# davipatti/abdpymc

Hardware: AMD Instinct MI355X
Metric: logp+grad evals/sec (higher is better)
Workload: dtype f64; 1 GPU; synthetic 10000 ind x 200 gaps, fp64, 4 chains/GPU; n_inds=10000, n_gaps=200, storage=f64, chains_per_gpu=4, total_chains=4, parallelism=chains sharded 4/GPU x 1

## Files before the change

abdpymc_amd/csrc/abd_context.hip:

```cpp
#include "abd_host.hpp"

#include <memory>
#include <unordered_map>
#include "abd_small.hpp"
#include "abd_curves.hpp"
#include "abd_risk.hpp"
#include "abd_diag.hpp"
#include "abd_timeline.hpp"

static_assert(ABD_TL_BINS == ABD_TIMELINE_BINS && ABD_TL_MAX_DRAWS == ABD_TIMELINE_MAX_DRAWS && ABD_TL_MAX_Q == ABD_TIMELINE_MAX_Q &&
                  ABD_TL_NINF == ABD_TIMELINE_NINF,
              "abd_timeline.hpp and include/abd_hip.h describe the same counters");

namespace abdi {

namespace {
thread_local std::string g_err = "";
}
int fail(int code, const char* fmt, ...) {
  char buf[512];
  va_list ap;
  va_start(ap, fmt);
  vsnprintf(buf, sizeof buf, fmt, ap);
  va_end(ap);
  g_err = buf;
  return code;
}
const char* last_error() { return g_err.c_str(); }
void set_error(const std::string& msg) { g_err = msg; }

double prior_constant(int G) {
  double v = -(std::lgamma(1.0) + std::lgamma((double)(G - 1)) - std::lgamma((double)G));
  v += -2.0 * (std::lgamma(10.0) + std::lgamma(1.0) - std::lgamma(11.0));
  const double gmu[5] = {2.0, 1.0, 2.0, 1.0, 1.0};
  for (int q = 0; q < 5; ++q) {
    const double al = gmu[q] * gmu[q] / 0.25, be = gmu[q] / 0.25;
    v += al * std::log(be) - std::lgamma(al);
  }
  const double nsd[6] = {1.0, 1.0, 0.5, 0.5, 0.5, 0.5};
  for (int q = 0; q < 6; ++q) v += -std::log(nsd[q]) - 0.5 * kLog2Pi;
  return v;
}

ModelSizes model_sizes(const abd_ctx* c) {
  ModelSizes m;
  m.G = c->G;
  m.dense = c->dense ? 1 : 0;
  m.N = (double)c->N;
  m.cells = (double)c->G * (double)c->N;
  m.Kn = (double)c->n.K;
  m.Ks = (double)c->s.K;
  m.prior_const = c->prior_const;
  return m;
}

void assemble(const abd_ctx* c, const HostTerms& h, const double* t, const double* sums, double* logp, double* grad,
              bool with_priors) {
  assemble_terms(model_sizes(c), h, t, sums, logp, grad, with_priors);
}

ChainPar chain_par(const abd_ctx* c, int chain, const Transformed& tr) {
  ChainPar p;
  chain_par_from_tr(p, &tr.p);
  p.rw = c->slots[chain].rw;
  p.waner = c->slots[chain].waner;
  p.iw = c->slots[chain].iw;
  p.cnt = c->slots[chain].cnt;
  return p;
}
ChainPar chain_par(const abd_ctx* c, int chain, const double* t) { return chain_par(c, chain, transform(t)); }

ConstrainArgs constrain_args(const abd_ctx* c) {
  ConstrainArgs a;
  std::memset(&a, 0, sizeof a);
  a.pw = c->ignore_pcr ? nullptr : c->pw;
  a.N = c->N;
  a.nt = c->nt;
  a.n_chunks = c->n_chunks;
  std::memcpy(a.chunk_mask, c->chunk_mask, sizeof a.chunk_mask);
  return a;
}

#ifdef ABD_STAMPS
unsigned long long* stamps_buffer() {
  static MappedBuf<unsigned long long>& stamps = *new MappedBuf<unsigned long long>();
  if (!stamps) {
    (void)stamps.alloc(4096 * 16);
    if (const char* e = std::getenv("ABD_STAMPS_PTR_OUT")) {
      FILE* f = std::fopen(e, "w");
      if (f) {
        std::fprintf(f, "%llu\n", (unsigned long long)(uintptr_t)stamps.host());
        std::fclose(f);
      }
    }
  }
  return stamps.dev();
}
#endif

void base_args(const abd_ctx* c, EvalArgs& a) {
  std::memset(&a, 0, sizeof a);
  a.y_n = c->n.y;
  a.x_n = c->n.x;
  a.y_s = c->s.y;
  a.x_s = c->s.x;
  a.g_n = c->n.g;
  a.g_s = c->s.g;
  a.ptr_n = c->n.ptr;
  a.ptr_s = c->s.ptr;
  a.j_n = c->n.j;
  a.j_s = c->s.j;
  a.K_n = (int32_t)c->n.K;
  a.K_s = (int32_t)c->s.K;
  a.ob_n = c->ob_n;
  a.ob_s = c->ob_s;
  a.ob_c = c->ob_c;
  a.yx_n = c->n.yx;
  a.yx_s = c->s.yx;
  a.yxi_n = c->n.yxi;
  a.yxi_s = c->s.yxi;
  a.od_n = c->n.od;
  a.od_s = c->s.od;
  a.xc_n = c->n.xc;
  a.xc_s = c->s.xc;
  a.dict_n = c->n.dict;
  a.dict_s = c->s.dict;
  a.n_dict_n = c->n.n_dict;
  a.n_dict_s = c->s.n_dict;
  a.vw = c->vw;
  a.pw = c->ignore_pcr ? nullptr : c->pw;
  a.exp2_tab = c->exp2_tab;
#ifdef ABD_STAMPS
  a.stamps = stamps_buffer();
#endif
  a.G = c->G;
  a.N = c->N;
  a.nt = c->nt;
  a.n_chunks = c->n_chunks;
  a.n_lg = c->n_lg;
  std::memcpy(a.chunk_mask, c->chunk_mask, sizeof a.chunk_mask);
}
int probe_stream_queues(abd_ctx* c) {
  if (c->n_queues > 0) return ABD_OK;
  HIP_TRY(hipSetDevice(c->device));
  constexpr int kCand = 2 * kMaxPipes;
  const int ns = c->n_streams;
  Stream spare[kMaxPipes];
  hipStream_t cand[kCand] = {};
  int n_cand = ns;
  for (int pi = 0; pi < ns; ++pi) cand[pi] = c->pipe[pi].st;
  for (; n_cand < ns + kMaxPipes; ++n_cand) {
    if (spare[n_cand - ns].create() != hipSuccess) {
      (void)hipGetLastError();
      break;
    }
    cand[n_cand] = spare[n_cand - ns];
  }
  DevBuf<unsigned long long> d;
  hipError_t le = d.alloc((size_t)kCand * 2);
  int best_nq = 0, best[kCand] = {};
  for (int attempt = 0; attempt < 3 && best_nq < 4 && le == hipSuccess; ++attempt) {
    le = hipDeviceSynchronize();
    for (int k = 0; k < n_cand && le == hipSuccess; ++k) {
      hipLaunchKernelGGL(abd_spin_kernel, dim3(1), dim3(64), 0, cand[k], d + 2 * k, 15000ull + 2000ull * (unsigned long long)k);
      le = hipGetLastError();
    }
    if (le == hipSuccess) le = hipDeviceSynchronize();
    unsigned long long h[kCand * 2] = {};
    if (le == hipSuccess) le = hipMemcpy(h, d, sizeof(unsigned long long) * 2 * (size_t)n_cand, hipMemcpyDeviceToHost);
    if (le != hipSuccess) break;
    int nq = 0, q_of[kCand] = {};
    unsigned long long busy_until[kCand] = {};
    for (int j = 0; j < n_cand; ++j) {
      int q = -1;
      for (int k = 0; k < nq && q < 0; ++k)
        if (h[2 * j] + 300 >= busy_until[k] && h[2 * j] <= busy_until[k] + 800) q = k;
      if (q < 0) q = nq++;
      q_of[j] = q;
      busy_until[q] = h[2 * j + 1];
    }
    if (nq > best_nq) {
      best_nq = nq;
      std::copy(q_of, q_of + kCand, best);
    }
  }
  const int nq = std::max(1, best_nq);
  if (le == hipSuccess && best_nq > 1) {
    int load[kCand] = {};
    bool used[kCand] = {};
    for (int pi = 0; pi < ns; ++pi) load[best[pi]]++;
    for (int pi = ns - 1; pi >= 1; --pi) {
      const int q = best[pi];
      int q_min = 0;
      for (int k = 1; k < nq; ++k)
        if (load[k] < load[q_min]) q_min = k;
      if (load[q] - load[q_min] < 2) continue;
      int k_spare = -1;
      for (int k = ns; k < n_cand && k_spare < 0; ++k)
        if (!used[k] && best[k] == q_min) k_spare = k;
      if (k_spare < 0) continue;
      used[k_spare] = true;
      std::swap(c->pipe[pi].st, spare[k_spare - ns]);
      cand[pi] = c->pipe[pi].st;
      best[pi] = q_min;
      load[q]--;
      load[q_min]++;
    }
  }
  HIP_TRY(le);
  int renum[kCand], n_seen = 0;
  std::fill(renum, renum + kCand, -1);
  for (int pi = 0; pi < ns; ++pi) {
    if (renum[best[pi]] < 0) renum[best[pi]] = n_seen++;
    c->queue_of_pipe[pi] = renum[best[pi]];
  }
  c->n_queues = std::max(1, n_seen);
  int k = 0;
  bool taken[kMaxPipes] = {};
  for (int round = 0; k < c->n_streams; ++round) {
    bool seen[kMaxPipes] = {};
    for (int pi = 0; pi < c->n_streams; ++pi)
      if (!taken[pi] && !seen[c->queue_of_pipe[pi]]) {
        seen[c->queue_of_pipe[pi]] = true;
// ... 90 lines not shown
    if (fits) {
      std::vector<R> od(code.size(), (R)0);
      for (size_t j = 0; j < (size_t)N; ++j)
        for (size_t g = 0; g < (size_t)G; ++g) od[cell_of(g, j)] = yx[g * N + j].y;
      d.n_dict = (int)dict.size();
      HIP_TRY(d.od.upload(od.data(), od.size() * sizeof(R)));
      HIP_TRY(d.xc.upload(code.data(), code.size()));
      dict.resize(ABD_XDICT, 0.0);
      HIP_TRY(d.dict.upload(dict.data(), ABD_XDICT));
    }
    return ABD_OK;
  }
  std::vector<R> y(std::max<size_t>(K, 1)), x(std::max<size_t>(K, 1));
  std::vector<uint16_t> g(std::max<size_t>(K, 1));
  std::vector<int32_t> jj(std::max<size_t>(K, 1));
  for (size_t k = 0; k < K; ++k) {
    const int64_t src = so.order[k];
    y[k] = (R)o.od[src];
    x[k] = (R)o.log_dilution[src];
    g[k] = (uint16_t)o.idx_gap[src];
    jj[k] = (int32_t)o.idx_ind[src];
  }
  HIP_TRY(d.j.upload(jj.data(), jj.size()));
  HIP_TRY(d.y.upload(y.data(), y.size() * sizeof(R)));
  HIP_TRY(d.x.upload(x.data(), x.size() * sizeof(R)));
  HIP_TRY(d.g.upload(g.data(), g.size()));
  HIP_TRY(d.ptr.upload(so.ptr.data(), so.ptr.size()));
  return ABD_OK;
}

std::vector<uint64_t> pack_ng(const int8_t* src, int G, int N, int nt) {
  std::vector<uint64_t> w((size_t)nt * N, 0);
  if (!src) return w;
  for (int j = 0; j < N; ++j)
    for (int g = 0; g < G; ++g)
      if (src[(size_t)j * G + g]) w[(size_t)(g >> 6) * N + j] |= 1ull << (g & 63);
  return w;
}

namespace {

int validate_desc(const abd_desc* d) {
  const int G = d->n_gaps, N = d->n_inds;
  if (G < 2) return fail(ABD_ERR_ARG, "n_gaps must be >= 2 (Beta(1, n_gaps - 1) prior on p), got %d", G);
  if (G > ABD_MAX_GAPS) return fail(ABD_ERR_ARG, "n_gaps=%d exceeds ABD_MAX_GAPS=%d", G, ABD_MAX_GAPS);
  if (N < 1) return fail(ABD_ERR_ARG, "n_inds must be >= 1, got %d", N);
  if ((int64_t)G * N >= (int64_t)1 << 31) return fail(ABD_ERR_ARG, "n_gaps*n_inds too large");
  if (d->n_chain_slots < 1) return fail(ABD_ERR_ARG, "n_chain_slots must be >= 1");
  if (d->storage != ABD_STORE_F64 && d->storage != ABD_STORE_F32) return fail(ABD_ERR_ARG, "unknown storage %d", d->storage);
  if (!d->vacs) return fail(ABD_ERR_ARG, "vacs is NULL");
  if (d->n_splits < 0 || d->n_splits > 2) return fail(ABD_ERR_ARG, "only implemented 1-3 time chunks (0-2 splits)");
  for (int k = 0; k < d->n_splits; ++k)
    if (d->splits[k] < 0) return fail(ABD_ERR_ARG, "split indexes must be positive");
  if (d->n_splits == 2 && d->splits[0] > d->splits[1]) return fail(ABD_ERR_ARG, "splits must be in ascending order");
  if (d->n_splits > 0 && d->splits[d->n_splits - 1] > G) return fail(ABD_ERR_ARG, "largest split must be less than n_gaps - 1, (%d)", d->splits[d->n_splits - 1]);
  if (d->n_splits == 2 && d->splits[0] == d->splits[1]) return fail(ABD_ERR_ARG, "splits not unique");
  for (int64_t k = 0; k < (int64_t)G * N; ++k) {
    if ((d->vacs[k] != 0 && d->vacs[k] != 1)) return fail(ABD_ERR_ARG, "vacs must be 0/1");
    if (d->pcrpos && d->pcrpos[k] != 0 && d->pcrpos[k] != 1) return fail(ABD_ERR_ARG, "pcrpos must be 0/1");
  }
  return ABD_OK;
}

int derive_sizes(abd_ctx* c, const abd_desc* d, bool one_per_cell) {
  const int G = d->n_gaps, N = d->n_inds;
  c->G = G;
  c->N = N;
  c->nt = (G + 63) / 64;
  c->prior_const = prior_constant(G);
  c->n_lg = (N + 63) / 64;
  c->n_chunks = d->n_splits + 1;
  for (int k = 0; k < d->n_splits; ++k) c->splits[k] = d->splits[k];
  c->storage = d->storage;
  c->dense = one_per_cell;
  if ((int64_t)N * (d->storage == ABD_STORE_F32 ? 8 : 16) * (G + 2) >= ((int64_t)1 << 32)) c->dense = false;
  if (!abd_div_magic_exact((uint64_t)c->n_lg * (uint64_t)G, (uint32_t)G)) c->dense = false;
  if (env_int("ABD_FORCE_SPARSE", 0)) c->dense = false;
  c->ignore_pcr = d->pcrpos == nullptr;
  c->n_slots = d->n_chain_slots;
  {
    const int edges[4] = {0, d->n_splits > 0 ? d->splits[0] : G, d->n_splits > 1 ? d->splits[1] : G, G};
    for (int ch = 0; ch < c->n_chunks; ++ch) {
      const int lo = edges[ch], hi = (ch == c->n_chunks - 1) ? G : edges[ch + 1];
      for (int g = lo; g < hi; ++g) c->chunk_mask[ch][g >> 6] |= 1ull << (g & 63);
    }
  }

  int dev = d->device;
  if (dev < 0) HIP_TRY(hipGetDevice(&dev));
  c->device = dev;
  HIP_TRY(hipSetDevice(dev));
  hipDeviceProp_t prop;
  HIP_TRY(hipGetDeviceProperties(&prop, dev));
  c->n_cu = prop.multiProcessorCount;
  snprintf(c->name, sizeof c->name, "%s %s %d CUs", prop.name, prop.gcnArchName, prop.multiProcessorCount);
  HIP_TRY(c->pipe[0].st.create());
  c->stream = c->pipe[0].st;

  const int bpc = std::max(1, tune_int("ABD_BLOCKS_PER_CU", 2));
  const int sparse_max = std::max(1, std::min((N + ABD_WAVES_PER_BLOCK - 1) / ABD_WAVES_PER_BLOCK, c->n_cu * 16));
  c->blocks_x = std::max(1, std::min(sparse_max, c->n_cu * bpc));
  c->dbpc = std::max(1, tune_int("ABD_DENSE_BLOCKS_PER_CU", 4));
  {
    const int cap = c->n_cu * 8;
    c->ob_n = (int)std::min<int64_t>((d->n.n_obs + ABD_BLOCK - 1) / ABD_BLOCK, cap);
    c->ob_s = (int)std::min<int64_t>((d->s.n_obs + ABD_BLOCK - 1) / ABD_BLOCK, cap);
    c->ob_c = 1;
    c->obs_lanes = d->s.n_obs + d->n.n_obs < (int64_t)256 * N;
    c->obs_lanes = env_int("ABD_OBS_LANES", c->obs_lanes ? 1 : 0) != 0;
  }
  c->blocks_max = std::max({sparse_max, c->n_cu * 16, c->ob_n + c->ob_s + c->ob_c});
  c->dense_blocks = std::min(c->n_cu * c->dbpc, c->blocks_max);
  if (dense_lds_bytes(G, 4) > 160 * 1024) return fail(ABD_ERR_ARG, "LDS tables for n_gaps=%d do not fit", G);
  return ABD_OK;
}

int upload_panels(abd_ctx* c, const abd_desc* d, SortedObs& so_s, SortedObs& so_n) {
  const int G = c->G, N = c->N;
  const auto upload = c->storage == ABD_STORE_F32 ? upload_antigen<float> : upload_antigen<double>;
  if (int rc = upload(c, d->s, so_s, c->s)) return rc;
  if (int rc = upload(c, d->n, so_n, c->n)) return rc;
  c->order_s = std::move(so_s.order);
  c->order_n = std::move(so_n.order);
  c->xc_ok = c->dense && c->s.od && c->n.od;
  c->xc_max_cb = tune_int("ABD_XC_MAX_CB", c->xc_max_cb);
  const size_t words = (size_t)c->nt * N;
  const std::vector<uint64_t> vw = pack_ng(d->vacs, G, N, c->nt);
  const std::vector<uint64_t> pw = pack_ng(d->pcrpos, G, N, c->nt);
  HIP_TRY(c->vw.upload(vw.data(), words));
  HIP_TRY(c->pw.upload(pw.data(), words));
  if (c->dense) {
    std::vector<double> tab(ABD_EXP2_TAB);
    for (int j = 0; j < ABD_EXP2_TAB; ++j) {
      const double t = (double)exp2l((long double)j / (long double)ABD_EXP2_TAB);
      uint64_t bits;
      std::memcpy(&bits, &t, sizeof bits);
      bits = abd_exp2_prebias(bits, j);
      std::memcpy(&tab[(size_t)j], &bits, sizeof bits);
    }
    HIP_TRY(c->exp2_tab.upload(tab.data(), tab.size()));
  }
  HIP_TRY(c->stage_gn.alloc((size_t)G * N));
  return ABD_OK;
}

int create_slots(abd_ctx* c) {
  const size_t words = (size_t)c->nt * c->N;
  c->slots.resize((size_t)c->n_slots);
  for (auto& s : c->slots) {
    HIP_TRY(s.rw.alloc(words));
    HIP_TRY(s.waner.alloc((size_t)c->N));
    HIP_TRY(s.iw.alloc(words));
    HIP_TRY(s.cnt.alloc(2));
  }
  return ABD_OK;
}

int create_pipes(abd_ctx* c) {
  c->n_pipes = std::max(1, std::min(6, env_int("ABD_PIPES", c->n_pipes)));
  if (!c->dense) c->n_pipes = 1;
  c->n_streams = kMaxPipes;
  c->n_sync_slots = std::max(4, c->n_slots);
  for (int pi = 1; pi < c->n_streams; ++pi) {
    HIP_TRY(c->pipe[pi].st.create());
    HIP_TRY(c->join_ev[pi].create(hipEventDisableTiming));
  }
  c->pipe_blocks = std::min(c->dense_blocks, c->n_cu * std::max(1, c->dbpc / c->n_pipes));
  if (const int pb = tune_int("ABD_PIPE_BLOCKS", 0)) c->pipe_blocks = std::max(1, std::min(pb, c->blocks_max));
  c->group_blocks = c->n_cu;
  if (const int gb = tune_int("ABD_GROUP_BLOCKS_PER_CU", 0)) c->group_blocks = std::max(1, std::min(c->n_cu * gb, c->blocks_max));
  for (int pi = 0; pi < kMaxPipes; ++pi)
    if (c->pipe[pi].st)
      for (int b = 0; b < 2; ++b) HIP_TRY(c->pipe[pi].partials[b].alloc((size_t)c->n_slots * c->blocks_max * ABD_NOUT));
  c->xcd_remap = tune_int("ABD_XCD_REMAP", 1) != 0;
  c->fin_rows = std::max(0, tune_int("ABD_FIN_ROWS", 2));
  HIP_TRY(c->out.alloc((size_t)(kResultSlots + c->n_sync_slots) * c->n_slots * ABD_NOUT));
  HIP_TRY(c->d_counts.alloc((size_t)c->n_slots * 2 + 8));
  HIP_TRY(c->d_work.alloc((size_t)2 * c->n_slots));
  HIP_TRY(c->d_counts_chain.alloc((size_t)c->n_slots * 2));
  HIP_TRY(c->d_fin_count.alloc_zero((size_t)kMaxPipes * ABD_MAX_BATCH, c->stream));
  HIP_TRY(c->d_train_count.alloc_zero((size_t)kMaxPipes * (1 + ABD_TRAIN_SHARDS) * ABD_TRAIN_CNT_STRIDE, c->stream));
  c->dense_own_sum = env_int("ABD_DENSE_OWN_SUM", 1) != 0;
  HIP_TRY(c->h_counts_chain.alloc_pinned((size_t)c->n_slots * 2));
  c->g2_refill_min = std::max(1, std::min(64, tune_int("ABD_G2_REFILL_MIN", ABD_G2_REFILL_MIN)));
  c->g2_tail_lanes = std::max(0, std::min(64, tune_int("ABD_G2_TAIL_LANES", ABD_G2_TAIL_LANES)));
  c->g2_tail_age = std::max(0, tune_int("ABD_G2_TAIL_AGE", ABD_G2_TAIL_AGE));
  c->results.resize((size_t)kResultSlots + c->n_sync_slots);
  HIP_TRY(hipStreamSynchronize(c->stream));
  if (c->dense && c->n_pipes > 1) {
    if (int rc = probe_stream_queues(c)) return rc;
    c->n_pipes = std::min(c->n_pipes, c->n_queues);
  }
  return ABD_OK;
}

}

int launch_deterministics(abd_ctx* c, int chain, const double* theta, hipStream_t st, int8_t* out_i, double* out_mun, double* out_mus,
                          double* sums) {
  EvalArgs a;
  base_args(c, a);
  a.n_chains = 1;
  a.ch[0] = chain_par(c, chain, theta);
  const size_t lds = (size_t)3 * (c->G + 1) * sizeof(double2_t);
  const int blocks = std::max(1, std::min((c->N + ABD_WAVES_PER_BLOCK - 1) / ABD_WAVES_PER_BLOCK, c->n_cu * 8));
  if (c->nt > ABD_MAXT)
    hipLaunchKernelGGL(abd_deterministics_kernel<ABD_MAXT_MAX>, dim3(blocks), dim3(ABD_BLOCK), lds, st, a, out_i, out_mun, out_mus, sums);
  else
    hipLaunchKernelGGL(abd_deterministics_kernel<ABD_MAXT>, dim3(blocks), dim3(ABD_BLOCK), lds, st, a, out_i, out_mun, out_mus, sums);
  HIP_TRY(hipGetLastError());
  return ABD_OK;
}

size_t curves_row_cols(const abd_ctx* c) { return (size_t)abd_curves_row_cols(c->G); }
size_t curves_scratch_cols(const abd_ctx* c) { return (size_t)abd_curves_slabs(c->N) * curves_row_cols(c); }

int launch_curves(abd_ctx* c, int chain, const double* theta, double thr_s, double thr_n, hipStream_t st, unsigned long long* scratch,
                  unsigned long long* row) {
  const ChainPar p = chain_par(c, chain, theta);
  CurvesArgs a;
  a.vw = c->vw;
  a.iw = p.iw;
  a.waner = p.waner;
  a.last = c->d_last;
  a.slab_rows = scratch;
  a.rho_n = p.rho_n, a.rho_s = p.rho_s, a.init_n = p.init_n, a.perm_n = p.perm_n, a.temp_n = p.temp_n;
  a.init_s = p.init_s, a.perm_s = p.perm_s;
  a.thr_s = thr_s, a.thr_n = thr_n;
  a.G = c->G, a.N = c->N, a.nt = c->nt, a.n_slabs = abd_curves_slabs(c->N);
  const size_t lds = (size_t)3 * (c->G + 1) * sizeof(double2_t) + (size_t)2 * c->G * sizeof(double) + ((size_t)4 * c->G + ABD_CURVES_NBIN) * sizeof(int);
  const int blocks = std::max(1, std::min(a.n_slabs, c->n_cu * 8));
  if (c->nt > ABD_MAXT)
    hipLaunchKernelGGL(abd_curves_kernel<ABD_MAXT_MAX>, dim3(blocks), dim3(ABD_BLOCK), lds, st, a);
  else
    hipLaunchKernelGGL(abd_curves_kernel<ABD_MAXT>, dim3(blocks), dim3(ABD_BLOCK), lds, st, a);
  HIP_TRY(hipGetLastError());
  const int sum_blocks = (int)((curves_row_cols(c) + ABD_CURVES_SUM_COLS - 1) / ABD_CURVES_SUM_COLS);
  hipLaunchKernelGGL(abd_curves_sum_kernel, dim3(sum_blocks), dim3(ABD_CURVES_SUM_PARTS * ABD_CURVES_SUM_COLS), 0, st, scratch, a.n_slabs,
                     c->G, row);
  HIP_TRY(hipGetLastError());
  return ABD_OK;
}

void split_curves_row(const abd_ctx* c, const unsigned long long* row, int64_t* counts, int64_t* n_infections, double* titer_sums) {
  const size_t G = (size_t)c->G;
  if (counts) std::memcpy(counts, row, 4 * G * sizeof(int64_t));
  if (n_infections) std::memcpy(n_infections, row + 4 * G, ABD_CURVES_NBIN * sizeof(int64_t));
  if (titer_sums) std::memcpy(titer_sums, row + 4 * G + ABD_CURVES_NBIN, 2 * G * sizeof(double));
}

int launch_diag(abd_ctx* c, int chain, const double* theta, hipStream_t st, int64_t d, int64_t H, int64_t L, double* tit, uint32_t* inf,
                unsigned long long* cb2) {
  const ChainPar p = chain_par(c, chain, theta);
  DiagArgs a;
  a.vw = c->vw;
  a.iw = p.iw;
  a.waner = p.waner;
  a.tit = tit, a.inf = reinterpret_cast<DiagInf*>(inf), a.cb2 = cb2;
  a.rho_n = p.rho_n, a.rho_s = p.rho_s, a.init_n = p.init_n, a.perm_n = p.perm_n, a.temp_n = p.temp_n;
  a.init_s = p.init_s, a.perm_s = p.perm_s;
  a.w = diag_draw(d, H, L);
  a.G = c->G, a.N = c->N, a.nt = c->nt;
  const size_t lds = (size_t)3 * (c->G + 1) * sizeof(double2_t);
  const int blocks = std::max(1, std::min((c->N + ABD_WAVES_PER_BLOCK - 1) / ABD_WAVES_PER_BLOCK, c->n_cu * 8));
  if (c->nt > ABD_MAXT)
    hipLaunchKernelGGL(abd_diag_kernel<ABD_MAXT_MAX>, dim3(blocks), dim3(ABD_BLOCK), lds, st, a);
  else
    hipLaunchKernelGGL(abd_diag_kernel<ABD_MAXT>, dim3(blocks), dim3(ABD_BLOCK), lds, st, a);
  HIP_TRY(hipGetLastError());
  return ABD_OK;
}

int launch_diag_export(abd_ctx* c, const void* src, int stride, int width, unsigned long long* dst, hipStream_t st) {
  const int64_t tiles = (int64_t)((c->G + ABD_DIAG_TILE - 1) / ABD_DIAG_TILE) * ((c->N + ABD_DIAG_TILE - 1) / ABD_DIAG_TILE);
  hipLaunchKernelGGL(abd_diag_export_kernel, dim3((unsigned)tiles), dim3(256), 0, st, static_cast<const unsigned char*>(src), stride, width,
                     c->G, c->N, dst);
  HIP_TRY(hipGetLastError());
  return ABD_OK;
}

int launch_timeline(abd_ctx* c, int chain, const double* theta, const double range_n[2], const double range_s[2], hipStream_t st,
                    uint32_t* hist_n, uint32_t* hist_s, uint32_t* cell, uint32_t* ninf) {
  const ChainPar p = chain_par(c, chain, theta);
  TimelineArgs a;
  a.vw = c->vw;
  a.iw = p.iw;
  a.waner = p.waner;
  a.last = c->d_last;
  a.hist_n = hist_n, a.hist_s = hist_s, a.cell = reinterpret_cast<TimelineCell*>(cell), a.ninf = ninf;
  a.rho_n = p.rho_n, a.rho_s = p.rho_s, a.init_n = p.init_n, a.perm_n = p.perm_n, a.temp_n = p.temp_n;
  a.init_s = p.init_s, a.perm_s = p.perm_s;
  a.rn = timeline_range(range_n[0], range_n[1]), a.rs = timeline_range(range_s[0], range_s[1]);
  a.G = c->G, a.N = c->N, a.nt = c->nt;
  a.n_splits = c->n_chunks - 1, a.s0 = c->splits[0], a.s1 = c->splits[1];
  const size_t lds = (size_t)3 * (c->G + 1) * sizeof(double2_t);
  const int blocks = std::max(1, std::min((c->N + ABD_WAVES_PER_BLOCK - 1) / ABD_WAVES_PER_BLOCK, c->n_cu * 8));
  if (c->nt > ABD_MAXT)
    hipLaunchKernelGGL(abd_timeline_kernel<ABD_MAXT_MAX>, dim3(blocks), dim3(ABD_BLOCK), lds, st, a);
  else
    hipLaunchKernelGGL(abd_timeline_kernel<ABD_MAXT>, dim3(blocks), dim3(ABD_BLOCK), lds, st, a);
  HIP_TRY(hipGetLastError());
  return ABD_OK;
}

int launch_timeline_hist_export(abd_ctx* c, const uint32_t* src, int g0, int n_g, void* dst, hipStream_t st) {
  const int64_t cells = (int64_t)n_g * c->N;
  const int blocks = (int)std::max<int64_t>(1, std::min<int64_t>((cells + 31) / 32, (int64_t)c->n_cu * 16));
  hipLaunchKernelGGL(abd_timeline_hist_export_kernel, dim3(blocks), dim3(256), 0, st, reinterpret_cast<const uint4*>(src), c->G, c->N, g0,
                     n_g, static_cast<uint4*>(dst));
  HIP_TRY(hipGetLastError());
  return ABD_OK;
}

int launch_timeline_quantiles(abd_ctx* c, const uint32_t* hist, int64_t chain_stride, int n_chains, const double range[2], int n_q,
                              const double* q, double* out, hipStream_t st) {
  const int64_t tiles = (int64_t)((c->G + ABD_TL_QTILE - 1) / ABD_TL_QTILE) * ((c->N + ABD_TL_QTILE - 1) / ABD_TL_QTILE);
  hipLaunchKernelGGL(abd_timeline_quantile_kernel, dim3((unsigned)tiles), dim3(256), 0, st, hist, chain_stride, n_chains, c->G, c->N,
                     timeline_range(range[0], range[1]), n_q, q, out);
  HIP_TRY(hipGetLastError());
  return ABD_OK;
}

size_t risk_table_cols(const abd_ctx* c) { return (size_t)abd_risk_table_cols(c->G); }
size_t risk_scratch_cols(const abd_ctx* c) { return (size_t)abd_curves_slabs(c->N) * (size_t)abd_risk_packed_cols(c->G); }

int check_risk_spec(const abd_ctx* c, const abd_risk_spec* spec) {
  if (!spec) return fail(ABD_ERR_ARG, "risk: spec is NULL");
  if (spec->start < 0 || spec->end > c->G || (int64_t)spec->end - spec->start < 2)
    return fail(ABD_ERR_ARG, "risk: window (%d, %d) needs 0 <= start, end <= %d and end - start >= 2", spec->start, spec->end, c->G);
  if (spec->first_only != 0 && spec->first_only != 1) return fail(ABD_ERR_ARG, "risk: first_only=%d is not 0 or 1", spec->first_only);
  const struct { const char* name; int n; const double* e; } ag[2] = {{"edges_s", spec->n_edges_s, spec->edges_s},
                                                                     {"edges_n", spec->n_edges_n, spec->edges_n}};
  for (const auto& x : ag) {
    if (x.n < 0 || x.n > ABD_RISK_MAX_EDGES) return fail(ABD_ERR_ARG, "risk: n_%s=%d outside [0, %d]", x.name, x.n, ABD_RISK_MAX_EDGES);
    for (int k = 0; k < x.n; ++k) {
      if (!std::isfinite(x.e[k])) return fail(ABD_ERR_ARG, "risk: %s[%d] is not finite", x.name, k);
      if (k && !(x.e[k] > x.e[k - 1])) return fail(ABD_ERR_ARG, "risk: %s is not strictly ascending at [%d]", x.name, k);
    }
  }
  return ABD_OK;
}

int launch_risk(abd_ctx* c, int chain, const double* theta, const abd_risk_spec& spec, hipStream_t st, unsigned long long* scratch,
                uint32_t* table) {
  const ChainPar p = chain_par(c, chain, theta);
  RiskArgs a;
  a.vw = c->vw;
  a.iw = p.iw;
  a.waner = p.waner;
  a.last = c->d_last;
  a.slab_rows = scratch;
  a.rho_n = p.rho_n, a.rho_s = p.rho_s, a.init_n = p.init_n, a.perm_n = p.perm_n, a.temp_n = p.temp_n;
  a.init_s = p.init_s, a.perm_s = p.perm_s;
  for (int k = 0; k < ABD_RISK_MAX_EDGES; ++k) {
    a.edges_s[k] = k < spec.n_edges_s ? spec.edges_s[k] : HUGE_VAL;
    a.edges_n[k] = k < spec.n_edges_n ? spec.edges_n[k] : HUGE_VAL;
  }
  a.G = c->G, a.N = c->N, a.nt = c->nt, a.n_slabs = abd_curves_slabs(c->N);
  a.start = spec.start, a.end = spec.end, a.first_only = spec.first_only;
  const size_t lds = (size_t)3 * (c->G + 1) * sizeof(double2_t) + (size_t)abd_risk_packed_cols(c->G) * sizeof(unsigned long long) +
                     (size_t)2 * ABD_RISK_MAX_EDGES * sizeof(double);
  const int blocks = std::max(1, std::min(a.n_slabs, c->n_cu * 8));
  if (c->nt > ABD_MAXT)
    hipLaunchKernelGGL(abd_risk_kernel<ABD_MAXT_MAX>, dim3(blocks), dim3(ABD_BLOCK), lds, st, a);
  else
    hipLaunchKernelGGL(abd_risk_kernel<ABD_MAXT>, dim3(blocks), dim3(ABD_BLOCK), lds, st, a);
  HIP_TRY(hipGetLastError());
  const int sum_blocks = (int)((abd_risk_packed_cols(c->G) + ABD_RISK_SUM_COLS - 1) / ABD_RISK_SUM_COLS);
  hipLaunchKernelGGL(abd_risk_sum_kernel, dim3(sum_blocks), dim3(ABD_RISK_SUM_PARTS * ABD_RISK_SUM_COLS), 0, st, scratch, a.n_slabs, c->G,
                     table);
  HIP_TRY(hipGetLastError());
  return ABD_OK;
}

int launch_unpack(abd_ctx* c, int chain, int8_t* dst, hipStream_t st) {
  dim3 grid((c->N + 255) / 256, c->G);
  hipLaunchKernelGGL(abd_unpack_bits_kernel, grid, dim3(256), 0, st, c->slots[(size_t)chain].rw, dst, c->G, c->N);
  HIP_TRY(hipGetLastError());
  return ABD_OK;
}

}

abd_ctx::~abd_ctx() {
  (void)hipSetDevice(device);
  for (Pipe& p : pipe)
    if (p.st) (void)hipStreamSynchronize(p.st);
}

extern "C" {

const char* abd_version(void) { return "abdpymc_amd hip gfx950 0.2"; }

const char* abd_last_error(void) { return last_error(); }

int abd_create(const abd_desc* d, abd_ctx** out) {
  if (!d || !out) return fail(ABD_ERR_ARG, "desc / out is NULL");
  *out = nullptr;
  if (int rc = validate_desc(d)) return rc;
  SortedObs so_s, so_n;
  if (int rc = sort_obs(d->s, d->n_gaps, d->n_inds, "s", so_s)) return rc;
  if (int rc = sort_obs(d->n, d->n_gaps, d->n_inds, "n", so_n)) return rc;
  std::unique_ptr<abd_ctx> c(new (std::nothrow) abd_ctx());
  if (!c) return fail(ABD_ERR_NOMEM, "out of host memory");
  if (int rc = derive_sizes(c.get(), d, so_s.one_per_cell && so_n.one_per_cell)) return rc;
  if (int rc = upload_panels(c.get(), d, so_s, so_n)) return rc;
  if (int rc = create_slots(c.get())) return rc;
  if (int rc = create_pipes(c.get())) return rc;
  *out = c.release();
  return ABD_OK;
}

int abd_destroy(abd_ctx* c) {
  delete c;
  return ABD_OK;
}

int abd_device_name(abd_ctx* c, char* buf, int32_t buflen) {
  if (!c || !buf || buflen < 1) return fail(ABD_ERR_ARG, "bad argument");
  snprintf(buf, (size_t)buflen, "%s", c->name);
  return ABD_OK;
}

int abd_is_dense(abd_ctx* c) { return c && c->dense ? 1 : 0; }
int abd_n_pipes(abd_ctx* c) { return c ? c->n_pipes : -1; }

int abd_set_discrete(abd_ctx* c, int32_t chain, const int8_t* i_raw, const int8_t* waner) {
  if (!c || !i_raw || !waner) return fail(ABD_ERR_ARG, "NULL argument");
  if (chain < 0 || chain >= c->n_slots) return fail(ABD_ERR_ARG, "chain %d outside [0, %d)", chain, c->n_slots);
  const size_t cells = (size_t)c->G * c->N;
  for (size_t k = 0; k < cells; ++k)
    if (i_raw[k] != 0 && i_raw[k] != 1) return fail(ABD_ERR_ARG, "i_raw must be 0/1");
  for (int j = 0; j < c->N; ++j)
    if (waner[j] != 0 && waner[j] != 1) return fail(ABD_ERR_ARG, "ab_s_waner must be 0/1");
  HIP_TRY(hipSetDevice(c->device));
  ChainSlot& s = c->slots[(size_t)chain];
  long long* const cnt = s.cnt;
  if (int jrc = join_pipes(c)) return jrc;
  HIP_TRY(hipStreamSynchronize(c->stream));
  HIP_TRY(hipMemcpy(c->stage_gn, i_raw, cells, hipMemcpyHostToDevice));
  HIP_TRY(hipMemcpy(s.waner, waner, (size_t)c->N, hipMemcpyHostToDevice));
  dim3 grid((c->N + 255) / 256, c->nt);
  hipLaunchKernelGGL(abd_pack_bits_kernel, grid, dim3(256), 0, c->stream, c->stage_gn, s.rw, c->G, c->N, c->nt);
  HIP_TRY(hipGetLastError());
  HIP_TRY(hipMemsetAsync(s.cnt, 0, 2 * sizeof(long long), c->stream));
  if (c->nt > ABD_MAXT)
    hipLaunchKernelGGL(abd_constrain_kernel<ABD_MAXT_MAX>, dim3((c->N + 255) / 256), dim3(256), 0, c->stream, constrain_args(c), s.rw,
                       s.waner, s.iw, reinterpret_cast<unsigned long long*>(cnt));
  else
    hipLaunchKernelGGL(abd_constrain_kernel<ABD_MAXT>, dim3((c->N + 255) / 256), dim3(256), 0, c->stream, constrain_args(c), s.rw,
                       s.waner, s.iw, reinterpret_cast<unsigned long long*>(cnt));
  HIP_TRY(hipGetLastError());
  HIP_TRY(hipStreamSynchronize(c->stream));
  s.set = true;
  return ABD_OK;
}

int abd_flip_discrete(abd_ctx* c, int32_t chain, int64_t flat) {
  if (!c) return fail(ABD_ERR_ARG, "ctx is NULL");
  if (chain < 0 || chain >= c->n_slots) return fail(ABD_ERR_ARG, "chain %d outside [0, %d)", chain, c->n_slots);
  const int64_t total = (int64_t)c->G * c->N + c->N;
  if (flat < 0 || flat >= total) return fail(ABD_ERR_ARG, "flat index %lld outside [0, %lld)", (long long)flat, (long long)total);
  if (!c->slots[(size_t)chain].set) return fail(ABD_ERR_STATE, "chain slot %d has no discrete state", chain);
  HIP_TRY(hipSetDevice(c->device));
  if (int jrc = join_pipes(c)) return jrc;
  ChainSlot& s = c->slots[(size_t)chain];
  long long* const cnt = s.cnt;
  if (c->nt > ABD_MAXT)
    hipLaunchKernelGGL(abd_flip_kernel<ABD_MAXT_MAX>, dim3(1), dim3(1), 0, c->stream, constrain_args(c), s.rw, s.waner, s.iw,
                       reinterpret_cast<unsigned long long*>(cnt), c->G, flat);
  else
    hipLaunchKernelGGL(abd_flip_kernel<ABD_MAXT>, dim3(1), dim3(1), 0, c->stream, constrain_args(c), s.rw, s.waner, s.iw,
                       reinterpret_cast<unsigned long long*>(cnt), c->G, flat);
  HIP_TRY(hipGetLastError());
  return ABD_OK;
}
int abd_deterministics(abd_ctx* c, int32_t chain, const double* theta, int8_t* i, double* mu_n, double* mu_s) {
  if (!c || !theta) return fail(ABD_ERR_ARG, "NULL argument");
  int rc = check_chains(c, 1, &chain);
  if (rc) return rc;
  HIP_TRY(hipSetDevice(c->device));
  if (int jrc = join_pipes(c)) return jrc;
  const size_t cells = (size_t)c->G * c->N;
  if (!c->d_det) HIP_TRY(c->d_det.alloc(2 * cells + (cells + 7) / 8));
  double* d_n = c->d_det;
  double* d_s = c->d_det + cells;
  int8_t* d_i = reinterpret_cast<int8_t*>(c->d_det + 2 * cells);
  if (int lrc = launch_deterministics(c, chain, theta, c->stream, i ? d_i : (int8_t*)nullptr, mu_n ? d_n : (double*)nullptr,
                                      mu_s ? d_s : (double*)nullptr, nullptr))
    return lrc;
  if (mu_n) HIP_TRY(hipMemcpyAsync(mu_n, d_n, cells * sizeof(double), hipMemcpyDeviceToHost, c->stream));
  if (mu_s) HIP_TRY(hipMemcpyAsync(mu_s, d_s, cells * sizeof(double), hipMemcpyDeviceToHost, c->stream));
  if (i) HIP_TRY(hipMemcpyAsync(i, d_i, cells, hipMemcpyDeviceToHost, c->stream));
  HIP_TRY(hipStreamSynchronize(c->stream));
  return ABD_OK;
}

int abd_set_follow_up(abd_ctx* c, const int32_t* last_gap) {
  if (!c) return fail(ABD_ERR_ARG, "ctx is NULL");
  if (last_gap)
    for (int j = 0; j < c->N; ++j)
      if (last_gap[j] < -1 || last_gap[j] >= c->G)
        return fail(ABD_ERR_ARG, "last_gap[%d]=%d outside [-1, %d)", j, last_gap[j], c->G);
  HIP_TRY(hipSetDevice(c->device));
  if (int jrc = join_pipes(c)) return jrc;
  HIP_TRY(hipStreamSynchronize(c->stream));
  if (!last_gap) {
    c->d_last.reset();
    return ABD_OK;
  }
  DevBuf<int32_t> fresh;
  HIP_TRY(fresh.upload(last_gap, (size_t)c->N));
  c->d_last = std::move(fresh);
  return ABD_OK;
}

int abd_curves(abd_ctx* c, int32_t chain, const double* theta, double thr_s, double thr_n, int64_t* counts, int64_t* n_infections,
               double* titer_sums) {
  if (!c || !theta) return fail(ABD_ERR_ARG, "NULL argument");
  int rc = check_chains(c, 1, &chain);
  if (rc) return rc;
  HIP_TRY(hipSetDevice(c->device));
  if (int jrc = join_pipes(c)) return jrc;
  const size_t n_scratch = curves_scratch_cols(c), n_row = curves_row_cols(c);
  if (!c->d_curves) HIP_TRY(c->d_curves.alloc(n_scratch + n_row));
  if (int lrc = launch_curves(c, chain, theta, thr_s, thr_n, c->stream, c->d_curves, c->d_curves + n_scratch)) return lrc;
  std::vector<unsigned long long> h(n_row);
  HIP_TRY(hipMemcpyAsync(h.data(), c->d_curves + n_scratch, n_row * sizeof(unsigned long long), hipMemcpyDeviceToHost, c->stream));
  HIP_TRY(hipStreamSynchronize(c->stream));
  split_curves_row(c, h.data(), counts, n_infections, titer_sums);
  return ABD_OK;
}

int abd_risk(abd_ctx* c, int32_t chain, const double* theta, const abd_risk_spec* spec, int64_t* table) {
  if (!c || !theta || !table) return fail(ABD_ERR_ARG, "NULL argument");
  int rc = check_chains(c, 1, &chain);
  if (rc) return rc;
  if (int src = check_risk_spec(c, spec)) return src;
  HIP_TRY(hipSetDevice(c->device));
  if (int jrc = join_pipes(c)) return jrc;
  const size_t n_scratch = risk_scratch_cols(c), n_tab = risk_table_cols(c);
  if (!c->d_risk) HIP_TRY(c->d_risk.alloc(n_scratch + (n_tab + 1) / 2));
  uint32_t* d_tab = reinterpret_cast<uint32_t*>(c->d_risk + n_scratch);
  if (int lrc = launch_risk(c, chain, theta, *spec, c->stream, c->d_risk, d_tab)) return lrc;
  std::vector<uint32_t> h(n_tab);
  HIP_TRY(hipMemcpyAsync(h.data(), d_tab, n_tab * sizeof(uint32_t), hipMemcpyDeviceToHost, c->stream));
  HIP_TRY(hipStreamSynchronize(c->stream));
  for (size_t e = 0; e < n_tab; ++e) table[e] = (int64_t)h[e];
  return ABD_OK;
}

int abd_get_discrete(abd_ctx* c, int32_t chain, int8_t* i_raw, int8_t* waner) {
  if (!c) return fail(ABD_ERR_ARG, "ctx is NULL");
  int rc = check_chains(c, 1, &chain);
  if (rc) return rc;
  HIP_TRY(hipSetDevice(c->device));
  if (int jrc = join_pipes(c)) return jrc;
  ChainSlot& s = c->slots[(size_t)chain];
  if (i_raw) {
    if (int urc = launch_unpack(c, chain, c->stage_gn, c->stream)) return urc;
    HIP_TRY(hipStreamSynchronize(c->stream));
    HIP_TRY(hipMemcpy(i_raw, c->stage_gn, (size_t)c->G * c->N, hipMemcpyDeviceToHost));
  } else {
    HIP_TRY(hipStreamSynchronize(c->stream));
  }
  if (waner) HIP_TRY(hipMemcpy(waner, s.waner, (size_t)c->N, hipMemcpyDeviceToHost));
  return ABD_OK;
}

int abd_set_launch_config(abd_ctx* c, int32_t blocks, int32_t chains_per_wave) {
  if (!c) return fail(ABD_ERR_ARG, "ctx is NULL");
  if (!(chains_per_wave == 0 || chains_per_wave == 1 || chains_per_wave == 2 || chains_per_wave == 4))
    return fail(ABD_ERR_ARG, "chains_per_wave must be 0 (auto), 1, 2 or 4");
  c->cpw_forced = chains_per_wave;
  if (blocks > 0) {
    if (c->dense)
      c->dense_blocks = std::max(1, std::min(blocks, c->blocks_max));
    else
      c->blocks_x = std::max(1, std::min(blocks, c->blocks_max));
  }
  return ABD_OK;
}

int abd_theta_prior(abd_ctx* c, const double* theta, double* logp, double* grad) {
  if (!c || !theta || !logp) return fail(ABD_ERR_ARG, "NULL argument");
  *logp = priors(prepare(theta), theta, c->G, 0.0, 0.0, 0.0, 0.0, grad, c->prior_const);
  return ABD_OK;
}

int abd_set_individual_offset(abd_ctx* c, int64_t first_individual) {
  if (!c) return fail(ABD_ERR_ARG, "ctx is NULL");
  if (first_individual < 0 || first_individual > 0xFFFFFFFFll) return fail(ABD_ERR_ARG, "first_individual=%lld out of range", (long long)first_individual);
  c->ind_offset = (uint32_t)first_individual;
  return ABD_OK;
}
int abd_stream_queues(abd_ctx* c, int32_t* queue_of_stream, int32_t n) {
  if (!c || !queue_of_stream) return fail(ABD_ERR_ARG, "NULL argument");
  if (int rc = probe_stream_queues(c)) return rc;
  for (int i = 0; i < n; ++i) queue_of_stream[i] = i < c->n_streams ? c->queue_of_pipe[i] : -1;
  return ABD_OK;
}

int64_t abd_algorithmic_bytes(abd_ctx* c, int32_t n_chains) {
  if (!c) return 0;
  const int64_t R = c->storage == ABD_STORE_F32 ? 4 : 8;
  const int64_t cells = (int64_t)c->G * c->N;
  const int64_t bits = (int64_t)c->nt * c->N * 8 * (2 + n_chains) + (int64_t)n_chains * c->N;
  const int cpw = n_chains % 4 == 0 ? 4 : (n_chains % 2 == 0 ? 2 : 1);
  if (c->dense && c->xc_ok && cpw <= c->xc_max_cb) return cells * 2 * (R + 1) + bits;
  if (c->dense) return cells * 4 * R + bits;
  return (c->s.K + c->n.K) * (2 * R + 2) + 2 * (int64_t)(c->N + 1) * 4 + bits;
}

}
```

abdpymc_amd/csrc/abd_dense.hpp:

```cpp
#pragma once

#include <cstddef>

#include "abd_device.hpp"
#include "abd_terms.hpp"

typedef uint32_t abd_u32x4 __attribute__((ext_vector_type(4)));
typedef uint32_t abd_u32x2 __attribute__((ext_vector_type(2)));
template <typename R>
__device__ __forceinline__ YX<R> load_yx(const __amdgpu_buffer_rsrc_t& rs, uint32_t voff, uint32_t soff);
template <>
__device__ __forceinline__ YX<double> load_yx<double>(const __amdgpu_buffer_rsrc_t& rs, uint32_t voff, uint32_t soff) {
  const abd_u32x4 v = __builtin_amdgcn_raw_buffer_load_b128(rs, voff, soff, 0);
  YX<double> r;
  r.y = __hiloint2double((int)v.y, (int)v.x);
  r.x = __hiloint2double((int)v.w, (int)v.z);
  return r;
}
template <>
__device__ __forceinline__ YX<float> load_yx<float>(const __amdgpu_buffer_rsrc_t& rs, uint32_t voff, uint32_t soff) {
  const abd_u32x2 v = __builtin_amdgcn_raw_buffer_load_b64(rs, voff, soff, 0);
  YX<float> r;
  r.y = __uint_as_float(v.x);
  r.x = __uint_as_float(v.y);
  return r;
}

template <typename R, bool XC>
struct RowData;
template <typename R>
struct RowData<R, false> {
  YX<R> v;
};
template <typename R>
struct RowData<R, true> {
  R y;
  uint32_t code;
};
template <bool XC>
struct RowDesc;
template <>
struct RowDesc<false> {
  __amdgpu_buffer_rsrc_t rs;
};
template <>
struct RowDesc<true> {
  __amdgpu_buffer_rsrc_t rs_y, rs_c;
};
__device__ __forceinline__ __amdgpu_buffer_rsrc_t rsrc_at(const void* base, int64_t byte_off) {
  return __builtin_amdgcn_make_buffer_rsrc(const_cast<char*>(reinterpret_cast<const char*>(base)) + byte_off, 0, -1, 0x00020000);
}
template <typename R, bool XC, typename ARGS>
__device__ __forceinline__ RowDesc<XC> row_desc(const ARGS& a, int antigen, int lg, int g0) {
  RowDesc<XC> d;
  if constexpr (XC) {
    const int64_t cell0 = ((int64_t)lg * a.G + g0) * 64;
    d.rs_y = rsrc_at(antigen ? a.od_s : a.od_n, cell0 * (int64_t)sizeof(R));
    d.rs_c = rsrc_at(antigen ? a.xc_s : a.xc_n, cell0);
  } else {
    const int64_t cell0 = (int64_t)g0 * a.N + (int64_t)lg * 64;
    d.rs = rsrc_at(antigen ? a.yx_s : a.yx_n, cell0 * (int64_t)sizeof(YX<R>));
  }
  return d;
}
template <typename R, bool XC>
__device__ __forceinline__ RowData<R, XC> row_load(const RowDesc<XC>& d, int lane, int row, int N) {
  RowData<R, XC> r;
  if constexpr (XC) {
    const uint32_t soff = (uint32_t)row * 64u;
    if constexpr (sizeof(R) == 8) {
      const abd_u32x2 v = __builtin_amdgcn_raw_buffer_load_b64(d.rs_y, (uint32_t)lane * 8u, soff * 8u, 0);
      r.y = __hiloint2double((int)v.y, (int)v.x);
    } else {
      r.y = __uint_as_float(__builtin_amdgcn_raw_buffer_load_b32(d.rs_y, (uint32_t)lane * 4u, soff * 4u, 0));
    }
    r.code = __builtin_amdgcn_raw_buffer_load_b8(d.rs_c, (uint32_t)lane, soff, 0);
  } else {
    r.v = load_yx<R>(d.rs, (uint32_t)lane * (uint32_t)sizeof(YX<R>), (uint32_t)row * (uint32_t)N * (uint32_t)sizeof(YX<R>));
  }
  return r;
}
template <typename R, bool XC>
__device__ __forceinline__ double row_y(const RowData<R, XC>& r) {
  if constexpr (XC) return (double)r.y;
  else return (double)r.v.y;
}
template <typename R, bool XC>
__device__ __forceinline__ double row_x(const RowData<R, XC>& r, const double* dict ) {
  if constexpr (XC) return dict[r.code];
  else return (double)r.v.x;
}

__device__ __forceinline__ uint32_t word32(const uint32_t* base, uint32_t j2, int q, int N) {
  const uint32_t* row = base + ((int64_t)(q >> 1) * 2 * N + (q & 1));
  return row[j2];
}

#define ABD_EXP2_C2 0x1.ebfbe033445b4p-23
__device__ __forceinline__ void one_plus_exp2_pair(double t_n, double t_s, const double* tab , double c2v, double& A,
                                                   double& B) {
  const double kf_n = __builtin_rint(t_n), kf_s = __builtin_rint(t_s);
  const double f_n = t_n - kf_n, f_s = t_s - kf_s;
  int k_n, k_s;
  asm("v_cvt_i32_f64 %0, %1" : "=v"(k_n) : "v"(kf_n));
  asm("v_cvt_i32_f64 %0, %1" : "=v"(k_s) : "v"(kf_s));
  const int kc_n = min(max(k_n, ABD_EXP2_K_MIN), ABD_EXP2_K_MAX), kc_s = min(max(k_s, ABD_EXP2_K_MIN), ABD_EXP2_K_MAX);
  const double T_n = tab[kc_n & (ABD_EXP2_TAB - 1)], T_s = tab[kc_s & (ABD_EXP2_TAB - 1)];
  double p_n, p_s;
  asm("v_fma_f64 %0, %1, %2, %3" : "=v"(p_n) : "s"(0x1.c6b08d910ecbdp-35), "v"(f_n), "v"(c2v));
  asm("v_fma_f64 %0, %1, %2, %3" : "=v"(p_s) : "s"(0x1.c6b08d910ecbdp-35), "v"(f_s), "v"(c2v));
  p_n = fma(p_n, f_n, 0x1.62e42fefa39efp-11);
  p_s = fma(p_s, f_s, 0x1.62e42fefa39efp-11);
  p_n = fma(p_n, f_n, 1.0);
  p_s = fma(p_s, f_s, 1.0);
  const double Ts_n = __hiloint2double((int)abd_exp2_scaled_hi((uint32_t)__double2hiint(T_n), kc_n), __double2loint(T_n));
  const double Ts_s = __hiloint2double((int)abd_exp2_scaled_hi((uint32_t)__double2hiint(T_s), kc_s), __double2loint(T_s));
  A = fma(Ts_n, p_n, 1.0);
  B = fma(Ts_s, p_s, 1.0);
}

template <bool GRAD>
__device__ __forceinline__ void obs_pair_scaled(double t_n, double yn, double d_n, double t_s, double ys, double d_s,
                                                const double* tab, double c2v, double (&acc)[16], double& h_n, double& h_s) {
  double A, B;
  one_plus_exp2_pair(t_n, t_s, tab, c2v, A, B);
  const double r = rcp_newton(A * B);
  const double s_n = r * B, s_s = r * A;
  const double q_n = fma(-d_n, s_n, yn), q_s = fma(-d_s, s_s, ys);
  acc[A_N_Q2] = fma(q_n, q_n, acc[A_N_Q2]);
  acc[A_S_Q2] = fma(q_s, q_s, acc[A_S_Q2]);
  if (GRAD) {
    const double u_n = q_n * s_n, u_s = q_s * s_s;
    acc[A_N_QS] += u_n;
    acc[A_S_QS] += u_s;
    h_n = fma(-u_n, s_n, u_n);
    h_s = fma(-u_s, s_s, u_s);
    acc[A_N_H] += h_n;
    acc[A_S_H] += h_s;
    acc[A_N_HX] = fma(h_n, t_n, acc[A_N_HX]);
    acc[A_S_HX] = fma(h_s, t_s, acc[A_S_HX]);
  }
}

#ifdef ABD_STAMPS
#define ABD_STAMP(k)                                                                                  \
  do {                                                                                                \
    if (a.stamps && wave == 0 && lane == 0 && blockIdx.y == 0)                                        \
      a.stamps[(int64_t)blockIdx.x * 16 + (k)] = __builtin_amdgcn_s_memrealtime();                   \
  } while (0)
#else
#define ABD_STAMP(k)
#endif

struct DenseChain {
  double rho_n, rho_s;
  double ct_n, cp_n, ci_n, mc_n;
  double c_s, cp_s, ci_s, mc_s;
  double d_n, d_s;
};
__device__ __forceinline__ DenseChain dense_chain(const ChainPar& p) {
  DenseChain k;
  const double c_n = p.b_n * (1.4426950408889634074 * ABD_EXP2_TAB), c_s = p.b_s * (1.4426950408889634074 * ABD_EXP2_TAB);
  k.rho_n = p.rho_n;
  k.rho_s = p.rho_s;
  k.ct_n = readfirstlane_f64(c_n * p.temp_n);
  k.cp_n = readfirstlane_f64(c_n * p.perm_n);
  k.ci_n = to_vgpr(c_n * p.init_n);
  k.mc_n = readfirstlane_f64(-c_n);
  k.c_s = readfirstlane_f64(c_s);
  k.cp_s = readfirstlane_f64(c_s * p.perm_s);
  k.ci_s = to_vgpr(c_s * p.init_s);
  k.mc_s = readfirstlane_f64(-c_s);
  k.d_n = p.d_n;
  k.d_s = p.d_s;
  return k;
}

#define ABD_SW 8
template <typename R, bool XC>
struct PieceLoads {
  uint32_t seg_i, seg_v, nxt_i, nxt_v;
  RowData<R, XC> en, es, on, os;
  int wj;
};

template <typename R, bool XC, typename ARGS>
__device__ __forceinline__ void piece_issue_loads(const ARGS& a, const RowDesc<XC>& rs_n, const RowDesc<XC>& rs_s,
                                                  const uint32_t* ibase, const uint32_t* vbase, const int8_t* waner, int lane, int j,
                                                  int g0, int g1, PieceLoads<R, XC>& pl) {
  const int N = a.N;
  const int q = g0 >> 5, q_end = (g1 - 1) >> 5;
  const int last = g1 - 1 - g0;
  const int re = min(g0 & 1, last), ro = min((g0 & 1) ^ 1, last);
  if (g0 & 1) {
    pl.on = row_load<R, XC>(rs_n, lane, ro, N);
    pl.os = row_load<R, XC>(rs_s, lane, ro, N);
    pl.en = row_load<R, XC>(rs_n, lane, re, N);
    pl.es = row_load<R, XC>(rs_s, lane, re, N);
  } else {
    pl.en = row_load<R, XC>(rs_n, lane, re, N);
    pl.es = row_load<R, XC>(rs_s, lane, re, N);
    pl.on = row_load<R, XC>(rs_n, lane, ro, N);
    pl.os = row_load<R, XC>(rs_s, lane, ro, N);
  }
  const uint32_t j2 = 2u * (uint32_t)j;
  pl.seg_i = word32(ibase, j2, q, N);
  pl.seg_v = word32(vbase, j2, q, N);
  pl.nxt_i = pl.nxt_v = 0;
  if (q < q_end) {
    pl.nxt_i = word32(ibase, j2, q + 1, N);
    pl.nxt_v = word32(vbase, j2, q + 1, N);
  }
  pl.wj = waner[j];
}

__device__ __forceinline__ void state_issue_loads(const uint32_t* ibase, const uint32_t* vbase, uint32_t j2, int N, int g0,
                                                  uint32_t (&wi)[ABD_SW], uint32_t (&wv)[ABD_SW]) {
  const int qlast = (g0 - 1) >> 5;
#pragma unroll
  for (int u = 0; u < ABD_SW; ++u) {
    wi[u] = wv[u] = 0;
    if (u <= qlast) {
      wi[u] = word32(ibase, j2, u, N);
      wv[u] = word32(vbase, j2, u, N);
    }
  }
}

__device__ __forceinline__ void dense_start_state(uint32_t (&wi)[ABD_SW], uint32_t (&wv)[ABD_SW], const uint32_t* ibase,
                                                  const uint32_t* vbase, uint32_t j2, int N, int g0, const double2_t* tab_n,
                                                  const double2_t* tab_s, bool wj, double& tn, double& dn, double& ts, double& ds,
                                                  uint32_t& cfn_hi, uint32_t& cfs_hi) {
  const int qlast = (g0 - 1) >> 5;
  uint32_t any_i = 0, any_v = 0;
  int cnt = 0;
  for (int q0 = 0;; q0 += ABD_SW) {
#pragma unroll
    for (int u = 0; u < ABD_SW; ++u) {
      const int q = q0 + u;
      if (q <= qlast) {
        const int rel = g0 - q * 32;
        uint32_t mi = wi[u], mv = wv[u];
        if (rel < 32) {
          const uint32_t below = (1u << rel) - 1u;
          mi &= below;
          mv &= below;
        }
        any_i |= mi;
        any_v |= mv;
        cnt += __builtin_popcount(mi) + __builtin_popcount(mv);
        if (__builtin_amdgcn_ballot_w64((mi | mv) != 0) != 0) {
          while (mi | mv) {
            const int idx_i = mi ? rel - __builtin_ctz(mi) : 0;
            const int idx_v = mv ? rel - __builtin_ctz(mv) : 0;
            mi &= mi - 1;
            mv &= mv - 1;
            const double2_t pn = tab_n[idx_i];
            const double2_t ps = tab_s[idx_i];
            const double2_t pv = tab_s[idx_v];
            tn += pn.x;
            dn += pn.y;
            ts += ps.x;
            ds += ps.y;
            ts += pv.x;
            ds += pv.y;
          }
        }
      }
    }
    if (q0 + ABD_SW > qlast) break;
#pragma unroll
    for (int u = 0; u < ABD_SW; ++u) {
      const int q = q0 + ABD_SW + u;
      wi[u] = wv[u] = 0;
      if (q <= qlast) {
        wi[u] = word32(ibase, j2, q, N);
        wv[u] = word32(vbase, j2, q, N);
      }
    }
  }
  if (!wj) {
    ts = (double)cnt;
    ds = 0.0;
  }
  cfn_hi = any_i ? 0x3FF00000u : 0u;
  cfs_hi = (any_i | any_v) ? 0x3FF00000u : 0u;
}

template <typename R, bool GRAD, bool XC, typename ARGS>
__device__ __forceinline__ void dense_walk(const ARGS& a, const DenseChain& k, const RowDesc<XC>& rs_n,
                                           const RowDesc<XC>& rs_s, const double* dict_n, const double* dict_s,
                                           const uint32_t* ibase, const uint32_t* vbase,
                                           uint32_t j2, PieceLoads<R, XC>& pl, int lane, int g0, int g1, bool wj, double tn, double dn, double ts,
                                           double ds, uint32_t cfn_hi, uint32_t cfs_hi, const double* tab_e2, double c2v,
                                           double (&acc)[16]) {
  const int N = a.N;
  const double rho_n = k.rho_n, ct_n = k.ct_n, cp_n = k.cp_n, ci_n = k.ci_n, mc_n = k.mc_n;
  const double c_s = k.c_s, cp_s = k.cp_s, ci_s = k.ci_s, mc_s = k.mc_s, d_n = k.d_n, d_s = k.d_s;
  const double rho_j = wj ? k.rho_s : 1.0;
  double hd_s = 0.0;
  const uint32_t z_ei = zero_vgpr(), z_ev = zero_vgpr(), z_cn = zero_vgpr(), z_cs = zero_vgpr();
  const int last = g1 - 1 - g0;
  auto ldrow = [&](const RowDesc<XC>& rs, int g) { return row_load<R, XC>(rs, lane, min(g - g0, last), N); };
  int q = g0 >> 5;
  const int q_end = (g1 - 1) >> 5;
  uint32_t seg_i = pl.seg_i, seg_v = pl.seg_v;
  auto next_word = [&]() {
    seg_i = pl.nxt_i;
    seg_v = pl.nxt_v;
    ++q;
    if (q < q_end) {
      pl.nxt_i = word32(ibase, j2, q + 1, N);
      pl.nxt_v = word32(vbase, j2, q + 1, N);
    }
  };

  auto step = [&](int g, const RowData<R, XC>& on, const RowData<R, XC>& os) {
    const uint32_t bit = (uint32_t)g & 31u;
    const uint32_t ei_hi = (uint32_t)__builtin_amdgcn_sbfe((int)seg_i, bit, 1u) & 0x3FF00000u;
    const uint32_t ev_hi = (uint32_t)__builtin_amdgcn_sbfe((int)seg_v, bit, 1u) & 0x3FF00000u;
    const double e_i = hi_to_double(ei_hi, z_ei), e_v = hi_to_double(ev_hi, z_ev);
    cfn_hi |= ei_hi;
    cfs_hi |= ei_hi | ev_hi;
    dn = fma_s(rho_n, dn, tn);
    tn = fma_s(rho_n, tn, e_i);
    ds = fma_v(rho_j, ds, ts);
    ts = fma_v(rho_j, ts, e_i + e_v);
    const double cf_n = hi_to_double(cfn_hi, z_cn), cf_s = hi_to_double(cfs_hi, z_cs);
    const double t_n = fma(mc_n, row_x<R, XC>(on, dict_n), fma(ct_n, tn, fma(cf_n, cp_n, ci_n)));
    const double t_s = fma(mc_s, row_x<R, XC>(os, dict_s), fma(c_s, ts, fma(cf_s, cp_s, ci_s)));
    double h_n = 0.0, h_s = 0.0;
    obs_pair_scaled<GRAD>(t_n, row_y<R, XC>(on), d_n, t_s, row_y<R, XC>(os), d_s, tab_e2, c2v, acc, h_n, h_s);
    if (GRAD) {
      acc[A_N_HC] = fma(h_n, cf_n, acc[A_N_HC]);
      acc[A_N_HU] = fma(h_n, tn, acc[A_N_HU]);
      acc[A_N_HD] = fma(h_n, dn, acc[A_N_HD]);
      acc[A_S_HC] = fma(h_s, cf_s, acc[A_S_HC]);
      hd_s = fma(h_s, ds, hd_s);
    }
  };

  RowData<R, XC> en = pl.en, es = pl.es, on = pl.on, os = pl.os;
  int g = g0;
  if (g & 1) {
    step(g, on, os);
    on = ldrow(rs_n, g + 2);
    os = ldrow(rs_s, g + 2);
    ++g;
    if (g < g1 && (g & 31) == 0) next_word();
  }
  while (g + 1 < g1) {
    const int pair_end = min(((g >> 5) + 1) << 5, g1 - 1);
    for (; g < pair_end; g += 2) {
      step(g, en, es);
      en = ldrow(rs_n, g + 2);
      es = ldrow(rs_s, g + 2);
      step(g + 1, on, os);
      on = ldrow(rs_n, g + 3);
      os = ldrow(rs_s, g + 3);
    }
    if (g < g1 && (g & 31) == 0) next_word();
  }
  if (g < g1) step(g, en, es);
  acc[A_S_HD] += wj ? hd_s : 0.0;
}

__device__ __forceinline__ const char* train_kernarg() {
#if defined(__HIP_DEVICE_COMPILE__)
  return (const char*)__builtin_amdgcn_kernarg_segment_ptr();
#else
  return nullptr;
#endif
}
__device__ __forceinline__ const TrainPoint* train_point(const TrainArgs& T) {
  return T.use_slot >= 0 ? T.slots + T.use_slot
                         : reinterpret_cast<const TrainPoint*>(train_kernarg() + offsetof(EvalArgs, train) + offsetof(TrainArgs, first));
}

__device__ __forceinline__ void train_forward_record(const TrainArgs& T, int lane) {
  const TrainPoint* cur = T.slots + T.use_slot;
  if (lane < ABD_NT) {
    T.fwd_rec->g[lane] = cur->prev_g[lane];
    T.fwd_rec->next_theta[lane] = cur->theta[lane];
    T.fwd_rec->next_p_half[lane] = cur->p_half[lane];
    if (lane == 0) T.fwd_rec->lp = cur->prev_lp;
  }
  __threadfence_system();
  __builtin_amdgcn_wave_barrier();
  if (lane == 0) __hip_atomic_store(&T.fwd_rec->tag, T.fwd_tag, __ATOMIC_RELEASE, __HIP_MEMORY_SCOPE_SYSTEM);
}

__device__ __forceinline__ void train_epilogue(const EvalArgs& a, double* sm, int lane) {
  const TrainArgs& T = a.train;
  const TrainPoint* cur = train_point(T);
  const double* inv_mass = reinterpret_cast<const double*>(train_kernarg() + offsetof(EvalArgs, train) + offsetof(TrainArgs, inv_mass));
  double* lps = sm + 16;
  const int k = lane < ABD_NT ? lane : 0;
  const int q4 = k == 0 ? 0 : k == 3 ? 1 : k == 6 ? 2 : k == 7 ? 3 : -1;
  abdi::Transformed tr;
  tr.p = cur->tr[0];
  tr.perm_n = cur->tr[1];
  tr.temp_n = cur->tr[2];
  tr.rho_n = cur->tr[3];
  tr.init_n = cur->tr[4];
  tr.perm_s = cur->tr[5];
  tr.rho_s = cur->tr[6];
  tr.q = cur->tr[7];
  tr.tinf = cur->tr[8];
  tr.tvac = cur->tr[9];
  tr.init_s = cur->tr[10];
  tr.b_n = cur->tr[11];
  tr.d_n = cur->tr[12];
  tr.sig_n = cur->tr[13];
  tr.b_s = cur->tr[14];
  tr.d_s = cur->tr[15];
  tr.sig_s = cur->tr[16];
  abdi::ModelSizes m;
  m.G = a.G;
  m.dense = 0;
  m.N = (double)a.N;
  m.cells = (double)a.G * (double)a.N;
  m.Kn = (double)a.K_n;
  m.Ks = (double)a.K_s;
  m.prior_const = T.prior_const;
  const double tk = cur->theta[k];
  const double l0 = q4 >= 0 ? cur->L0[q4] : 0.0, l1 = q4 >= 0 ? cur->L1[q4] : 0.0;
  double lp_k, g_k;
  abdi::assemble_lane(k, m, tr, tk, cur->tr[k], l0, l1, sm, lp_k, g_k);
  if (lane < ABD_NT) lps[lane] = lp_k;
  __builtin_amdgcn_wave_barrier();
  double lp = 0.0;
#pragma unroll
  for (int q = 0; q < ABD_NT; ++q) lp += lps[q];
  if (lane < ABD_NT) {
    if (T.own_record) {
      T.rec->g[lane] = g_k;
      if (lane == 0) T.rec->lp = lp;
    }
    const bool finite = __builtin_isfinite(lp);
    const double gd = finite ? g_k : 0.0;
    const double kick = __dmul_rn(__dmul_rn(0.5, T.ve), gd);
    const double p = __dadd_rn(cur->p_half[lane], kick);
    const double ph = __dadd_rn(p, kick);
    const double v = __dmul_rn(inv_mass[lane], ph);
    const double t2 = __dadd_rn(tk, __dmul_rn(T.ve, v));
    if (T.own_record) {
      T.rec->next_theta[lane] = t2;
      T.rec->next_p_half[lane] = ph;
    }
    double tr2, n0, n1;
    abdi::transform_lane(lane, t2, tr2, n0, n1);
    TrainPoint* nx = T.slots + T.next_slot;
    nx->theta[lane] = t2;
    nx->p_half[lane] = ph;
    nx->tr[lane] = tr2;
    if (q4 >= 0) {
      nx->L0[q4] = n0;
      nx->L1[q4] = n1;
    }
    nx->prev_g[lane] = g_k;
    if (lane == 0) nx->prev_lp = lp;
  }
  if (!T.own_record) return;
  __threadfence_system();
  __builtin_amdgcn_wave_barrier();
  if (lane == 0) __hip_atomic_store(&T.rec->tag, T.tag, __ATOMIC_RELEASE, __HIP_MEMORY_SCOPE_SYSTEM);
}

#define ABD_TRAIN_SM 64
__host__ __device__ inline size_t abd_dense_lds(int G, int cb, bool xc = false, bool train = false) {
  const size_t need = (size_t)cb * 2 * (size_t)(G + 1) * sizeof(double2_t) + (size_t)ABD_WAVES_PER_BLOCK * ABD_NOUT * sizeof(double) +
                      (size_t)ABD_EXP2_TAB * sizeof(double) + (xc ? (size_t)2 * ABD_XDICT * sizeof(double) : 0);
  const size_t fin = (size_t)ABD_FIN_PARTS * ABD_NOUT * sizeof(double) + (train ? (size_t)ABD_TRAIN_CB * ABD_TRAIN_SM * sizeof(double) : 0);
  return need > fin ? need : fin;
}

template <typename ARGS>
struct is_train_args {
  static constexpr bool value = false;
};
template <>
struct is_train_args<DenseTrainArgs> {
  static constexpr bool value = true;
};

__device__ __forceinline__ void train_service(const DenseTrainArgs& a, int wave, int lane);
__device__ __forceinline__ void train_step(const DenseTrainArgs& a, const TrainChainArgs& tc, double* sm, int lane);

template <int CB>
__device__ __forceinline__ bool two_level_sums(const double* rows, double* shard_rows, unsigned int* cnt, int nblk, int blk, unsigned int mask,
                                               int* flag, double* sm_chain, int tid) {
  const int lane = tid & 63, wave = tid >> 6;
  const int shard = blk % ABD_TRAIN_SHARDS;
  const int n_in_shard = (nblk - shard + ABD_TRAIN_SHARDS - 1) / ABD_TRAIN_SHARDS;
  const int n_shards = min(nblk, ABD_TRAIN_SHARDS);
  unsigned int* cnt_shard = cnt + (1 + shard) * ABD_TRAIN_CNT_STRIDE;
  if (wave == 0) {
    handoff_drain_stores();
    if (lane == 0) {
      const unsigned int old = handoff_count_in(cnt_shard);
      flag[0] = old + 1u == (unsigned int)n_in_shard ? 1 : 0;
    }
  }
  __syncthreads();
  const bool shard_last = flag[0] != 0;
  __syncthreads();
  if (!shard_last) return false;
  handoff_acquire();
  if (wave == 0) {
    if (lane < CB * ABD_NOUT) {
      const int cc = lane / ABD_NOUT, k = lane % ABD_NOUT;
      double v = 0.0;
      if ((mask >> cc) & 1u) {
        const double* col = rows + ((int64_t)cc * nblk + shard) * ABD_NOUT + k;
        for (int i0 = 0; i0 < n_in_shard; i0 += 8) {
          double q[8];
#pragma unroll
          for (int u = 0; u < 8; ++u)
            q[u] = i0 + u < n_in_shard ? __hip_atomic_load(col + (int64_t)(i0 + u) * ABD_TRAIN_SHARDS * ABD_NOUT, __ATOMIC_RELAXED, __HIP_MEMORY_SCOPE_AGENT) : 0.0;
#pragma unroll
          for (int u = 0; u < 8; ++u) v += q[u];
        }
      }
      __hip_atomic_store(shard_rows + ((int64_t)cc * ABD_TRAIN_SHARDS + shard) * ABD_NOUT + k, v, __ATOMIC_RELAXED, __HIP_MEMORY_SCOPE_AGENT);
    }
    handoff_drain_stores();
    if (lane == 0) {
      __hip_atomic_store(cnt_shard, 0u, __ATOMIC_RELAXED, __HIP_MEMORY_SCOPE_AGENT);
      const unsigned int old = handoff_count_in(cnt);
      flag[0] = old + 1u == (unsigned int)n_shards ? 1 : 0;
    }
  }
  __syncthreads();
  const bool last = flag[0] != 0;
  __syncthreads();
  if (!last) return false;
  handoff_acquire();
  if (wave == 0 && lane < CB * ABD_NOUT) {
    const int cc = lane / ABD_NOUT, k = lane % ABD_NOUT;
    const double* col = shard_rows + (int64_t)cc * ABD_TRAIN_SHARDS * ABD_NOUT + k;
    double v = 0.0;
    for (int i0 = 0; i0 < n_shards; i0 += 8) {
      double q[8];
#pragma unroll
      for (int u = 0; u < 8; ++u) q[u] = i0 + u < n_shards ? __hip_atomic_load(col + (int64_t)(i0 + u) * ABD_NOUT, __ATOMIC_RELAXED, __HIP_MEMORY_SCOPE_AGENT) : 0.0;
#pragma unroll
      for (int u = 0; u < 8; ++u) v += q[u];
    }
    sm_chain[cc * ABD_TRAIN_SM + k] = v;
  }
  if (tid == 0) __hip_atomic_store(cnt, 0u, __ATOMIC_RELAXED, __HIP_MEMORY_SCOPE_AGENT);
  __syncthreads();
  return true;
}

template <typename R, int CB, bool GRAD, bool XC, typename ARGS>
__device__ __forceinline__ void dense_body(const ARGS& a) {
  constexpr bool TRAINK = is_train_args<ARGS>::value;
  static_assert(CB * ABD_NOUT <= 64, "the own-sum hand-off needs every partial row of the workgroup stored by wave 0");
  static_assert(!TRAINK || (GRAD && CB <= ABD_TRAIN_CB), "a train launch evaluates gradients for at most ABD_TRAIN_CB chains");
  extern __shared__ __align__(16) unsigned char smem[];
  const int G = a.G, N = a.N;
  const int tstride = G + 1;
  double2_t* tabs = reinterpret_cast<double2_t*>(smem);
  double* red = reinterpret_cast<double*>(tabs + CB * 2 * tstride);
  double* tab_e2 = red + ABD_WAVES_PER_BLOCK * ABD_NOUT;
  double* dict_n = tab_e2 + ABD_EXP2_TAB;
  double* dict_s = dict_n + ABD_XDICT;

  const int tid = threadIdx.x;
  const int lane = tid & 63;
  const int wave = __builtin_amdgcn_readfirstlane(tid >> 6);
  constexpr int NSUB = ABD_WAVES_PER_BLOCK / CB;
  const int c = wave % CB;
  const int sub = wave / CB;
  const int cbase = blockIdx.y * CB;
  int service = 0;
  if constexpr (TRAINK) {
    service = a.service;
    if (service && blockIdx.x == 0) {
      train_service(a, wave, lane);
      return;
    }
  }
  ChainPar p;
  bool chain_on = true;
  if constexpr (TRAINK) {
    const TrainChainArgs& tc = a.tc[c];
    chain_on = tc.action == ABD_TR_STEP;
    p.rw = nullptr;
    p.waner = tc.waner;
    p.iw = tc.iw;
    p.cnt = tc.cnt;
    p.perm_n = p.temp_n = p.rho_n = p.init_n = p.perm_s = p.rho_s = p.init_s = p.b_n = p.d_n = p.b_s = p.d_s = 0.0;
    if (chain_on) {
      abdi::chain_par_from_tr(p, tc.st->pt[tc.use_slot].tr);
    }
  } else {
    p = a.ch[cbase + c];
  }

  ABD_STAMP(0);
  const int nblk = (int)gridDim.x - service;
  const int bid = (int)blockIdx.x - service;
  const int xcd = bid % 8, q8 = nblk / 8, rem8 = nblk % 8;
  const int blk = a.xcd_remap ? xcd * q8 + min(xcd, rem8) + bid / 8 : bid;

  if constexpr (!TRAINK) {
    const int n_fin = blockIdx.y == 0 ? a.prev_n_chains : 0;
    if (blk < n_fin) {
      finalize_chain<ABD_BLOCK>(a.prev_partials + (int64_t)blk * a.prev_blocks * ABD_NOUT, a.prev_blocks,
                     a.prev_out + (int64_t)blk * ABD_NOUT, reinterpret_cast<double*>(smem), tid, a.prev_tag);
      __syncthreads();
    }
  }

  double e2v[ABD_EXP2_TAB / ABD_BLOCK];
#pragma unroll
  for (int q = 0; q < ABD_EXP2_TAB / ABD_BLOCK; ++q) e2v[q] = a.exp2_tab[q * ABD_BLOCK + tid];
  double dv_n = 0.0, dv_s = 0.0;
  if (XC) {
    static_assert(ABD_XDICT == ABD_BLOCK, "one dictionary entry per thread");
    if (tid < a.n_dict_n) dv_n = a.dict_n[tid];
    if (tid < a.n_dict_s) dv_s = a.dict_s[tid];
  }

  auto range_start = [&](int r) { return r * a.rg_base + min(r, a.rg_extra) - a.rg_e_fin * min(r, a.rg_n_short); };
  auto range_of = [&](int r, int& r_lg, int& r_g0, int& r_rows) {
    const int pos = range_start(r);
    r_lg = G > 1 ? (int)__umulhi((uint32_t)pos, a.rg_g_magic) : pos;
    r_g0 = pos - r_lg * G;
    r_rows = range_start(r + 1) - pos;
  };
  int lg, g0, rows_left;
  range_of(blk * NSUB + sub, lg, g0, rows_left);
  if (TRAINK && !chain_on) rows_left = 0;
  int n_entries = rows_left > 0 ? g0 + 1 : 0;
#pragma unroll
  for (int s = 0; s < NSUB; ++s)
    if (NSUB > 1 && s != sub) {
      int o_lg, o_g0, o_rows;
      range_of(blk * NSUB + s, o_lg, o_g0, o_rows);
      n_entries = max(n_entries, o_rows > 0 ? o_g0 + 1 : 0);
    }
  if (TRAINK && !chain_on) n_entries = 0;
  ABD_STAMP(1);
#ifdef ABD_STAMPS
  if (a.stamps && wave == 0 && lane == 0 && blockIdx.y == 0) a.stamps[(int64_t)blockIdx.x * 16 + 9] = (unsigned long long)g0;
#endif

  const uint32_t* vbase = reinterpret_cast<const uint32_t*>(a.vw);
  const uint32_t* ibase = reinterpret_cast<const uint32_t*>(p.iw);
  PieceLoads<R, XC> pl;
  int g1 = min(G, g0 + rows_left);
  int j = lg * 64 + lane;
  uint32_t wi[ABD_SW], wv[ABD_SW];
  const bool first_inside = rows_left > 0 && j < N && g0 > 0;
  RowDesc<XC> rs_n = row_desc<R, XC>(a, 0, lg, g0), rs_s = row_desc<R, XC>(a, 1, lg, g0);
  if (rows_left > 0 && j < N) piece_issue_loads<R, XC>(a, rs_n, rs_s, ibase, vbase, p.waner, lane, j, g0, g1, pl);
  if (first_inside) state_issue_loads(ibase, vbase, 2u * (uint32_t)j, N, g0, wi, wv);
  long long n1 = 0, m1 = 0;
  if (blk == 0 && sub == 0 && chain_on) {
    n1 = p.cnt[0];
    m1 = p.cnt[1];
  }

  if (n_entries > 1) {
    if (NSUB >= 2) {
      if (sub == 0) fill_pow_table_wave(tabs + (c * 2 + 0) * tstride, p.rho_n, n_entries, lane);
      if (sub == 1) fill_pow_table_wave(tabs + (c * 2 + 1) * tstride, p.rho_s, n_entries, lane);
    } else {
      fill_pow_table_wave(tabs + (c * 2 + 0) * tstride, p.rho_n, n_entries, lane);
      fill_pow_table_wave(tabs + (c * 2 + 1) * tstride, p.rho_s, n_entries, lane);
    }
  }
  ABD_STAMP(2);
#pragma unroll
  for (int q = 0; q < ABD_EXP2_TAB / ABD_BLOCK; ++q) tab_e2[q * ABD_BLOCK + tid] = e2v[q];
  if (XC) {
    dict_n[tid] = dv_n;
    dict_s[tid] = dv_s;
  }
  ABD_STAMP(3);

  double acc[16];
#pragma unroll
  for (int k = 0; k < ABD_NACC; ++k) acc[k] = 0.0;

  const DenseChain kc = dense_chain(p);
  const double c2v = to_vgpr(ABD_EXP2_C2);
  const double2_t* tab_n = tabs + (c * 2 + 0) * tstride;
  const double2_t* tab_s = tabs + (c * 2 + 1) * tstride;
  if (NSUB == 1) {
    asm volatile("s_waitcnt lgkmcnt(0)" ::: "memory");
    __builtin_amdgcn_wave_barrier();
  } else {
    __syncthreads();
  }
  ABD_STAMP(4);

  double tn = 0.0, dn = 0.0, ts = 0.0, ds = 0.0;
  uint32_t cfn_hi = 0, cfs_hi = 0;
  ABD_STAMP(5);
  if (first_inside)
    dense_start_state(wi, wv, ibase, vbase, 2u * (uint32_t)j, N, g0, tab_n, tab_s, pl.wj != 0, tn, dn, ts, ds, cfn_hi, cfs_hi);
  if (NSUB == 1) __syncthreads();
  ABD_STAMP(6);

  while (rows_left > 0) {
    rows_left -= g1 - g0;
    if (j < N)
      dense_walk<R, GRAD, XC>(a, kc, rs_n, rs_s, dict_n, dict_s, ibase, vbase, 2u * (uint32_t)j, pl, lane, g0, g1, pl.wj != 0, tn, dn, ts, ds, cfn_hi, cfs_hi, tab_e2, c2v,
                          acc);
    if (rows_left <= 0) break;
    ++lg;
    g0 = 0;
    g1 = min(G, rows_left);
    j = lg * 64 + lane;
    tn = dn = ts = ds = 0.0;
    cfn_hi = cfs_hi = 0;
    rs_n = row_desc<R, XC>(a, 0, lg, g0);
    rs_s = row_desc<R, XC>(a, 1, lg, g0);
    if (j < N) piece_issue_loads<R, XC>(a, rs_n, rs_s, ibase, vbase, p.waner, lane, j, g0, g1, pl);
  }

  ABD_STAMP(7);
  acc[ABD_NACC] = lane == 0 ? (double)n1 : 0.0;
  acc[ABD_NACC + 1] = lane == 0 ? (double)m1 : 0.0;
  acc[ABD_NACC + 2] = 0.0;
  const double tot = wave_reduce16(acc, lane);
  if ((lane & 3) == 0) red[wave * ABD_NOUT + reduce16_index(lane)] = tot;
  __syncthreads();
  bool own_sum = TRAINK;
  if constexpr (!TRAINK) own_sum = a.fin_count != nullptr;
  if (tid < CB * ABD_NOUT) {
    const int cc = tid / ABD_NOUT, k = tid % ABD_NOUT;
    double v = 0.0;
#pragma unroll
    for (int w = 0; w < NSUB; ++w) v += red[(w * CB + cc) * ABD_NOUT + k];
    double* dst = a.partials + ((int64_t)(cbase + cc) * nblk + blk) * ABD_NOUT + k;
    if (own_sum)
      __hip_atomic_store(dst, v, __ATOMIC_RELAXED, __HIP_MEMORY_SCOPE_AGENT);
    else
      *dst = v;
  }
  ABD_STAMP(8);
  if (!own_sum) return;

  int* flag = reinterpret_cast<int*>(red);
  __syncthreads();
  if constexpr (TRAINK) {
    if (nblk <= ABD_TRAIN_ONE_LEVEL) {
      if (wave == 0) {
        handoff_drain_stores();
        if (lane == 0) {
          const unsigned int old = handoff_count_in(a.fin_count);
          flag[0] = old + 1u == (unsigned int)nblk ? 1 : 0;
        }
      }
      __syncthreads();
      const bool last1 = flag[0] != 0;
      __syncthreads();
      if (!last1) return;
      ABD_STAMP(10);
      handoff_acquire();
      double* sm = reinterpret_cast<double*>(smem);
      double* sm_chain1 = sm + ABD_FIN_PARTS * ABD_NOUT;
#pragma unroll
      for (int cc = 0; cc < CB; ++cc) {
        if (a.tc[cc].action == ABD_TR_STEP) {
          sum_chain_coherent<ABD_BLOCK>(a.partials + (int64_t)cc * nblk * ABD_NOUT, nblk, sm, tid);
          if (tid < ABD_NOUT) sm_chain1[cc * ABD_TRAIN_SM + tid] = sm[tid];
          __syncthreads();
        }
      }
      ABD_STAMP(11);
      if (wave < CB && a.tc[wave].action != ABD_TR_SKIP) train_step(a, a.tc[wave], sm_chain1 + wave * ABD_TRAIN_SM, lane);
      ABD_STAMP(12);
      if (tid == 0) __hip_atomic_store(a.fin_count, 0u, __ATOMIC_RELAXED, __HIP_MEMORY_SCOPE_AGENT);
      return;
    }
    unsigned int step_mask = 0;
#pragma unroll
    for (int cc = 0; cc < CB; ++cc) step_mask |= a.tc[cc].action == ABD_TR_STEP ? 1u << cc : 0u;
    double* sm_chain = reinterpret_cast<double*>(smem);
    if (!two_level_sums<CB>(a.partials, a.partials + (int64_t)CB * nblk * ABD_NOUT, a.fin_count, nblk, blk, step_mask, flag, sm_chain, tid)) return;
    if (wave < CB && a.tc[wave].action != ABD_TR_SKIP) train_step(a, a.tc[wave], sm_chain + wave * ABD_TRAIN_SM, lane);
  } else if (a.fin_count != nullptr) {
    if (wave == 0) {
      handoff_drain_stores();
      if (lane < CB) {
        const unsigned int old = handoff_count_in(a.fin_count + cbase + lane);
        flag[lane] = old + 1u == gridDim.x ? 1 : 0;
      }
    }
    __syncthreads();
    bool last[CB];
#pragma unroll
    for (int cc = 0; cc < CB; ++cc) last[cc] = flag[cc] != 0;
    __syncthreads();
#pragma unroll
    for (int cc = 0; cc < CB; ++cc) {
      if (last[cc]) {
        handoff_acquire();
        finalize_chain_coherent<ABD_BLOCK>(a.partials + (int64_t)(cbase + cc) * gridDim.x * ABD_NOUT, (int)gridDim.x,
                                           a.fin_out + (int64_t)(cbase + cc) * ABD_NOUT, reinterpret_cast<double*>(smem), tid, a.fin_tag);
        if (tid == 0) __hip_atomic_store(a.fin_count + cbase + cc, 0u, __ATOMIC_RELAXED, __HIP_MEMORY_SCOPE_AGENT);
        __syncthreads();
      }
    }
  }
}

template <typename R, int CB, bool GRAD, bool XC>
#ifndef ABD_DENSE_MINW
#define ABD_DENSE_MINW 4
#endif
__global__ __launch_bounds__(ABD_BLOCK, ABD_DENSE_MINW) void abd_dense_kernel(const EvalArgs a) {
  dense_body<R, CB, GRAD, XC, EvalArgs>(a);
}

template <typename R, int CB, bool XC>
__global__ __launch_bounds__(ABD_BLOCK, ABD_DENSE_MINW) void abd_train_kernel(const DenseTrainArgs a) {
  dense_body<R, CB, true, XC, DenseTrainArgs>(a);
}
```

abdpymc_amd/csrc/abd_eval.hip:

```cpp
#include "abd_host.hpp"
#include "abd_fuse_plan.hpp"
#include "abd_eval_kernels.hpp"
#include "abd_train.hpp"
#include "abd_readings.hpp"
#include "abd_simulate.hpp"

namespace abdi {

LaunchProfile g_launch_profile;

size_t table_lds_bytes(int G, int cpw, int red_rows, bool exp2_tab = false);
size_t dense_lds_bytes(int G, int cpw) { return abd_dense_lds(G, cpw); }
size_t table_lds_bytes(int G, int cpw, int red_rows, bool exp2_tab) {
  return std::max<size_t>(ABD_FIN_PARTS * ABD_NOUT * sizeof(double),
                          (size_t)(cpw * 2 + 1) * (G + 1) * sizeof(double2_t) + (size_t)red_rows * ABD_NOUT * sizeof(double) +
                              (exp2_tab ? (size_t)ABD_EXP2_TAB * sizeof(double) : 0));
}

enum class Family { Dense, Lanes, Sparse };
using EvalKernel = void (*)(const EvalArgs);
template <typename R, bool GRAD>
EvalKernel eval_kernel(Family f, int cpw, bool xc, bool wide) {
  switch (f) {
    case Family::Dense:
      if (cpw == 4) return xc ? abd_dense_kernel<R, 4, GRAD, true> : abd_dense_kernel<R, 4, GRAD, false>;
      if (cpw == 2) return xc ? abd_dense_kernel<R, 2, GRAD, true> : abd_dense_kernel<R, 2, GRAD, false>;
      return xc ? abd_dense_kernel<R, 1, GRAD, true> : abd_dense_kernel<R, 1, GRAD, false>;
    case Family::Sparse:
      if (cpw == 2) return wide ? abd_sparse_kernel<R, 2, GRAD, ABD_MAXT_MAX> : abd_sparse_kernel<R, 2, GRAD, ABD_MAXT>;
      return wide ? abd_sparse_kernel<R, 1, GRAD, ABD_MAXT_MAX> : abd_sparse_kernel<R, 1, GRAD, ABD_MAXT>;
    default:
      return wide ? abd_obs_kernel<R, GRAD, ABD_MAXT_MAX> : abd_obs_kernel<R, GRAD, ABD_MAXT>;
  }
}

bool dense_xc(const abd_ctx* c, int cpw) { return c->xc_ok && cpw <= c->xc_max_cb; }

int pick_cpw(const abd_ctx* c, int n) {
  const int forced = c->cpw_forced;
  if (forced == 1 || forced == 2 || forced == 4) {
    if (n % forced == 0) return forced;
  }
  if (n % 4 == 0) return 4;
  if (n % 2 == 0) return 2;
  return 1;
}

int dense_blocks(const abd_ctx* c, int cpw, int share, int grid_rows, int steps) {
  const int nsub = ABD_WAVES_PER_BLOCK / cpw;
  const int64_t rows = (int64_t)c->n_lg * c->G;
  const int64_t cap = std::max<int64_t>(1, rows / ((int64_t)kMinRows * nsub));
  const int64_t alone = std::max<int64_t>(c->n_cu, c->dense_blocks / std::max(1, grid_rows));
  const int64_t half = std::max<int64_t>(c->n_cu, c->group_blocks / std::max(1, grid_rows));
  const int64_t want = share == 1 ? std::max<int64_t>(1, c->pipe_blocks / std::max(1, steps)) : (share == 2 ? half : alone);
  return (int)std::max<int64_t>(1, std::min<int64_t>({want, cap, (int64_t)c->blocks_max}));
}

bool partial_rows_fit(const abd_ctx* c, int n_rows, int64_t blocks) { return (int64_t)n_rows * blocks <= (int64_t)c->n_slots * c->blocks_max; }

template <typename ARGS>
void range_split(const abd_ctx* c, int blocks, int nsub, ARGS& a, bool fused_sums = true) {
  const int64_t rows_total = (int64_t)c->n_lg * c->G, n_ranges = (int64_t)blocks * nsub;
  const int64_t n_short = (nsub == 1 && fused_sums) ? std::min<int64_t>(ABD_MAX_BATCH, n_ranges) : 0;
  const int64_t e_fin = (nsub == 1 && (rows_total + n_short * c->fin_rows) / n_ranges >= 2 * c->fin_rows) ? c->fin_rows : 0;
  const int64_t virt = rows_total + n_short * e_fin;
  a.rg_base = (int32_t)(virt / n_ranges);
  a.rg_extra = (int32_t)(virt % n_ranges);
  a.rg_e_fin = (int32_t)e_fin;
  a.rg_n_short = (int32_t)n_short;
  a.rg_g_magic = abd_div_magic((uint32_t)c->G);
}

int flush_pipe(abd_ctx* c, int pi) {
  abd_ctx::Pipe& p = c->pipe[pi];
  if (p.on) {
    const hipError_t le = profiled_launch(true, [&] {
      return launch_kernel(abd_finalize_kernel, dim3(p.n), dim3(ABD_FIN_THREADS), 0, p.st, p.partials[p.buf], p.blocks, p.out, p.tag);
    });
    HIP_TRY(le);
    p.on = false;
  }
  return ABD_OK;
}

int join_pipes(abd_ctx* c) {
  for (int pi = 1; pi < c->n_streams; ++pi) {
    abd_ctx::Pipe& p = c->pipe[pi];
    if (!p.st) continue;
    if (int rc = flush_pipe(c, pi)) return rc;
    if (p.busy) {
      HIP_TRY(hipEventRecord(c->join_ev[pi], p.st));
      HIP_TRY(hipStreamWaitEvent(c->stream, c->join_ev[pi], 0));
      p.busy = false;
    }
  }
  c->next_pipe = 0;
  return ABD_OK;
}

int flush_pending(abd_ctx* c) {
  if (int rc = flush_pipe(c, 0)) return rc;
  return join_pipes(c);
}

int use_pipe(abd_ctx* c, int pi) {
  if (int rc = flush_pipe(c, pi)) return rc;
  if (pi > 0) c->pipe[pi].busy = true;
  return ABD_OK;
}

enum class Sum {
  Pending,
  FinalizeNow,
  Own,
};

struct LaunchPlan {
  Family family;
  int cpw;
  dim3 grid;
  size_t lds;
  int pipe;
  bool rotate;
  bool join;
  Sum sum;
};

LaunchPlan plan_launch(const abd_ctx* c, const Caller& who, int n, int steps) {
  LaunchPlan p;
  p.family = c->dense ? Family::Dense : (c->obs_lanes ? Family::Lanes : Family::Sparse);
  p.cpw = p.family == Family::Lanes ? 1 : pick_cpw(c, n);
  if (p.family == Family::Sparse) p.cpw = std::min(p.cpw, 2);
  const bool own_pipe = who.kind == Caller::Unit || who.kind == Caller::Train;
  p.rotate = who.kind == Caller::Stream && c->n_pipes > 1 && c->dense && c->timing != 1;
  p.join = !own_pipe && !p.rotate;
  p.pipe = own_pipe ? who.pipe : (p.rotate ? c->pipe_order[c->next_pipe] : 0);
  int blocks;
  if (p.family == Family::Dense) {
    const int share = who.kind == Caller::Unit ? 2 : (p.rotate && c->steps_behind != 0 ? 1 : 0);
    blocks = dense_blocks(c, p.cpw, share, steps * n / p.cpw, steps);
    p.lds = abd_dense_lds(c->G, p.cpw, dense_xc(c, p.cpw));
  } else if (p.family == Family::Lanes) {
    blocks = c->ob_n + c->ob_s + c->ob_c;
    p.lds = who.kind == Caller::Train ? abd_obs_lds_own_sum(c->G) : abd_obs_lds_head(c->G);
  } else {
    blocks = c->blocks_x;
    p.lds = table_lds_bytes(c->G, p.cpw, ABD_WAVES_PER_BLOCK * p.cpw);
  }
  p.grid = dim3(blocks, steps * n / p.cpw);
  if (!c->dense)
    p.sum = who.kind == Caller::Train ? Sum::Own : Sum::FinalizeNow;
  else if (who.kind == Caller::Unit)
    p.sum = c->dense_own_sum && blocks <= ABD_TRAIN_ONE_LEVEL ? Sum::Own : Sum::FinalizeNow;
  else
    p.sum = Sum::Pending;
  return p;
}

int enqueue_group(abd_ctx* c, const Caller& who, int n, const int32_t* chains, const HostTerms* host, bool grad, double* rows, int steps) {
  const LaunchPlan p = plan_launch(c, who, n, steps);
  const int n_rows = n * steps;
  if (steps < 1 || n_rows > ABD_MAX_BATCH || (steps > 1 && (p.family != Family::Dense || p.sum != Sum::Pending)))
    return fail(ABD_ERR_STATE, "internal: a launch of %d steps x %d chains", steps, n);
  if (steps > 1 && !partial_rows_fit(c, n_rows, p.grid.x))
    return fail(ABD_ERR_STATE, "internal: a launch of %d rows x %d workgroups exceeds the partial rows", n_rows, (int)p.grid.x);
  if (who.kind == Caller::Train && (n != 1 || p.family != Family::Lanes))
    return fail(ABD_ERR_STATE, "internal: a leapfrog-train launch needs one chain and the observation-lane kernel");
  if ((int)p.grid.x > c->blocks_max) return fail(ABD_ERR_STATE, "internal: grid %d exceeds partial rows %d", (int)p.grid.x, c->blocks_max);
  double& seq = who.seq ? *who.seq : c->seq;
  EvalArgs a;
  base_args(c, a);
  a.n_chains = n_rows;
  for (int k = 0; k < n_rows; ++k) a.ch[k] = chain_par(c, chains[k % n], host[k].tr);
  if (p.family == Family::Dense) range_split(c, (int)p.grid.x, ABD_WAVES_PER_BLOCK / p.cpw, a);
  a.fin_rows = c->fin_rows;
  a.xcd_remap = c->xcd_remap ? 1 : 0;
  if (p.rotate) {
    c->next_pipe = (c->next_pipe + 1) % c->n_pipes;
  } else if (p.join) {
    if (int rc = join_pipes(c)) return rc;
  }
  abd_ctx::Pipe& pp = c->pipe[p.pipe];
  if (p.family == Family::Dense && p.sum != Sum::Own && pp.on && pp.n <= (int)p.grid.x) {
    a.prev_partials = pp.partials[pp.buf];
    a.prev_out = pp.out;
    a.prev_n_chains = pp.n;
    a.prev_blocks = pp.blocks;
    a.prev_tag = pp.tag;
    pp.on = false;
  }
  if (int rc = use_pipe(c, p.pipe)) return rc;
  const int buf = pp.pbuf;
  pp.pbuf ^= 1;
  a.partials = pp.partials[buf];
  if (p.sum == Sum::Own) {
    a.fin_count = c->d_fin_count + (size_t)p.pipe * ABD_MAX_BATCH;
    a.fin_out = rows;
    a.fin_tag = seq + 1.0;
    if (who.train) {
      who.train->tag = seq + 1.0;
      a.train = *who.train;
    }
  }
  const bool stream_ordered = who.kind == Caller::Stream;
  hipEvent_t e1 = nullptr;
  if (c->timing == 1 || (c->timing == 2 && stream_ordered && !c->win_open)) {
    if (c->ev_used == c->ev_pool.size()) {
      Event a0, a1;
      HIP_TRY(a0.create());
      HIP_TRY(a1.create());
      c->ev_pool.emplace_back(std::move(a0), std::move(a1));
    }
    HIP_TRY(hipEventRecord(c->ev_pool[c->ev_used].first, pp.st));
    if (c->timing == 1) e1 = c->ev_pool[c->ev_used++].second;
    if (c->timing == 2) c->win_open = true;
  }
  if (c->timing == 2 && stream_ordered) c->win_launches += steps;
  const bool f32 = c->storage == ABD_STORE_F32, xc = p.family == Family::Dense && dense_xc(c, p.cpw), wide = c->nt > ABD_MAXT;
  const EvalKernel k = f32 ? (grad ? eval_kernel<float, true>(p.family, p.cpw, xc, wide) : eval_kernel<float, false>(p.family, p.cpw, xc, wide))
                           : (grad ? eval_kernel<double, true>(p.family, p.cpw, xc, wide) : eval_kernel<double, false>(p.family, p.cpw, xc, wide));
  const hipError_t le = profiled_launch(false, [&] { return launch_kernel(k, p.grid, dim3(ABD_BLOCK), p.lds, pp.st, a); });
  if (e1) HIP_TRY(hipEventRecord(e1, pp.st));
  HIP_TRY(le);
  seq += 1.0;
  if (p.sum == Sum::Own) return ABD_OK;
  pp.on = true;
  pp.buf = buf;
  pp.n = n_rows;
  pp.blocks = (int)p.grid.x;
  pp.out = rows;
  pp.tag = seq;
  return p.sum == Sum::FinalizeNow ? flush_pipe(c, p.pipe) : ABD_OK;
}

int flush_ring(abd_ctx* c) {
  if (c->win_open) {
    const size_t w = c->ev_used;
    if (c->win_end.size() < (w + 1) * kMaxPipes) {
      const size_t old_n = c->win_end.size();
      c->win_end.resize((w + 1) * kMaxPipes);
      for (size_t k = old_n; k < c->win_end.size(); ++k) HIP_TRY(c->win_end[k].create());
    }
    if (c->win_mask.size() < w + 1) c->win_mask.resize(w + 1, 0u);
    c->win_mask[w] = 0u;
    for (int pi = 0; pi < c->n_streams; ++pi) {
      if (!c->pipe[pi].st || !(pi == 0 || c->pipe[pi].busy || c->pipe[pi].on)) continue;
      if (int prc = flush_pipe(c, pi)) return prc;
      HIP_TRY(hipEventRecord(c->win_end[w * kMaxPipes + pi], c->pipe[pi].st));
      c->win_mask[w] |= 1u << pi;
    }
    c->ev_used++;
    c->win_open = false;
  }
  return flush_pending(c);
}

int wait_rows(abd_ctx* c, int slot, int n, double tag, hipStream_t st) {
  volatile const double* rows = c->out.host() + (size_t)slot * c->n_slots * ABD_NOUT;
  const int first = ((n - 1) / ABD_MAX_BATCH) * ABD_MAX_BATCH;
  int k = n - 1;
  for (int spin = 0; spin < 2000000; ++spin) {
    while (k >= first && rows[(size_t)k * ABD_NOUT + ABD_NOUT - 1] == tag) --k;
    if (k < first) {
      __atomic_thread_fence(__ATOMIC_ACQUIRE);
      return ABD_OK;
    }
    __builtin_ia32_pause();
  }
  __atomic_fetch_add(&c->wait_fallbacks, (int64_t)1, __ATOMIC_RELAXED);
  HIP_TRY(hipStreamSynchronize(st ? st : c->stream));
  for (int q = first; q < n; ++q)
    if (rows[(size_t)q * ABD_NOUT + ABD_NOUT - 1] != tag) return fail(ABD_ERR_STATE, "result row %d of slot %d never received its completion tag", q, slot);
  __atomic_thread_fence(__ATOMIC_ACQUIRE);
  return ABD_OK;
}

int wait_slot(abd_ctx* c, int slot) {
  const ResultSlot& r = c->results[slot];
  volatile const double* rows = c->out.host() + r.row0 * ABD_NOUT;
  const auto t_poll = std::chrono::steady_clock::now();
  int k = r.n - 1;
  for (long spin = 0;; ++spin) {
    while (k >= 0 && rows[(size_t)k * ABD_NOUT + ABD_NOUT - 1] == r.tag_first + (double)(k / ABD_MAX_BATCH)) --k;
    if (k < 0) {
      __atomic_thread_fence(__ATOMIC_ACQUIRE);
      return ABD_OK;
    }
    __builtin_ia32_pause();
    if ((spin & 4095) == 4095 && std::chrono::steady_clock::now() - t_poll > std::chrono::seconds(1)) break;
  }
  __atomic_fetch_add(&c->wait_fallbacks, (int64_t)1, __ATOMIC_RELAXED);
  HIP_TRY(hipStreamSynchronize(c->stream));
  for (int q = 0; q < r.n; ++q)
    if (rows[(size_t)q * ABD_NOUT + ABD_NOUT - 1] != r.tag_first + (double)(q / ABD_MAX_BATCH))
      return fail(ABD_ERR_STATE, "result row %d of stream-ordered slot %d never received its completion tag", q, slot);
  __atomic_thread_fence(__ATOMIC_ACQUIRE);
  return ABD_OK;
}

int enqueue_slot(abd_ctx* c, const Caller& who, int slot, int n, const int32_t* chains, const double* theta, bool grad) {
  if (slot < 0 || slot >= kSyncSlot + c->n_sync_slots) return fail(ABD_ERR_ARG, "result slot %d outside [0, %d)", slot, kResultSlots);
  int rc = check_chains(c, n, chains);
  if (rc) return rc;
  HIP_TRY(hipSetDevice(c->device));
  ResultSlot& r = c->results[slot];
  r.n = n;
  r.grad = grad;
  r.row0 = (size_t)slot * c->n_slots;
  r.chains.assign(chains, chains + n);
  r.theta.assign(theta, theta + (size_t)n * ABD_N_THETA);
  r.host.resize((size_t)n);
  for (int k = 0; k < n; ++k) r.host[(size_t)k] = prepare(theta + (size_t)k * ABD_N_THETA);
  double* rows = c->out.dev() + r.row0 * ABD_NOUT;
  r.tag_first = (who.seq ? *who.seq : c->seq) + 1.0;
  if (who.kind == Caller::Stream) c->pending_slots.push_back(slot);
  for (int k0 = 0; k0 < n; k0 += ABD_MAX_BATCH)
    if ((rc = enqueue_group(c, who, std::min(ABD_MAX_BATCH, n - k0), chains + k0, r.host.data() + k0, grad, rows + (size_t)k0 * ABD_NOUT)))
      return rc;
  return ABD_OK;
}

int enqueue_fused(abd_ctx* c, int slot0, int steps, int n, const int32_t* chains, const double* theta, bool grad) {
  if (slot0 < 0 || steps < 1 || slot0 + steps > kResultSlots || n > c->n_slots || n * steps > ABD_MAX_BATCH)
    return fail(ABD_ERR_STATE, "internal: %d fused steps of %d chains at result slot %d", steps, n, slot0);
  if (int rc = check_chains(c, n, chains)) return rc;
  HIP_TRY(hipSetDevice(c->device));
  const size_t row0 = (size_t)slot0 * c->n_slots;
  HostTerms host[ABD_MAX_BATCH];
  for (int s = 0; s < steps; ++s) {
    ResultSlot& r = c->results[slot0 + s];
    const double* th = theta + (size_t)s * n * ABD_N_THETA;
    r.n = n;
    r.grad = grad;
    r.row0 = row0 + (size_t)s * n;
    r.chains.assign(chains, chains + n);
    r.theta.assign(th, th + (size_t)n * ABD_N_THETA);
    r.host.resize((size_t)n);
    for (int k = 0; k < n; ++k) host[s * n + k] = r.host[(size_t)k] = prepare(th + (size_t)k * ABD_N_THETA);
    r.tag_first = c->seq + 1.0;
    c->pending_slots.push_back(slot0 + s);
  }
  return enqueue_group(c, Caller{Caller::Stream}, n, chains, host, grad, c->out.dev() + row0 * ABD_NOUT, steps);
}

using TrainKernel = void (*)(const DenseTrainArgs);
template <typename R>
TrainKernel train_kernel(int cb, bool xc) {
  if (cb == 4) return xc ? abd_train_kernel<R, 4, true> : abd_train_kernel<R, 4, false>;
  if (cb == 2) return xc ? abd_train_kernel<R, 2, true> : abd_train_kernel<R, 2, false>;
  return xc ? abd_train_kernel<R, 1, true> : abd_train_kernel<R, 1, false>;
}

int enqueue_dense_train(abd_ctx* c, int pi, int cb, int blocks, DenseTrainArgs* a) {
  if (!c->dense) return fail(ABD_ERR_STATE, "internal: dense train launch on a cohort kept as observation lists");
  if (cb != 1 && cb != 2 && cb != 4) return fail(ABD_ERR_STATE, "internal: train unit of %d chains", cb);
  bool any_step = false, any_fwd = false;
  for (int k = 0; k < cb; ++k) {
    TrainChainArgs& tc = a->tc[k];
    if (tc.action != ABD_TR_SKIP || tc.fwd_slot >= 0) {
      if (!tc.st || !tc.ring || !tc.iw || !tc.cnt || !tc.waner || (tc.action == ABD_TR_BEGIN && !tc.begin))
        return fail(ABD_ERR_STATE, "internal: train launch with a NULL pointer for chain %d of the unit", k);
      if ((tc.action == ABD_TR_STEP && (tc.use_slot | 1) != 1) || tc.fwd_slot > 1)
        return fail(ABD_ERR_STATE, "internal: train launch with slot %d / %d for chain %d of the unit", tc.use_slot, tc.fwd_slot, k);
    }
    any_step |= tc.action == ABD_TR_STEP;
    any_fwd |= tc.fwd_slot >= 0;
  }
  for (int k = cb; k < ABD_TRAIN_CB; ++k) {
    std::memset(&a->tc[k], 0, sizeof a->tc[k]);
    a->tc[k].fwd_slot = -1;
  }
  if (!any_step) blocks = 1;
  if (blocks < 1 || blocks > c->blocks_max) return fail(ABD_ERR_STATE, "internal: train grid %d outside [1, %d]", blocks, c->blocks_max);
  const bool xc = c->xc_ok;
  a->yx_n = c->n.yx;
  a->yx_s = c->s.yx;
  a->od_n = c->n.od;
  a->od_s = c->s.od;
  a->xc_n = c->n.xc;
  a->xc_s = c->s.xc;
  a->dict_n = c->n.dict;
  a->dict_s = c->s.dict;
  a->n_dict_n = c->n.n_dict;
  a->n_dict_s = c->s.n_dict;
  a->vw = c->vw;
  a->exp2_tab = c->exp2_tab;
  if (int rc = use_pipe(c, pi)) return rc;
  a->partials = c->pipe[pi].partials[0];
  a->fin_count = c->d_train_count + (size_t)pi * (1 + ABD_TRAIN_SHARDS) * ABD_TRAIN_CNT_STRIDE;
  if ((int64_t)cb * (blocks + ABD_TRAIN_SHARDS) > (int64_t)c->n_slots * c->blocks_max)
    return fail(ABD_ERR_STATE, "internal: train launch of %d x %d workgroups exceeds the partial rows", cb, blocks);
  a->prior_const = c->prior_const;
  a->xcd_remap = c->xcd_remap ? 1 : 0;
  a->service = any_fwd ? 1 : 0;
  if (any_step && blocks > 1 && blocks % c->n_cu == 0) blocks -= 1;
  a->G = c->G;
  a->N = c->N;
  a->n_lg = c->n_lg;
  a->K_n = (int32_t)c->n.K;
  a->K_s = (int32_t)c->s.K;
#ifdef ABD_STAMPS
  a->stamps = stamps_buffer();
#endif
  range_split(c, blocks, ABD_WAVES_PER_BLOCK / cb, *a, false);
  const size_t lds = abd_dense_lds(c->G, cb, xc, true);
  dim3 grid(blocks + a->service, 1);
  const TrainKernel k = c->storage == ABD_STORE_F32 ? train_kernel<float>(cb, xc) : train_kernel<double>(cb, xc);
  const hipError_t le = profiled_launch(false, [&] { return launch_kernel(k, grid, dim3(ABD_BLOCK), lds, c->pipe[pi].st, *a); });
  HIP_TRY(le);
  return ABD_OK;
}

int fetch_slot(abd_ctx* c, int slot, double* logp, double* grad, bool with_priors) {
  if (slot < 0 || slot >= kSyncSlot + c->n_sync_slots) return fail(ABD_ERR_ARG, "result slot %d outside [0, %d)", slot, kResultSlots);
  const ResultSlot& r = c->results[slot];
  if (r.n == 0) return fail(ABD_ERR_STATE, "result slot %d is empty", slot);
  const double* rows = c->out.host() + r.row0 * ABD_NOUT;
  for (int k = 0; k < r.n; ++k)
    assemble(c, r.host[(size_t)k], r.theta.data() + (size_t)k * ABD_N_THETA, rows + (size_t)k * ABD_NOUT, logp + k,
             (grad && r.grad) ? grad + (size_t)k * ABD_N_THETA : nullptr, with_priors);
  return ABD_OK;
}


Readings readings_of(const abd_ctx* c, int chain, const Transformed& tr) {
  Readings w;
  std::memset(&w, 0, sizeof w);
  if (c->dense) {
    w.y_n = c->n.yxi;
    w.y_s = c->s.yxi;
  } else {
    w.y_n = c->n.y;
    w.x_n = c->n.x;
    w.y_s = c->s.y;
    w.x_s = c->s.x;
    w.g_n = c->n.g;
    w.g_s = c->s.g;
    w.j_n = c->n.j;
    w.j_s = c->s.j;
    const int64_t cap = (int64_t)c->n_cu * 8;
    w.bn = (int32_t)std::min<int64_t>((c->n.K + ABD_BLOCK - 1) / ABD_BLOCK, cap);
    w.bs = (int32_t)std::min<int64_t>((c->s.K + ABD_BLOCK - 1) / ABD_BLOCK, cap);
  }
  const ChainSlot& sl = c->slots[(size_t)chain];
  w.vw = c->vw;
  w.iw = sl.iw;
  w.waner = sl.waner;
  constexpr double kLog2E = 1.4426950408889634074;
  w.rho[kAgN] = tr.rho_n;
  w.rho[kAgS] = tr.rho_s;
  w.init[kAgN] = tr.init_n;
  w.init[kAgS] = tr.init_s;
  w.perm[kAgN] = tr.perm_n;
  w.perm[kAgS] = tr.perm_s;
  w.b2[kAgN] = tr.b_n * kLog2E;
  w.b2[kAgS] = tr.b_s * kLog2E;
  w.d[kAgN] = tr.d_n;
  w.d[kAgS] = tr.d_s;
  w.temp_n = tr.temp_n;
  w.K_s = c->s.K;
  w.K_n = c->n.K;
  w.G = c->G;
  w.N = c->N;
  w.nt = c->nt;
  return w;
}

template <typename Op>
int launch_readings(abd_ctx* c, int chain, const Transformed& tr, const Op& op, hipStream_t st) {
  const ReadingArgs<Op> a{readings_of(c, chain, tr), op};
  const bool f32 = c->storage == ABD_STORE_F32, wide = c->nt > ABD_MAXT;
  using Kernel = void (*)(const ReadingArgs<Op>);
  Kernel k;
  int blocks;
  size_t lds;
  if (c->dense) {
    k = f32 ? (wide ? abd_readings_dense_kernel<Op, float, ABD_MAXT_MAX> : abd_readings_dense_kernel<Op, float, ABD_MAXT>)
            : (wide ? abd_readings_dense_kernel<Op, double, ABD_MAXT_MAX> : abd_readings_dense_kernel<Op, double, ABD_MAXT>);
    lds = (size_t)3 * (c->G + 1) * sizeof(double2_t);
    blocks = std::max(1, std::min((c->N + ABD_WAVES_PER_BLOCK - 1) / ABD_WAVES_PER_BLOCK, c->n_cu * 8));
  } else {
    k = f32 ? (wide ? abd_readings_lists_kernel<Op, float, ABD_MAXT_MAX> : abd_readings_lists_kernel<Op, float, ABD_MAXT>)
            : (wide ? abd_readings_lists_kernel<Op, double, ABD_MAXT_MAX> : abd_readings_lists_kernel<Op, double, ABD_MAXT>);
    lds = (size_t)2 * (c->G + 1) * sizeof(double2_t);
    blocks = a.rd.bn + a.rd.bs;
  }
  HIP_TRY(launch_kernel(k, dim3(blocks), dim3(ABD_BLOCK), lds, st, a));
  return ABD_OK;
}

int launch_pointwise(abd_ctx* c, int chain, const double* theta, hipStream_t st, double* ll, double* acc, int64_t n_draw) {
  if (c->s.K + c->n.K == 0 || (!ll && !acc)) return ABD_OK;
  const Transformed tr = transform(theta);
  LogLik op;
  std::memset(&op, 0, sizeof op);
  op.ll = ll;
  op.acc = acc;
  op.n_draw = acc ? n_draw : 0;
  op.inv_n = acc ? 1.0 / (double)n_draw : 0.0;
  op.inv_sig[kAgN] = 1.0 / tr.sig_n;
  op.inv_sig[kAgS] = 1.0 / tr.sig_s;
  op.lnorm[kAgN] = -(theta[13] + 0.5 * kLog2Pi);
  op.lnorm[kAgS] = -(theta[16] + 0.5 * kLog2Pi);
  return launch_readings(c, chain, tr, op, st);
}

int upload_order(abd_ctx* c) {
  if (c->d_order) return ABD_OK;
  const int64_t Ks = c->s.K, Kn = c->n.K;
  if (Ks >= ((int64_t)1 << 32) || Kn >= ((int64_t)1 << 32))
    return fail(ABD_ERR_ARG, "%lld / %lld readings: at most 2^32 - 1 per antigen can be keyed by their index", (long long)Ks, (long long)Kn);
  std::vector<uint32_t> h((size_t)std::max<int64_t>(1, Ks + Kn));
  for (int64_t k = 0; k < Ks; ++k) h[(size_t)k] = (uint32_t)c->order_s[(size_t)k];
  for (int64_t k = 0; k < Kn; ++k) h[(size_t)(Ks + k)] = (uint32_t)c->order_n[(size_t)k];
  DevBuf<uint32_t> d;
  HIP_TRY(d.upload(h.data(), h.size()));
  c->d_order = std::move(d);
  return ABD_OK;
}

int launch_predictive(abd_ctx* c, int chain, const double* theta, hipStream_t st, uint64_t seed, uint32_t stream, uint64_t draw,
                      double* yrep, double* mean, double* acc, int64_t n_draw) {
  if (c->s.K + c->n.K == 0 || (!yrep && !mean && !acc)) return ABD_OK;
  if (!c->d_order) return fail(ABD_ERR_STATE, "internal: the reading order is not on the device (upload_order)");
  const Transformed tr = transform(theta);
  Predictive op;
  std::memset(&op, 0, sizeof op);
  op.ord = c->d_order;
  op.yrep = yrep;
  op.mean = mean;
  op.acc = acc;
  op.n_draw = acc ? n_draw : 0;
  op.inv_n = acc ? 1.0 / (double)n_draw : 0.0;
  op.sig[kAgN] = tr.sig_n;
  op.sig[kAgS] = tr.sig_s;
  op.inv_sig[kAgN] = 1.0 / tr.sig_n;
  op.inv_sig[kAgS] = 1.0 / tr.sig_s;
  op.seed_lo = (uint32_t)seed;
  op.seed_hi = (uint32_t)(seed >> 32);
  op.stream = stream;
  op.draw_lo = (uint32_t)draw;
  const uint32_t draw_hi = (uint32_t)(draw >> 32) & 0x3FFFFFFFu;
  op.c3[kAgS] = 0x80000000u | (0u << 30) | draw_hi;
  op.c3[kAgN] = 0x80000000u | (1u << 30) | draw_hi;
  return launch_readings(c, chain, tr, op, st);
}

template <typename F>
int readings_sync(abd_ctx* c, int32_t chain, int rows, std::vector<double>& h, F&& launch) {
  if (int rc = check_chains(c, 1, &chain)) return rc;
  HIP_TRY(hipSetDevice(c->device));
  if (int rc = flush_ring(c)) return rc;
  const size_t Kt = (size_t)(c->s.K + c->n.K);
  if (Kt == 0 || rows == 0) return ABD_OK;
  if (!c->d_stage || c->stage_rows < rows) {
    HIP_TRY(c->d_stage.alloc((size_t)rows * Kt));
    c->stage_rows = rows;
  }
  if (int rc = launch(c->d_stage)) return rc;
  h.resize((size_t)rows * Kt);
// ... 349 lines not shown
```

abdpymc_amd/csrc/abd_gibbs.hip:

```cpp
#include "abd_host.hpp"
#include "abd_gibbs_lists.hpp"
#include "abd_gibbs_dense.hpp"

namespace abdi {

using GibbsKernel = void (*)(const GibbsArgs);
template <typename R>
GibbsKernel gibbs_kernel(const abd_ctx* c, bool stats) {
  const bool wide = c->nt > ABD_MAXT;
  if (c->dense && stats) return wide ? abd_gibbs_dense_kernel<R, true, ABD_MAXT_MAX> : abd_gibbs_dense_kernel<R, true, ABD_MAXT>;
  if (c->dense) return wide ? abd_gibbs_dense_kernel<R, false, ABD_MAXT_MAX> : abd_gibbs_dense_kernel<R, false, ABD_MAXT>;
  if (c->nt == 1) return abd_gibbs_kernel<R, 1>;
  return wide ? abd_gibbs_kernel<R, ABD_MAXT_MAX> : abd_gibbs_kernel<R, ABD_MAXT>;
}

int enqueue_gibbs(abd_ctx* c, int m, const int32_t* chains, const double* theta, uint64_t seed, uint32_t sweep,
                         uint32_t stream_offset, hipStream_t st, unsigned long long* counts_dev, unsigned int* work_dev,
                         unsigned long long* stats_dev) {
  GibbsArgs ga;
  base_args(c, ga.e);
  ga.e.n_chains = m;
  ga.seed_lo = (uint32_t)seed;
  ga.seed_hi = (uint32_t)(seed >> 32);
  ga.sweep = sweep;
  ga.ind_offset = c->ind_offset;
  ga.counts = counts_dev;
  for (int k = 0; k < m; ++k) {
    const double* t = theta + (size_t)k * ABD_N_THETA;
    ga.e.ch[k] = chain_par(c, chains[k], t);
    const Transformed tr = transform(t);
    ga.stream[k] = (uint32_t)chains[k] + stream_offset;
    ga.theta0[k] = t[0];
    ga.theta7[k] = t[7];
    ga.is2_n[k] = 1.0 / (tr.sig_n * tr.sig_n);
    ga.is2_s[k] = 1.0 / (tr.sig_s * tr.sig_s);
  }
  HIP_TRY(hipMemsetAsync(counts_dev, 0, (size_t)m * 2 * sizeof(unsigned long long), st));
  ga.work = work_dev;
  ga.refill_min = c->g2_refill_min;
  ga.tail_lanes = c->g2_tail_lanes;
  ga.tail_age = c->g2_tail_age;
  ga.stats = stats_dev;
  if (stats_dev) HIP_TRY(hipMemsetAsync(stats_dev, 0, 8 * sizeof(unsigned long long), st));
  dim3 grid, block(ABD_BLOCK);
  size_t lds;
  if (c->dense) {
    const int rbytes = c->storage == ABD_STORE_F32 ? 4 : 8;
    int nw2 = abd_g2_waves(c->G, rbytes);
    if (m == 1) nw2 = std::max(ABD_G2_MIN_WAVES, std::min(nw2, tune_int("ABD_G2_WAVES_ONE", 8)));
    lds = abd_g2_lds(c->G, rbytes, nw2);
    HIP_TRY(hipMemsetAsync(work_dev, 0, (size_t)m * sizeof(unsigned int), st));
    grid = dim3(std::max(1, std::min(c->n_cu / m, (c->N + nw2 - 1) / nw2)), m);
    block = dim3(64 * nw2);
  } else {
    grid = dim3(std::max(1, std::min((c->N + ABD_WAVES_PER_BLOCK - 1) / ABD_WAVES_PER_BLOCK, c->n_cu * 8)), m);
    lds = abd_gibbs_lds(c->G);
  }
  const bool stats = stats_dev != nullptr;
  const GibbsKernel k = c->storage == ABD_STORE_F32 ? gibbs_kernel<float>(c, stats) : gibbs_kernel<double>(c, stats);
  HIP_TRY(launch_kernel(k, grid, block, lds, st, ga));
  return ABD_OK;
}

}

extern "C" {

int abd_gibbs_sweep(abd_ctx* c, int32_t n, const int32_t* chains, const double* theta, uint64_t seed, uint32_t sweep,
                    int64_t* accepted, int64_t* proposed) {
  if (!c || !chains || !theta) return fail(ABD_ERR_ARG, "NULL argument");
  int rc = check_chains(c, n, chains);
  if (rc) return rc;
  for (int a = 0; a < n; ++a)
    for (int b = a + 1; b < n; ++b)
      if (chains[a] == chains[b]) return fail(ABD_ERR_ARG, "chain %d listed twice: a sweep updates its state in place", chains[a]);
  HIP_TRY(hipSetDevice(c->device));
  if (int frc = flush_ring(c)) return frc;
  std::vector<unsigned long long> counts((size_t)n * 2, 0);
  static const bool want_stats = env_int("ABD_GIBBS_STATS", 0) != 0;
  for (int k0 = 0; k0 < n; k0 += ABD_MAX_BATCH) {
    const int m = std::min(ABD_MAX_BATCH, n - k0);
    unsigned long long* stats_dev = want_stats ? c->d_counts + (size_t)c->n_slots * 2 : nullptr;
    rc = enqueue_gibbs(c, m, chains + k0, theta + (size_t)k0 * ABD_N_THETA, seed, sweep, 0u, c->stream, c->d_counts,
                       c->d_work, stats_dev);
    if (rc) return rc;
    HIP_TRY(hipMemcpyAsync(counts.data() + (size_t)k0 * 2, c->d_counts, (size_t)m * 2 * sizeof(unsigned long long),
                           hipMemcpyDeviceToHost, c->stream));
    HIP_TRY(hipStreamSynchronize(c->stream));
    if (stats_dev) {
      unsigned long long st[8];
      HIP_TRY(hipMemcpy(st, stats_dev, sizeof st, hipMemcpyDeviceToHost));
      const double ni = (double)std::max<unsigned long long>(1, st[0]);
      std::fprintf(stderr, "[abd gibbs stats] individuals x chains %llu; per individual: iterations %.1f, refills %.1f, walk steps %.1f "
                   "(lanes busy %.1f of 64), tail finishes %.1f, commit scans %.1f, acceptances %.2f\n",
                   st[0], st[1] / ni, st[2] / ni, st[3] / ni, st[3] ? (double)st[4] / (double)st[3] : 0.0, st[5] / ni, st[6] / ni, st[7] / ni);
    }
  }
  for (int k = 0; k < n; ++k) {
    if (accepted) accepted[k] = (int64_t)counts[(size_t)k * 2];
    if (proposed) proposed[k] = (int64_t)counts[(size_t)k * 2 + 1];
  }
  return ABD_OK;
}

}
```

abdpymc_amd/csrc/abd_host.hpp:

```cpp
#pragma once

#include <algorithm>
#include <atomic>
#include <chrono>
#include <cmath>
#include <cstdarg>
#include <cstdio>
#include <cstdlib>
#include <cstring>
#include <limits>
#include <mutex>
#include <new>
#include <string>
#include <thread>
#include <vector>

#include "../../include/abd_hip.h"
#include "abd_types.hpp"
#include "abd_owned.hpp"
#include "abd_terms.hpp"

static_assert(ABD_MAX_BATCH == ABD_MAX_BATCH_K, "header / kernel batch size mismatch");
static_assert(ABD_MAX_GAPS == 64 * ABD_MAXT_MAX, "header / kernel gap limit mismatch");
static_assert(ABD_N_THETA == ABD_NT, "header / kernel value-variable count mismatch");

namespace abdi {

int fail(int code, const char* fmt, ...);
const char* last_error();
void set_error(const std::string& msg);

#define HIP_TRY(expr)                                                                              \
  do {                                                                                             \
    hipError_t e_ = (expr);                                                                        \
    if (e_ != hipSuccess) return fail(ABD_ERR_HIP, "%s: %s", #expr, hipGetErrorString(e_));        \
  } while (0)

inline int env_int(const char* name, int dflt) {
  const char* e = std::getenv(name);
  return e ? std::atoi(e) : dflt;
}
inline int tune_int(const char* name, int dflt) {
#ifdef ABD_TUNING
  return env_int(name, dflt);
#else
  (void)name;
  return dflt;
#endif
}

constexpr int kResultSlots = 1024;
constexpr int kSyncSlot = kResultSlots;
constexpr int kMaxPipes = 8;
constexpr int kMinRows = 4;
constexpr int64_t kSimStageBytes = (int64_t)1 << 30;

struct LaunchProfile {
  bool on = false;
  double eval_s = 0.0, sum_s = 0.0;
  long evals = 0, sums = 0;
};
extern LaunchProfile g_launch_profile;

template <typename K, typename... A>
hipError_t launch_kernel(K kernel, dim3 grid, dim3 block, size_t lds, hipStream_t st, const A&... args) {
  if (lds > 64 * 1024)
    if (hipError_t e = hipFuncSetAttribute(reinterpret_cast<const void*>(kernel), hipFuncAttributeMaxDynamicSharedMemorySize, (int)lds))
      return e;
  hipLaunchKernelGGL(kernel, grid, block, lds, st, args...);
  return hipGetLastError();
}

template <typename F>
hipError_t profiled_launch(bool sum, F&& launch) {
  if (!g_launch_profile.on) return launch();
  const auto t0 = std::chrono::steady_clock::now();
  const hipError_t e = launch();
  const double s = std::chrono::duration<double>(std::chrono::steady_clock::now() - t0).count();
  if (sum) {
    g_launch_profile.sum_s += s;
    g_launch_profile.sums++;
  } else {
    g_launch_profile.eval_s += s;
    g_launch_profile.evals++;
  }
  return e;
}

struct Caller {
  enum Kind {
    Stream,
    Sync,
    Unit,
    Train,
  } kind;
  int pipe = 0;
  double* seq = nullptr;
  TrainArgs* train = nullptr;
};

struct AntigenDev {
  int64_t K = 0;
  DevBuf<unsigned char> y;
  DevBuf<unsigned char> x;
  DevBuf<uint16_t> g;
  DevBuf<int32_t> ptr;
  DevBuf<int32_t> j;
  DevBuf<unsigned char> yx;
  DevBuf<unsigned char> yxi;
  DevBuf<unsigned char> od;
  DevBuf<uint8_t> xc;
  DevBuf<double> dict;
  int n_dict = 0;
};

struct ChainSlot {
  DevBuf<uint64_t> rw;
  DevBuf<int8_t> waner;
  DevBuf<uint64_t> iw;
  DevBuf<long long> cnt;
  bool set = false;
};

struct ResultSlot {
  int n = 0;
  bool grad = true;
  size_t row0 = 0;
  std::vector<int32_t> chains;
  std::vector<double> theta;
  std::vector<HostTerms> host;
  double tag_first = 0.0;
};

}

using namespace abdi;

struct abd_ctx {
  int device = 0;
  int G = 0, N = 0, nt = 0, n_chunks = 1;
  int storage = ABD_STORE_F64;
  bool dense = false;
  bool xc_ok = false;
  int xc_max_cb = 1;
  bool ignore_pcr = false;
  int n_slots = 0;
  int n_cu = 256;
  int n_lg = 0;
  int blocks_x = 0;
  int ob_n = 0, ob_s = 0, ob_c = 0;
  bool obs_lanes = true;
  int blocks_max = 0;
  int cpw_forced = 0;
  int dense_blocks = 0;
  uint64_t chunk_mask[3][ABD_MAXT_MAX] = {};
  int splits[2] = {0, 0};
  ~abd_ctx();
  struct Pipe {
    Stream st;
    DevBuf<double> partials[2];
    int pbuf = 0;
    bool on = false;
    int buf = 0, n = 0, blocks = 0;
    double* out = nullptr;
    double tag = 0.0;
    bool busy = false;
  } pipe[kMaxPipes];
  hipStream_t stream = nullptr;
  Event join_ev[kMaxPipes];
  std::vector<std::pair<Event, Event>> ev_pool;
  std::vector<Event> win_end;
  std::vector<uint32_t> win_mask;
  AntigenDev s, n;
  std::vector<int64_t> order_s, order_n;
  DevBuf<uint64_t> vw;
  DevBuf<uint64_t> pw;
  DevBuf<double> exp2_tab;
  DevBuf<int8_t> stage_gn;
  std::vector<ChainSlot> slots;
  int n_pipes = 4;
  int n_streams = kMaxPipes;
  int n_sync_slots = 4;
  int pipe_blocks = 0;
  int group_blocks = 0;
  int dbpc = 4;
  int next_pipe = 0;
  double seq = 0.0;
  bool dense_own_sum = true;
  DevBuf<unsigned int> d_fin_count;
  DevBuf<unsigned int> d_train_count;
  uint32_t ind_offset = 0;
  bool xcd_remap = true;
  int fin_rows = 2;
  int steps_behind = -1;
  double prior_const = 0.0;
  MappedBuf<double> out;
  std::vector<int> pending_slots;
  DevBuf<unsigned long long> d_counts;
  DevBuf<unsigned int> d_work;
  DevBuf<unsigned long long> d_counts_chain;
  MappedBuf<unsigned long long> h_counts_chain;
  int g2_refill_min = ABD_G2_REFILL_MIN, g2_tail_lanes = ABD_G2_TAIL_LANES, g2_tail_age = ABD_G2_TAIL_AGE;
  DevBuf<double> d_stage;
  int stage_rows = 0;
  DevBuf<uint32_t> d_order;
  DevBuf<double> d_det;
  DevBuf<int32_t> d_last;
  DevBuf<unsigned long long> d_curves;
  DevBuf<unsigned long long> d_risk;
  std::vector<ResultSlot> results;
  int timing = 0;
  bool win_open = false;
  int64_t win_launches = 0;
  size_t ev_used = 0;
  double ev_total_ms = 0.0;
  int64_t ev_count = 0;
  int queue_of_pipe[kMaxPipes] = {};
  int n_queues = 0;
  int pipe_order[kMaxPipes] = {0, 1, 2, 3, 4, 5, 6, 7};
  std::vector<double> unit_seq;
  int64_t wait_fallbacks = 0;
  char name[256] = {0};
};

namespace abdi {

ModelSizes model_sizes(const abd_ctx* c);
void assemble(const abd_ctx* c, const HostTerms& h, const double* t, const double* sums, double* logp, double* grad, bool with_priors = true);
ChainPar chain_par(const abd_ctx* c, int chain, const Transformed& tr);
ChainPar chain_par(const abd_ctx* c, int chain, const double* t);
void base_args(const abd_ctx* c, EvalArgs& a);
#ifdef ABD_STAMPS
unsigned long long* stamps_buffer();
#endif
int probe_stream_queues(abd_ctx* c);
inline int unit_pipe(const abd_ctx* c, int u) { return c->pipe_order[u % c->n_streams]; }
int check_chains(abd_ctx* c, int n, const int32_t* chains);
int launch_deterministics(abd_ctx* c, int chain, const double* theta, hipStream_t st, int8_t* out_i, double* out_mun, double* out_mus, double* sums);
int launch_curves(abd_ctx* c, int chain, const double* theta, double thr_s, double thr_n, hipStream_t st, unsigned long long* scratch,
                  unsigned long long* row);
size_t curves_row_cols(const abd_ctx* c);
size_t curves_scratch_cols(const abd_ctx* c);
void split_curves_row(const abd_ctx* c, const unsigned long long* row, int64_t* counts, int64_t* n_infections, double* titer_sums);
int check_risk_spec(const abd_ctx* c, const abd_risk_spec* spec);
int launch_risk(abd_ctx* c, int chain, const double* theta, const abd_risk_spec& spec, hipStream_t st, unsigned long long* scratch,
                uint32_t* table);
size_t risk_table_cols(const abd_ctx* c);
size_t risk_scratch_cols(const abd_ctx* c);
int launch_diag(abd_ctx* c, int chain, const double* theta, hipStream_t st, int64_t d, int64_t H, int64_t L, double* tit, uint32_t* inf,
                unsigned long long* cb2);
int launch_diag_export(abd_ctx* c, const void* src, int stride, int width, unsigned long long* dst, hipStream_t st);
int launch_timeline(abd_ctx* c, int chain, const double* theta, const double range_n[2], const double range_s[2], hipStream_t st,
                    uint32_t* hist_n, uint32_t* hist_s, uint32_t* cell, uint32_t* ninf);
int launch_timeline_hist_export(abd_ctx* c, const uint32_t* src, int g0, int n_g, void* dst, hipStream_t st);
int launch_timeline_quantiles(abd_ctx* c, const uint32_t* hist, int64_t chain_stride, int n_chains, const double range[2], int n_q,
                              const double* q, double* out, hipStream_t st);
int launch_unpack(abd_ctx* c, int chain, int8_t* dst, hipStream_t st);

size_t dense_lds_bytes(int G, int cpw);
int flush_pipe(abd_ctx* c, int pi);
int join_pipes(abd_ctx* c);
int flush_pending(abd_ctx* c);
int flush_ring(abd_ctx* c);
int wait_rows(abd_ctx* c, int slot, int n, double tag, hipStream_t st = nullptr);
int enqueue_slot(abd_ctx* c, const Caller& who, int slot, int n, const int32_t* chains, const double* theta, bool grad);
int enqueue_group(abd_ctx* c, const Caller& who, int n, const int32_t* chains, const HostTerms* host, bool grad, double* rows, int steps = 1);
int fetch_slot(abd_ctx* c, int slot, double* logp, double* grad, bool with_priors = true);
int enqueue_dense_train(abd_ctx* c, int pi, int cb, int blocks, DenseTrainArgs* a);
int dense_blocks(const abd_ctx* c, int cpw, int share = 0, int grid_rows = 1, int steps = 1);

int launch_pointwise(abd_ctx* c, int chain, const double* theta, hipStream_t st, double* ll, double* acc, int64_t n_draw);
int upload_order(abd_ctx* c);
int launch_predictive(abd_ctx* c, int chain, const double* theta, hipStream_t st, uint64_t seed, uint32_t stream, uint64_t draw,
                      double* yrep, double* mean, double* acc, int64_t n_draw);
struct ReadingOut {
  double* s;
  double* n;
};
template <int R, typename At>
void scatter_readings(const abd_ctx* c, const ReadingOut (&out)[R], At at) {
  const size_t Ks = (size_t)c->s.K, Kn = (size_t)c->n.K;
  for (size_t k = 0; k < Ks; ++k) {
    const size_t o = (size_t)c->order_s[k];
    for (int v = 0; v < R; ++v)
      if (out[v].s) out[v].s[o] = at(v, k);
  }
  for (size_t k = 0; k < Kn; ++k) {
    const size_t o = (size_t)c->order_n[k];
    for (int v = 0; v < R; ++v)
      if (out[v].n) out[v].n[o] = at(v, Ks + k);
  }
}

int enqueue_gibbs(abd_ctx* c, int m, const int32_t* chains, const double* theta, uint64_t seed, uint32_t sweep,
                  uint32_t stream_offset, hipStream_t st, unsigned long long* counts_dev, unsigned int* work_dev,
                  unsigned long long* stats_dev);

}
```

abdpymc_amd/csrc/abd_sampler.hip:

```cpp
#include "abd_host.hpp"
#include "abd_nuts.hpp"

#include <deque>
#include <memory>

struct abd_sampler {
  ~abd_sampler();
  abd_ctx* c = nullptr;
  int n = 0;
  abd_sampler_opts o{};
  std::vector<int32_t> chains;
  std::vector<abdnuts::AdaptiveNuts> ch;
  int64_t it = 0;
  int64_t n_accumulated = 0;
  int64_t rec_chunk = 0;
  bool ran = false;
  std::vector<double> lp, gr;
  int unit = 1;
  int threads = 1;
  bool trains = false;
  bool unit_tags = false;
  int lookahead = 8;
  static constexpr int kTrainRing = 32;
  struct TrainUnit {
// ... 679 lines not shown
  abd_ctx* c = s->c;
  const int64_t n_iter = f.n_iter;
  const int n = s->n, B = s->unit;
  const int n_units = (n + B - 1) / B;
  enum { NEED_BEGIN, TREE, SWEEP, DONE };
  struct Step {
    int64_t idx;
    uint32_t epoch;
    bool eval0;
  };
  struct Run {
    int state = DONE;
    int64_t k = 0;
    uint32_t epoch = 0;
    int parity = 0;
    int steps_queued = 0, max_steps = 0;
    bool eval_first = false, eval_only = false;
    int begin_block = 0;
    int pend_slot = -1;
    int64_t pend_idx = 0;
    std::deque<Step> fifo;
  };
  std::vector<Run> runs((size_t)n);
  static const bool profile = env_int("ABD_SAMPLER_PROFILE", 0) != 0;
  g_launch_profile = LaunchProfile();
  g_launch_profile.on = profile;
  long n_launches = 0, n_records = 0, n_stale = 0;

  auto stage_begin = [&](int j, bool eval_first, bool eval_only) {
    Run& r = runs[(size_t)j];
    abd_sampler::DChain& d = s->dc[(size_t)j];
    const abdnuts::Nuts& nu = s->ch[(size_t)j].nuts;
    r.begin_block = (int)(d.n_begin++ % abd_sampler::kBeginBlocks);
    TrainBegin& b = d.begin.host()[r.begin_block];
    std::memcpy(b.q0, nu.q, sizeof b.q0);
    std::memcpy(b.p0, nu.p0_pending, sizeof b.p0);
    std::memcpy(b.g0, nu.g, sizeof b.g0);
    std::memcpy(b.inv_mass, nu.inv_mass, sizeof b.inv_mass);
    b.eps = nu.eps;
    b.dirs = nu.dir_bits;
    b.max_depth = eval_only ? 0 : nu.max_depth;
    b.eval_first = eval_first ? 1 : 0;
    __atomic_thread_fence(__ATOMIC_RELEASE);
    r.eval_first = eval_first;
    r.eval_only = eval_only;
    r.state = NEED_BEGIN;
  };
  auto iteration_done = [&](int j, bool with_counts) -> int {
    Run& r = runs[(size_t)j];
    abd_sampler::DChain& d = s->dc[(size_t)j];
    write_draw(f, j, r.k, with_counts ? d.done.host() : nullptr);
    if (int rc = queue_draw(f, j, r.k, d.side)) return rc;
    if (++r.k == n_iter) r.state = DONE;
    return ABD_OK;
  };
  auto transition_end = [&](int j) -> int {
    Run& r = runs[(size_t)j];
    abd_sampler::DChain& d = s->dc[(size_t)j];
    r.epoch += 1;
    s->ch[(size_t)j].end_transition();
    if (s->o.gibbs) {
      const int32_t id = s->chains[(size_t)j];
      if (int rc = queue_sweep(s, j, 1, &id, s->ch[(size_t)j].nuts.q, r.k, d.side)) return rc;
      d.sweep_tag += 1.0;
      hipLaunchKernelGGL(abd_sweep_done_kernel, dim3(1), dim3(64), 0, d.side, c->d_counts_chain + 2 * (size_t)j, d.done.dev(),
                         reinterpret_cast<double*>(d.done.dev() + 2), d.sweep_tag);
      HIP_TRY(hipGetLastError());
      r.state = SWEEP;
      return ABD_OK;
    }
    if (int rc = iteration_done(j, false)) return rc;
    if (r.state != DONE) {
      s->ch[(size_t)j].begin();
      stage_begin(j, false, false);
    }
    return ABD_OK;
  };

  for (int j = 0; j < n && n_iter > 0; ++j) {
    s->ch[(size_t)j].begin();
    stage_begin(j, false, false);
  }

  int rc_loop = ABD_OK;
  for (long spins = 0; rc_loop == ABD_OK;) {
    bool any = false, progressed = false;
    for (int u = 0; u < n_units && rc_loop == ABD_OK; ++u) {
      const int lo = u * B, hi = std::min(n, lo + B);
      for (int j = lo; j < hi && rc_loop == ABD_OK; ++j) {
        Run& r = runs[(size_t)j];
        abd_sampler::DChain& d = s->dc[(size_t)j];
        abdnuts::Nuts& nu = s->ch[(size_t)j].nuts;
        while (!r.fifo.empty() && rc_loop == ABD_OK) {
          const Step e = r.fifo.front();
          if (e.epoch != r.epoch) {
            r.fifo.pop_front();
            ++n_stale;
            continue;
          }
          const TrainRecord& tr = d.ring.host()[e.idx % ABD_TRAIN_RING];
          if (*(volatile const double*)&tr.tag != (double)(e.idx + 1)) break;
          __atomic_thread_fence(__ATOMIC_ACQUIRE);
          r.fifo.pop_front();
          progressed = true;
          ++n_records;
          if (e.eval0) {
            nu.set_point(tr.lp, tr.g);
            if ((rc_loop = iteration_done(j, true)) != ABD_OK) break;
            if (r.state == DONE) break;
            nu.begin_finish();
            nu.adopt_request(tr.next_theta, tr.next_p_half);
          } else {
            nu.feed(tr.lp, tr.g, tr.next_theta, tr.next_p_half, true);
            if (!nu.active) rc_loop = transition_end(j);
          }
        }
      }
      if (rc_loop != ABD_OK) break;
      for (int j = lo; j < hi; ++j) {
        Run& r = runs[(size_t)j];
        if (r.state != SWEEP) continue;
        const abd_sampler::DChain& dj = s->dc[(size_t)j];
        if (*reinterpret_cast<volatile const double*>(dj.done.host() + 2) != dj.sweep_tag) continue;
        __atomic_thread_fence(__ATOMIC_ACQUIRE);
        progressed = true;
        const bool last = r.k + 1 == n_iter;
        if (!last) s->ch[(size_t)j].begin_draw();
        stage_begin(j, true, last);
      }
      if (rc_loop != ABD_OK) break;
      for (;;) {
        size_t out = 0;
        bool any_begin = false, any_step = false;
        for (int j = lo; j < hi; ++j) {
          const Run& r = runs[(size_t)j];
          out = std::max(out, r.fifo.size());
          any_begin |= r.state == NEED_BEGIN;
          any_step |= r.state == TREE && r.steps_queued < r.max_steps;
        }
        if (!any_begin && !(any_step && out < (size_t)s->dtrain_lookahead)) break;
        const bool step_now = out < (size_t)s->dtrain_lookahead;
        DenseTrainArgs a;
        std::memset(&a, 0, sizeof a);
        for (int k = 0; k < ABD_TRAIN_CB; ++k) a.tc[k].fwd_slot = -1;
        for (int j = lo; j < hi; ++j) {
          Run& r = runs[(size_t)j];
          abd_sampler::DChain& d = s->dc[(size_t)j];
          const ChainSlot& slot = c->slots[(size_t)s->chains[(size_t)j]];
          TrainChainArgs& tc = a.tc[j - lo];
          tc.st = d.st;
          tc.ring = d.ring.dev();
          tc.begin = d.begin.dev();
          tc.iw = slot.iw;
          tc.cnt = slot.cnt;
          tc.waner = slot.waner;
          tc.action = ABD_TR_SKIP;
          tc.fwd_slot = -1;
          if (r.state == NEED_BEGIN) {
            tc.action = ABD_TR_BEGIN;
            tc.begin = d.begin.dev() + r.begin_block;
            r.state = TREE;
            r.parity = 0;
            r.steps_queued = 0;
            r.max_steps = (r.eval_first ? 1 : 0) + (r.eval_only ? 0 : s->ch[(size_t)j].nuts.max_leaves());
            r.pend_slot = -1;
          } else if (r.state == TREE && r.steps_queued < r.max_steps && step_now) {
            tc.action = ABD_TR_STEP;
            tc.use_slot = r.parity;
            tc.rec_idx = d.n_rec++;
            tc.own = r.steps_queued + 1 == r.max_steps ? 1 : 0;
            if (r.pend_slot >= 0) {
              tc.fwd_slot = r.pend_slot;
              tc.fwd_idx = r.pend_idx;
            }
            r.pend_slot = tc.own ? -1 : (r.parity ^ 1);
            r.pend_idx = tc.rec_idx;
            r.fifo.push_back(Step{tc.rec_idx, r.epoch, r.eval_first && r.steps_queued == 0});
            r.parity ^= 1;
            r.steps_queued += 1;
          } else if (r.pend_slot >= 0) {
            tc.fwd_slot = r.pend_slot;
            tc.fwd_idx = r.pend_idx;
            r.pend_slot = -1;
          }
        }
        if ((rc_loop = enqueue_dense_train(c, unit_pipe(c, u), B, s->dtrain_blocks, &a)) != ABD_OK) break;
        ++n_launches;
        progressed = true;
      }
      for (int j = lo; j < hi; ++j) any |= runs[(size_t)j].state != DONE;
    }
    if (rc_loop != ABD_OK || !any) break;
    if (progressed) {
      spins = 0;
    } else if (++spins > 40000000) {
      __atomic_fetch_add(&c->wait_fallbacks, (int64_t)1, __ATOMIC_RELAXED);
      (void)hipDeviceSynchronize();
      rc_loop = fail(ABD_ERR_STATE, "the native sampler's leapfrog trains stalled: a record never received its tag");
    } else {
      __builtin_ia32_pause();
    }
  }
  for (int u = 0; u < n_units; ++u) (void)hipStreamSynchronize(c->pipe[unit_pipe(c, u)].st);
  for (int j = 0; j < n; ++j) (void)hipStreamSynchronize(s->dc[(size_t)j].side);
  g_launch_profile.on = false;
  if (rc_loop != ABD_OK) return rc_loop;
  if (profile) {
    const double wall = std::chrono::duration<double>(std::chrono::steady_clock::now() - f.t_begin).count();
    std::fprintf(stderr, "abd sampler (trains): %d units of %d chains, %ld launches, %ld records (%ld stale steps) in %.3f s; %.2f us inside the "
                 "launch call per launch\n", n_units, B, n_launches, n_records, n_stale, wall,
                 g_launch_profile.evals ? 1e6 * g_launch_profile.eval_s / g_launch_profile.evals : 0.0);
  }
  return ABD_OK;
}

}

int abd_sampler_run_record(abd_sampler* s, int64_t n_iter, double* theta, double* stats, const abd_record* rec) {
  if (!s) return fail(ABD_ERR_ARG, "sampler is NULL");
  if (n_iter < 0) return fail(ABD_ERR_ARG, "n_iter=%lld is negative", (long long)n_iter);
  abd_ctx* c = s->c;
  const int n = s->n;
  if (s->d_curves && s->it + n_iter - s->o.tune > s->curves_capacity)
    return fail(ABD_ERR_STATE, "curves: draws up to %lld do not fit capacity %lld", (long long)(s->it + n_iter - s->o.tune),
                (long long)s->curves_capacity);
  if (s->d_diag_tit && s->it + n_iter - s->o.tune > s->diag_draws)
    return fail(ABD_ERR_STATE, "diagnostics: draws up to %lld pass the planned %lld", (long long)(s->it + n_iter - s->o.tune),
                (long long)s->diag_draws);
  if (s->d_risk && s->it + n_iter - s->o.tune > s->risk_capacity)
    return fail(ABD_ERR_STATE, "risk: draws up to %lld do not fit capacity %lld", (long long)(s->it + n_iter - s->o.tune),
                (long long)s->risk_capacity);
  if (s->d_tl_hist && s->it + n_iter - s->o.tune > s->tl_draws)
    return fail(ABD_ERR_STATE, "timelines: draws up to %lld pass the planned %lld", (long long)(s->it + n_iter - s->o.tune),
                (long long)s->tl_draws);
  const bool with_ll = rec && (rec->ll_s || rec->ll_n);
  const bool with_yrep = rec && (rec->yrep_s || rec->yrep_n);
  const bool recording = rec && (rec->i_raw || rec->ab_s_waner || rec->i || rec->ab_n_mu || rec->ab_s_mu || with_ll || with_yrep);
  const size_t Kt = (size_t)(c->s.K + c->n.K);
  s->ran = true;
  if (recording) {
    if (rec->thin < 0) return fail(ABD_ERR_ARG, "record: thin=%lld is negative", (long long)rec->thin);
    const int64_t thin = std::max<int64_t>(1, rec->thin), n_rec = (n_iter + thin - 1) / thin;
    if (rec->first < 0 || rec->first + n_rec > rec->capacity)
      return fail(ABD_ERR_ARG, "record: draws [%lld, %lld) do not fit capacity %lld", (long long)rec->first,
                  (long long)(rec->first + n_rec), (long long)rec->capacity);
    if (!s->d_rec_mu) {
      HIP_TRY(hipSetDevice(c->device));
      const size_t cells = (size_t)c->G * c->N;
      const size_t per_draw = (size_t)n * (cells * 18 + c->N + (with_ll ? Kt * sizeof(double) : 0) +
                                           (with_yrep ? Kt * sizeof(double) : 0));
      s->rec_chunk = std::max<int64_t>(1, std::min<int64_t>(256, (int64_t)(((size_t)256 << 20) / per_draw)));
      DevBuf<double> mu;
      DevBuf<int8_t> i8;
      HIP_TRY(mu.alloc((size_t)2 * n * s->rec_chunk * cells));
      HIP_TRY(i8.alloc((size_t)2 * n * s->rec_chunk * cells + (size_t)n * s->rec_chunk * c->N));
      s->d_rec_mu = std::move(mu);
      s->d_rec_i8 = std::move(i8);
    }
    HIP_TRY(hipSetDevice(c->device));
    if (with_ll)
      if (int rc = alloc_rec_rows(s, s->d_rec_ll, "pointwise log-likelihood")) return rc;
    if (with_yrep) {
      if (int rc = upload_order(c)) return rc;
      if (int rc = alloc_rec_rows(s, s->d_rec_yrep, "posterior predictive")) return rc;
    }
  }
  RunFrame f{s, n_iter, theta, stats, recording ? rec : nullptr, recording ? std::max<int64_t>(1, rec->thin) : 1, {}, {}};
  f.staging.resize((size_t)n);
  for (auto& sg : f.staging) sg.flushed_to = recording ? rec->first : 0;
  HIP_TRY(hipSetDevice(c->device));
  if (int rc = flush_ring(c)) return rc;
  HIP_TRY(hipStreamSynchronize(c->stream));
  f.t_begin = std::chrono::steady_clock::now();
  if (int rc = s->dtrains ? sampler_run_trains(f) : sampler_run_units(f)) return rc;
  for (int pi = 1; pi < c->n_streams; ++pi) c->pipe[pi].busy = true;
  if (int rc = join_pipes(c)) return rc;
  const int64_t first_draw = std::max<int64_t>(s->it, s->o.tune);
  if (s->d_sums && s->it + n_iter > first_draw) s->n_accumulated += s->it + n_iter - first_draw;
  s->it += n_iter;
  return ABD_OK;
}

int abd_sampler_means(abd_sampler* s, int32_t k, double* i_mean, double* mu_n_mean, double* mu_s_mean, int64_t* n_draws) {
  if (!s) return fail(ABD_ERR_ARG, "sampler is NULL");
  if (k < 0 || k >= s->n) return fail(ABD_ERR_ARG, "k=%d outside [0, %d)", k, s->n);
  if (!s->d_sums) return fail(ABD_ERR_STATE, "the sampler was created without accumulate");
  abd_ctx* c = s->c;
  HIP_TRY(hipSetDevice(c->device));
  HIP_TRY(hipStreamSynchronize(c->stream));
  const size_t cells = (size_t)c->G * c->N;
  double* outs[3] = {i_mean, mu_n_mean, mu_s_mean};
  const double inv = s->n_accumulated ? 1.0 / (double)s->n_accumulated : 0.0;
  for (int v = 0; v < 3; ++v) {
    if (!outs[v]) continue;
    HIP_TRY(hipMemcpy(outs[v], s->d_sums + ((size_t)k * 3 + v) * cells, cells * sizeof(double), hipMemcpyDeviceToHost));
    for (size_t e = 0; e < cells; ++e) outs[v][e] *= inv;
  }
  if (n_draws) *n_draws = s->n_accumulated;
  return ABD_OK;
}

int abd_sampler_enable_pointwise(abd_sampler* s, int32_t accumulate) {
  if (!s) return fail(ABD_ERR_ARG, "sampler is NULL");
  return enable_acc(s, s->d_pw_acc, 4, accumulate, false, "pointwise");
}

// ... 349 lines not shown
```

abdpymc_amd/csrc/abd_small.hpp:

```cpp
#pragma once

#include "abd_device.hpp"

__global__ void abd_spin_kernel(unsigned long long* out, unsigned long long ticks) {
  const unsigned long long t0 = __builtin_amdgcn_s_memrealtime();
  unsigned long long t = t0;
  while (t - t0 < ticks) {
    __builtin_amdgcn_s_sleep(16);
    t = __builtin_amdgcn_s_memrealtime();
  }
  if (threadIdx.x == 0) {
    out[0] = t0;
    out[1] = t;
  }
}

__global__ __launch_bounds__(256) void abd_pack_bits_kernel(const int8_t* __restrict__ src, uint64_t* __restrict__ dst,
                                                            int G, int N, int nt) {
  const int j = blockIdx.x * blockDim.x + threadIdx.x;
  const int t = blockIdx.y;
  if (j >= N || t >= nt) return;
  uint64_t w = 0;
  const int g_end = min(64, G - t * 64);
  for (int b = 0; b < g_end; ++b) w |= (uint64_t)(src[(int64_t)(t * 64 + b) * N + j] != 0) << b;
  dst[(int64_t)t * N + j] = w;
}

struct ConstrainArgs {
  const uint64_t* pw;
  int32_t N, nt, n_chunks, pad_;
  uint64_t chunk_mask[3][ABD_MAXT_MAX];
};

template <int MT>
__global__ __launch_bounds__(256) void abd_constrain_kernel(const ConstrainArgs a, const uint64_t* __restrict__ rw,
                                                            const int8_t* __restrict__ waner, uint64_t* __restrict__ iw,
                                                            unsigned long long* cnt) {
  const int j = blockIdx.x * blockDim.x + threadIdx.x;
  int n1 = 0, m1 = 0;
  if (j < a.N) {
    uint64_t P[MT], Rw[MT], I[MT];
#pragma unroll
    for (int t = 0; t < MT; ++t) {
      P[t] = Rw[t] = 0;
      if (t < a.nt) {
        Rw[t] = rw[(int64_t)t * a.N + j];
        if (a.pw) P[t] = a.pw[(int64_t)t * a.N + j];
        n1 += __builtin_popcountll(Rw[t]);
      }
    }
    constrain_masks<MT>(Rw, P, a, I);
#pragma unroll
    for (int t = 0; t < MT; ++t)
      if (t < a.nt) iw[(int64_t)t * a.N + j] = I[t];
    m1 = waner[j] != 0;
  }
#pragma unroll
  for (int off = 32; off > 0; off >>= 1) {
    n1 += __shfl_xor(n1, off, 64);
    m1 += __shfl_xor(m1, off, 64);
  }
  if ((threadIdx.x & 63) == 0 && (n1 | m1)) {
    atomicAdd(cnt + 0, (unsigned long long)n1);
    atomicAdd(cnt + 1, (unsigned long long)m1);
  }
}

template <int MT>
__global__ void abd_flip_kernel(const ConstrainArgs a, uint64_t* rw, int8_t* waner, uint64_t* iw, unsigned long long* cnt, int G,
                                int64_t flat) {
  const int N = a.N;
  const int64_t gn = (int64_t)G * N;
  if (flat < gn) {
    const int64_t g = flat / N, j = flat % N;
    const uint64_t bit = 1ull << (g & 63);
    const uint64_t w = rw[(g >> 6) * N + j] ^ bit;
    rw[(g >> 6) * N + j] = w;
    cnt[0] += (w & bit) ? 1ull : ~0ull;
    uint64_t P[MT], Rw[MT], I[MT];
#pragma unroll
    for (int t = 0; t < MT; ++t) {
      P[t] = Rw[t] = 0;
      if (t < a.nt) {
        Rw[t] = rw[(int64_t)t * N + j];
        if (a.pw) P[t] = a.pw[(int64_t)t * N + j];
      }
    }
    constrain_masks<MT>(Rw, P, a, I);
#pragma unroll
    for (int t = 0; t < MT; ++t)
      if (t < a.nt) iw[(int64_t)t * N + j] = I[t];
  } else {
    const int8_t w = waner[flat - gn] ^ 1;
    waner[flat - gn] = w;
    cnt[1] += w ? 1ull : ~0ull;
  }
}

template <int MT>
__global__ __launch_bounds__(ABD_BLOCK) void abd_deterministics_kernel(const EvalArgs a, int8_t* __restrict__ out_i,
                                                                       double* __restrict__ out_mun,
                                                                       double* __restrict__ out_mus,
                                                                       double* __restrict__ sums) {
  extern __shared__ __align__(16) unsigned char smem[];
  double2_t* tabs = reinterpret_cast<double2_t*>(smem);
  const int G = a.G, N = a.N, nt = a.nt, tstride = G + 1;
  double2_t* tab_ones = tabs + 2 * tstride;
  const int tid = threadIdx.x, lane = tid & 63;
  const int wave = __builtin_amdgcn_readfirstlane(tid >> 6);
  const ChainPar& p = a.ch[0];
  fill_pow_table(tabs, p.rho_n, tstride, tid, ABD_BLOCK);
  fill_pow_table(tabs + tstride, p.rho_s, tstride, tid, ABD_BLOCK);
  fill_ones_table(tab_ones, tstride, tid, ABD_BLOCK);
  __syncthreads();
  const int waves_total = gridDim.x * ABD_WAVES_PER_BLOCK;
  for (int j = blockIdx.x * ABD_WAVES_PER_BLOCK + wave; j < N; j += waves_total) {
    uint64_t V[MT], I[MT];
#pragma unroll
    for (int t = 0; t < MT; ++t) {
      V[t] = I[t] = 0;
      if (t < nt) {
        V[t] = uniform_word(a.vw, (int64_t)t * N + j);
        I[t] = uniform_word(p.iw, (int64_t)t * N + j);
      }
    }
    const bool wj = __builtin_amdgcn_readfirstlane((int)p.waner[j]) != 0;
    const double2_t* ts = wj ? tabs + tstride : tab_ones;
    for (int t = 0; t < nt; ++t) {
      const int g = t * 64 + lane;
      if (g < G) {
        const Resp rs = responses<MT>(g, t + 1, I, V, tabs, ts);
        const int64_t o = (int64_t)g * N + j;
        const int bit = (int)((I[t] >> lane) & 1ull);
        const double mun = p.init_n + (rs.cum_i ? p.perm_n : 0.0) + p.temp_n * rs.un;
        const double mus = p.init_s + (rs.cum_iv ? p.perm_s : 0.0) + rs.us;
        if (out_i) out_i[o] = (int8_t)bit;
        if (out_mun) out_mun[o] = mun;
        if (out_mus) out_mus[o] = mus;
        if (sums) {
          const int64_t cells = (int64_t)G * N;
          sums[o] += (double)bit;
          sums[cells + o] += mun;
          sums[2 * cells + o] += mus;
        }
      }
    }
  }
}


__global__ __launch_bounds__(256) void abd_unpack_bits_kernel(const uint64_t* __restrict__ src, int8_t* __restrict__ dst,
                                                              int G, int N) {
  const int j = blockIdx.x * blockDim.x + threadIdx.x;
  const int g = blockIdx.y;
  if (j < N && g < G) dst[(int64_t)g * N + j] = (int8_t)((src[(int64_t)(g >> 6) * N + j] >> (g & 63)) & 1ull);
}
```

abdpymc_amd/csrc/abd_terms.hpp:

```cpp
#pragma once

#include <cmath>

#include "../../include/abd_hip.h"
#include "abd_types.hpp"

#define ABD_HD __host__ __device__ __forceinline__

namespace abdi {

constexpr double kLog2Pi = 1.8378770664093453;

struct Transformed {
  double p, perm_n, temp_n, rho_n, init_n, perm_s, rho_s, q, tinf, tvac, init_s;
  double b_n, d_n, sig_n, b_s, d_s, sig_s;
};
static_assert(sizeof(Transformed) == ABD_N_THETA * sizeof(double), "Transformed is indexed like theta (abd_dense.hpp: train epilogue)");

struct HostTerms {
  Transformed tr;
  double L0[4], L1[4];
};

struct ModelSizes {
  int32_t G, dense;
  double N, cells, Kn, Ks, prior_const;
};

ABD_HD double sigmoid(double t) { return 1.0 / (1.0 + exp(-t)); }
ABD_HD double softplus(double t) { return fmax(t, 0.0) + log1p(exp(-fabs(t))); }

ABD_HD double transform_one(int k, double t) {
  switch (k) {
    case 0: case 3: case 6: case 7: return sigmoid(t);
    case 1: case 2: case 5: case 8: case 9: case 13: case 16: return exp(t);
    case 11: case 14: return t == 0.0 ? 1e-300 : t;
    default: return t;
  }
}

ABD_HD Transformed transform(const double* t) {
  Transformed c;
  double* v = &c.p;
  for (int k = 0; k < ABD_N_THETA; ++k) v[k] = transform_one(k, t[k]);
  return c;
}

ABD_HD HostTerms prepare(const double* t) {
  HostTerms h;
  h.tr = transform(t);
  const int k4[4] = {0, 3, 6, 7};
  for (int q = 0; q < 4; ++q) {
    h.L0[q] = -softplus(-t[k4[q]]);
    h.L1[q] = -softplus(t[k4[q]]);
  }
  return h;
}

ABD_HD double priors(const HostTerms& h, const double* t, int G, double cells, double n1, double N, double m1,
                            double* g , double prior_const) {
  double lp = prior_const;
  if (g)
    for (int k = 0; k < ABD_N_THETA; ++k) g[k] = 0.0;
  {
    const double L0 = h.L0[0], L1 = h.L1[0], p = h.tr.p;
    const double bm1 = (double)(G - 1) - 1.0;
    lp += (bm1 == 0.0 ? 0.0 : bm1 * L1) + L0 + L1 + n1 * L0 + (cells - n1) * L1;
    if (g) g[0] = (1.0 + n1) * (1.0 - p) - p * (bm1 + 1.0 + (cells - n1));
  }
  const int gk[5] = {1, 2, 5, 8, 9};
  const double gmu[5] = {2.0, 1.0, 2.0, 1.0, 1.0};
  const double gx[5] = {h.tr.perm_n, h.tr.temp_n, h.tr.perm_s, h.tr.tinf, h.tr.tvac};
  for (int q = 0; q < 5; ++q) {
    const double al = gmu[q] * gmu[q] / (0.5 * 0.5), be = gmu[q] / (0.5 * 0.5);
    const double x = gx[q];
    lp += al * t[gk[q]] - be * x;
    if (g) g[gk[q]] = al - be * x;
  }
  for (int w = 0; w < 2; ++w) {
    const int k = w == 0 ? 3 : 6;
    const double L0 = h.L0[w + 1], L1 = h.L1[w + 1], r = w == 0 ? h.tr.rho_n : h.tr.rho_s;
    lp += 9.0 * L0 + L0 + L1;
    if (g) g[k] = 10.0 * (1.0 - r) - r;
  }
  {
    const double L0 = h.L0[3], L1 = h.L1[3], q = h.tr.q;
    lp += L0 + L1 + m1 * L0 + (N - m1) * L1;
    if (g) g[7] = (1.0 + m1) * (1.0 - q) - q * (1.0 + (N - m1));
  }
  const int nk[6] = {4, 10, 11, 12, 14, 15};
  const double nmu[6] = {-2.0, -2.0, -1.0, 2.0, -1.0, 2.0};
  const double nsd[6] = {1.0, 1.0, 0.5, 0.5, 0.5, 0.5};
  for (int q = 0; q < 6; ++q) {
    const double z = (t[nk[q]] - nmu[q]) / nsd[q];
    lp += -0.5 * z * z;
    if (g) g[nk[q]] = -z / nsd[q];
  }
  for (int w = 0; w < 2; ++w) {
    const int k = w == 0 ? 13 : 16;
    const double x = w == 0 ? h.tr.sig_n : h.tr.sig_s;
    lp += -x + t[k];
    if (g) g[k] = -x + 1.0;
  }
  return lp;
}

ABD_HD void assemble_terms(const ModelSizes& m, const HostTerms& h, const double* t, const double* sums, double* logp,
                                  double* grad, bool with_priors) {
  const Transformed& tr = h.tr;
  const double n1 = sums[ABD_NACC], m1 = sums[ABD_NACC + 1];
  double lp = 0.0;
  if (with_priors)
    lp = priors(h, t, m.G, m.cells, n1, m.N, m1, grad, m.prior_const);
  else if (grad)
    for (int k = 0; k < ABD_N_THETA; ++k) grad[k] = 0.0;
  const double is2_n = 1.0 / (tr.sig_n * tr.sig_n), is2_s = 1.0 / (tr.sig_s * tr.sig_s);
  lp += -0.5 * is2_n * sums[A_N_Q2] - m.Kn * (t[13] + 0.5 * kLog2Pi);
  lp += -0.5 * is2_s * sums[A_S_Q2] - m.Ks * (t[16] + 0.5 * kLog2Pi);
  *logp = lp;
  if (grad) {
    const double fn = -tr.b_n * tr.d_n * is2_n, fs = -tr.b_s * tr.d_s * is2_s;
    grad[1] += fn * tr.perm_n * sums[A_N_HC];
    grad[2] += fn * tr.temp_n * sums[A_N_HU];
    grad[3] += fn * tr.temp_n * tr.rho_n * (1.0 - tr.rho_n) * sums[A_N_HD];
    grad[4] += fn * sums[A_N_H];
    const double kC = 1.4426950408889634074 * ABD_EXP2_TAB;
    const double hx_n = m.dense ? sums[A_N_HX] / (kC * tr.b_n) : sums[A_N_HX];
    const double hx_s = m.dense ? sums[A_S_HX] / (kC * tr.b_s) : sums[A_S_HX];
    grad[11] += -tr.d_n * is2_n * hx_n;
    grad[12] += is2_n * sums[A_N_QS];
    grad[13] += is2_n * sums[A_N_Q2] - m.Kn;
    grad[5] += fs * tr.perm_s * sums[A_S_HC];
    grad[6] += fs * tr.rho_s * (1.0 - tr.rho_s) * sums[A_S_HD];
    grad[10] += fs * sums[A_S_H];
    grad[14] += -tr.d_s * is2_s * hx_s;
    grad[15] += is2_s * sums[A_S_QS];
    grad[16] += is2_s * sums[A_S_Q2] - m.Ks;
  }
}

ABD_HD void chain_par_from_tr(ChainPar& p, const double* tr) {
  p.perm_n = tr[1];
  p.temp_n = tr[2];
  p.rho_n = tr[3];
  p.init_n = tr[4];
  p.perm_s = tr[5];
  p.rho_s = tr[6];
  p.init_s = tr[10];
  p.b_n = tr[11];
  p.d_n = tr[12];
  p.b_s = tr[14];
  p.d_s = tr[15];
}
static_assert(sizeof(ChainPar) == 11 * sizeof(double) + 4 * sizeof(void*), "ChainPar changed: review chain_par_from_tr (11 constants) and chain_par (4 pointers)");


ABD_HD void transform_lane(int k, double t, double& tr, double& l0, double& l1) {
  tr = transform_one(k, t);
  const double L = log1p(exp(-fabs(t)));
  l0 = -(fmax(-t, 0.0) + L);
  l1 = -(fmax(t, 0.0) + L);
}

ABD_HD void assemble_lane(int k, const ModelSizes& m, const Transformed& tr, double tk, double xk, double l0, double l1,
                          const double* sums, double& lp_k, double& g_k) {
  const double n1 = sums[ABD_NACC], m1 = sums[ABD_NACC + 1];
  const double is2_n = 1.0 / (tr.sig_n * tr.sig_n), is2_s = 1.0 / (tr.sig_s * tr.sig_s);
  const double fn = -tr.b_n * tr.d_n * is2_n, fs = -tr.b_s * tr.d_s * is2_s;
  const double kC = 1.4426950408889634074 * ABD_EXP2_TAB;
  double lp = 0.0, g = 0.0;
  switch (k) {
    case 0: {
      const double bm1 = (double)(m.G - 1) - 1.0;
      lp = m.prior_const + (bm1 == 0.0 ? 0.0 : bm1 * l1) + l0 + l1 + n1 * l0 + (m.cells - n1) * l1;
      g = (1.0 + n1) * (1.0 - xk) - xk * (bm1 + 1.0 + (m.cells - n1));
      break;
    }
    case 1: case 2: case 5: case 8: case 9: {
      const double mu = (k == 1 || k == 5) ? 2.0 : 1.0;
      const double al = mu * mu / (0.5 * 0.5), be = mu / (0.5 * 0.5);
      lp = al * tk - be * xk;
      g = al - be * xk;
      if (k == 1) g += fn * xk * sums[A_N_HC];
      if (k == 2) g += fn * xk * sums[A_N_HU];
      if (k == 5) g += fs * xk * sums[A_S_HC];
      break;
    }
    case 3: case 6: {
      const double r = xk;
      lp = 9.0 * l0 + l0 + l1;
      g = 10.0 * (1.0 - r) - r;
      g += k == 3 ? fn * tr.temp_n * r * (1.0 - r) * sums[A_N_HD] : fs * r * (1.0 - r) * sums[A_S_HD];
      break;
    }
    case 7:
      lp = l0 + l1 + m1 * l0 + (m.N - m1) * l1;
      g = (1.0 + m1) * (1.0 - xk) - xk * (1.0 + (m.N - m1));
      break;
    case 4: case 10: case 11: case 12: case 14: case 15: {
      const double mu = (k == 4 || k == 10) ? -2.0 : (k == 11 || k == 14) ? -1.0 : 2.0;
      const double sd = (k == 4 || k == 10) ? 1.0 : 0.5;
      const double z = (tk - mu) / sd;
      lp = -0.5 * z * z;
      g = -z / sd;
      if (k == 4) g += fn * sums[A_N_H];
      if (k == 10) g += fs * sums[A_S_H];
      if (k == 11) g += -tr.d_n * is2_n * (m.dense ? sums[A_N_HX] / (kC * tr.b_n) : sums[A_N_HX]);
      if (k == 14) g += -tr.d_s * is2_s * (m.dense ? sums[A_S_HX] / (kC * tr.b_s) : sums[A_S_HX]);
      if (k == 12) g += is2_n * sums[A_N_QS];
      if (k == 15) g += is2_s * sums[A_S_QS];
      break;
    }
    default: {
      const bool nn = k == 13;
      const double x = xk, is2 = nn ? is2_n : is2_s, q2 = nn ? sums[A_N_Q2] : sums[A_S_Q2], K = nn ? m.Kn : m.Ks;
      lp = (-x + tk) + (-0.5 * is2 * q2 - K * (tk + 0.5 * kLog2Pi));
      g = (-x + 1.0) + (is2 * q2 - K);
      break;
    }
  }
  lp_k = lp;
  g_k = g;
}

}
```

abdpymc_amd/csrc/abd_types.hpp:

```cpp
#pragma once

#if defined(__HIPCC__)
#include <hip/hip_runtime.h>
#else
#define __host__
#define __device__
#define __forceinline__ inline
#endif
#include <stddef.h>
#include <stdint.h>

#define ABD_MAXT 4
#define ABD_MAXT_MAX 8
#define ABD_NACC 13
#define ABD_NOUT 16
#define ABD_MAX_BATCH_K 16
#define ABD_WAVES_PER_BLOCK 4
#define ABD_BLOCK (64 * ABD_WAVES_PER_BLOCK)

enum {
  A_N_Q2 = 0,
  A_N_H,
  A_N_HC,
  A_N_HU,
  A_N_HD,
  A_N_HX,
  A_N_QS,
  A_S_Q2,
  A_S_H,
  A_S_HC,
  A_S_HD,
  A_S_HX,
  A_S_QS,
};

struct ChainPar {
  double perm_n, temp_n, rho_n, init_n;
  double perm_s, rho_s, init_s;
  double b_n, d_n;
  double b_s, d_s;
  const uint64_t* rw;
  const int8_t* waner;
  const uint64_t* iw;
  const long long* cnt;
};

#define ABD_NT 17
struct TrainPoint {
  double theta[ABD_NT];
  double p_half[ABD_NT];
  double tr[ABD_NT];
  double L0[4], L1[4];
  double prev_lp, prev_g[ABD_NT];
};
struct TrainRecord {
  double lp;
  double g[ABD_NT];
  double next_theta[ABD_NT], next_p_half[ABD_NT];
  double tag;
};
struct TrainArgs {
  TrainPoint* slots;
  TrainRecord* rec;
  double tag;
  double ve;
  double prior_const;
  int32_t enabled;
  int32_t use_slot;
  int32_t next_slot;
  int32_t own_record;
  int32_t pad_[2];
  TrainRecord* fwd_rec;
  double fwd_tag;
  double inv_mass[ABD_NT];
  TrainPoint first;
};

#define ABD_TRAIN_CB 4
#define ABD_TRAIN_RING 64
#define ABD_TRAIN_SHARDS 32
#define ABD_TRAIN_ONE_LEVEL 256
#define ABD_TRAIN_CNT_STRIDE 32
enum { ABD_TR_SKIP = 0, ABD_TR_STEP = 1, ABD_TR_BEGIN = 2 };
enum { ABD_PH_IDLE = 0, ABD_PH_EVAL0 = 1, ABD_PH_LEAF = 2 };
struct TrainEnd {
  double q[ABD_NT], p[ABD_NT], g[ABD_NT];
};
struct TrainBegin {
  double q0[ABD_NT], p0[ABD_NT], g0[ABD_NT];
  double inv_mass[ABD_NT];
  double eps;
  uint32_t dirs;
  int32_t max_depth;
  int32_t eval_first;
  int32_t pad_;
};
struct TrainChain {
  TrainPoint pt[2];
  TrainEnd end[2];
  double inv_mass[ABD_NT];
  double eps;
  uint32_t dirs;
  int32_t max_depth;
  int32_t phase, depth, n_leaf, n_target, dir;
  int32_t pad_;
};
struct TrainChainArgs {
  TrainChain* st;
  TrainRecord* ring;
  const TrainBegin* begin;
  const uint64_t* iw;
  const long long* cnt;
  const int8_t* waner;
  int32_t action;
  int32_t use_slot;
  int32_t own;
  int32_t fwd_slot;
  int64_t rec_idx;
  int64_t fwd_idx;
};
struct DenseTrainArgs {
  const void* yx_n;
  const void* yx_s;
  const void* od_n;
  const void* od_s;
  const uint8_t* xc_n;
  const uint8_t* xc_s;
  const double* dict_n;
  const double* dict_s;
  const uint64_t* vw;
  const double* exp2_tab;
  double* partials;
  unsigned int* fin_count;
#ifdef ABD_STAMPS
  unsigned long long* stamps;
#endif
  double prior_const;
  int32_t n_dict_n, n_dict_s;
  int32_t rg_base, rg_extra, rg_e_fin, rg_n_short;
  uint32_t rg_g_magic;
  int32_t xcd_remap;
  int32_t service;
  int32_t G, N, n_lg, K_n, K_s;
  TrainChainArgs tc[ABD_TRAIN_CB];
};

struct EvalArgs {
  const void* y_n;
  const void* x_n;
  const void* y_s;
  const void* x_s;
  const uint16_t* g_n;
  const uint16_t* g_s;
  const int32_t* ptr_n;
  const int32_t* ptr_s;
  const int32_t* j_n;
  const int32_t* j_s;
  int32_t K_n, K_s;
  int32_t ob_n, ob_s, ob_c;
  int32_t pad3_;
  const void* yx_n;
  const void* yx_s;
  const void* yxi_n;
  const void* yxi_s;
  const void* od_n;
  const void* od_s;
  const uint8_t* xc_n;
  const uint8_t* xc_s;
  const double* dict_n;
  const double* dict_s;
  int32_t n_dict_n, n_dict_s;
  const uint64_t* vw;
  const uint64_t* pw;
#ifdef ABD_STAMPS
  unsigned long long* stamps;
#endif
  int32_t rg_base, rg_extra, rg_e_fin, rg_n_short;
  uint32_t rg_g_magic;
  const double* exp2_tab;
  double* partials;
  const double* prev_partials;
  double* prev_out;
  int32_t prev_n_chains, prev_blocks;
  int32_t fin_rows;
  int32_t xcd_remap;
  double prev_tag;
  unsigned int* fin_count;
  double* fin_out;
  double fin_tag;
  int32_t G, N, nt, n_chunks;
  int32_t n_chains, n_lg;
  uint64_t chunk_mask[3][ABD_MAXT_MAX];
  ChainPar ch[ABD_MAX_BATCH_K];
  TrainArgs train;
};

__host__ __device__ inline uint32_t abd_div_magic(uint32_t G) { return G > 1 ? (uint32_t)((((uint64_t)1 << 32) + G - 1) / G) : 0u; }
__host__ __device__ inline uint32_t abd_div_by_magic(uint32_t row, uint32_t magic) { return (uint32_t)(((uint64_t)row * magic) >> 32); }
__host__ __device__ inline bool abd_div_magic_exact(uint64_t n_rows, uint32_t G) {
  if (G <= 1) return n_rows < ((uint64_t)1 << 31);
  const uint64_t e = (uint64_t)abd_div_magic(G) * G - ((uint64_t)1 << 32);
  return n_rows < ((uint64_t)1 << 31) && n_rows * e < ((uint64_t)1 << 32);
}

struct double2_t {
  double x, y;
};

template <typename R>
struct YX {
  R y, x;
};


#define ABD_EXP2_TAB 1024
#define ABD_EXP2_K_MIN (-1022 * 1024)
#define ABD_EXP2_K_MAX (510 * 1024 + 1023)
__host__ __device__ inline uint64_t abd_exp2_prebias(uint64_t bits_of_2_to_j_1024, int j) {
  const uint32_t hi = (uint32_t)(bits_of_2_to_j_1024 >> 32) - ((uint32_t)j << 10);
  return ((uint64_t)hi << 32) | (bits_of_2_to_j_1024 & 0xFFFFFFFFull);
}
__host__ __device__ inline int abd_exp2_clamp(int k) { return k < ABD_EXP2_K_MIN ? ABD_EXP2_K_MIN : k > ABD_EXP2_K_MAX ? ABD_EXP2_K_MAX : k; }
__host__ __device__ inline uint32_t abd_exp2_scaled_hi(uint32_t entry_hi, int kc) { return entry_hi + ((uint32_t)kc << 10); }
#define ABD_XDICT 256

struct Philox4 {
  uint32_t w[4];
};

__host__ __device__ __forceinline__ Philox4 philox4x32_10(uint32_t c0, uint32_t c1, uint32_t c2, uint32_t c3, uint32_t k0,
                                                          uint32_t k1) {
#pragma unroll
  for (int r = 0; r < 10; ++r) {
    const uint64_t p0 = (uint64_t)0xD2511F53u * c0;
    const uint64_t p1 = (uint64_t)0xCD9E8D57u * c2;
    const uint32_t n0 = (uint32_t)(p1 >> 32) ^ c1 ^ k0;
    const uint32_t n1 = (uint32_t)p1;
    const uint32_t n2 = (uint32_t)(p0 >> 32) ^ c3 ^ k1;
    const uint32_t n3 = (uint32_t)p0;
    c0 = n0;
    c1 = n1;
    c2 = n2;
    c3 = n3;
    k0 += 0x9E3779B9u;
    k1 += 0xBB67AE85u;
  }
  Philox4 o;
  o.w[0] = c0;
  o.w[1] = c1;
  o.w[2] = c2;
  o.w[3] = c3;
  return o;
}

#ifndef ABD_TRANSIT_P_U32
#define ABD_TRANSIT_P_U32 3435973836u
#endif

struct GibbsArgs {
  EvalArgs e;
  uint32_t seed_lo, seed_hi, sweep;
  uint32_t ind_offset;
  uint32_t stream[ABD_MAX_BATCH_K];
  double theta0[ABD_MAX_BATCH_K];
  double theta7[ABD_MAX_BATCH_K];
  double is2_n[ABD_MAX_BATCH_K];
  double is2_s[ABD_MAX_BATCH_K];
  unsigned long long* counts;
  unsigned int* work;
  unsigned long long* stats;
  int32_t refill_min, tail_lanes, tail_age;
};


#define ABD_G2_REFILL_MIN 16
#define ABD_G2_TAIL_LANES 8
#define ABD_G2_TAIL_AGE 6
```

Baseline: 251,700 evals/s.

## Add per-lane-group transposed bit planes for infection/vaccination in dense walk

Adds a per-chain plane buffer that holds infection and vaccination bits transposed so each 64-lane group reads one uint64 mask per gap. The planes are rebuilt by a ballot-based transpose kernel after constrain, flip and Gibbs updates. The dense eval kernel gets a variant that walks these planes through scalar (constant address space) loads and tracks first exposure with wave-wide masks, replacing per-lane word extraction. The cost is an extra transpose launch after every discrete-state change, more memory per slot, and more template instantiations. It also disables FP contraction in several hot functions, which may change the instruction mix.

```diff
diff --git a/abdpymc_amd/csrc/abd_context.hip b/abdpymc_amd/csrc/abd_context.hip
--- a/abdpymc_amd/csrc/abd_context.hip
+++ b/abdpymc_amd/csrc/abd_context.hip
@@ -66,9 +66,30 @@
   p.waner = c->slots[chain].waner;
   p.iw = c->slots[chain].iw;
   p.cnt = c->slots[chain].cnt;
+  p.pl = c->slots[chain].pl;
   return p;
 }
 ChainPar chain_par(const abd_ctx* c, int chain, const double* t) { return chain_par(c, chain, transform(t)); }
+
+int enqueue_planes(abd_ctx* c, int m, const int32_t* chains, hipStream_t st, int lg0, int n_lg) {
+  if (!c->dense) return ABD_OK;
+  if (m < 1 || m > ABD_MAX_BATCH_K) return fail(ABD_ERR_STATE, "internal: planes of %d slots in one launch", m);
+  if (n_lg < 0) n_lg = c->n_lg - lg0;
+  if (lg0 < 0 || n_lg < 1 || lg0 + n_lg > c->n_lg) return fail(ABD_ERR_STATE, "internal: planes of lane groups [%d, %d) of %d", lg0, lg0 + n_lg, c->n_lg);
+  PlaneArgs a;
+  std::memset(&a, 0, sizeof a);
+  for (int k = 0; k < m; ++k) {
+    a.src[k] = c->slots[(size_t)chains[k]].iw;
+    a.dst[k] = c->slots[(size_t)chains[k]].pl;
+  }
+  a.N = c->N;
+  a.G = c->G;
+  a.which = 0;
+  a.lg0 = lg0;
+  hipLaunchKernelGGL(abd_planes_kernel, dim3(n_lg, c->nt, m), dim3(64), 0, st, a);
+  HIP_TRY(hipGetLastError());
+  return ABD_OK;
+}
 
 ConstrainArgs constrain_args(const abd_ctx* c) {
   ConstrainArgs a;
@@ -465,7 +486,20 @@
     HIP_TRY(s.waner.alloc((size_t)c->N));
     HIP_TRY(s.iw.alloc(words));
     HIP_TRY(s.cnt.alloc(2));
-  }
+    if (c->dense) {
+      HIP_TRY(s.pl.alloc_zero(abd_plane_words(c->n_lg, c->G), c->stream));
+      PlaneArgs a;
+      std::memset(&a, 0, sizeof a);
+      a.src[0] = c->vw;
+      a.dst[0] = s.pl;
+      a.N = c->N;
+      a.G = c->G;
+      a.which = 1;
+      hipLaunchKernelGGL(abd_planes_kernel, dim3(c->n_lg, c->nt, 1), dim3(64), 0, c->stream, a);
+      HIP_TRY(hipGetLastError());
+    }
+  }
+  c->dense_planes = env_int("ABD_DENSE_PLANES", 1) != 0;
   return ABD_OK;
 }
 
@@ -764,6 +798,7 @@
     hipLaunchKernelGGL(abd_constrain_kernel<ABD_MAXT>, dim3((c->N + 255) / 256), dim3(256), 0, c->stream, constrain_args(c), s.rw,
                        s.waner, s.iw, reinterpret_cast<unsigned long long*>(cnt));
   HIP_TRY(hipGetLastError());
+  if (int prc = enqueue_planes(c, 1, &chain, c->stream)) return prc;
   HIP_TRY(hipStreamSynchronize(c->stream));
   s.set = true;
   return ABD_OK;
@@ -786,6 +821,8 @@
     hipLaunchKernelGGL(abd_flip_kernel<ABD_MAXT>, dim3(1), dim3(1), 0, c->stream, constrain_args(c), s.rw, s.waner, s.iw,
                        reinterpret_cast<unsigned long long*>(cnt), c->G, flat);
   HIP_TRY(hipGetLastError());
+  if (flat < (int64_t)c->G * c->N)
+    if (int prc = enqueue_planes(c, 1, &chain, c->stream, (int)((flat % c->N) / 64), 1)) return prc;
   return ABD_OK;
 }
 int abd_deterministics(abd_ctx* c, int32_t chain, const double* theta, int8_t* i, double* mu_n, double* mu_s) {
diff --git a/abdpymc_amd/csrc/abd_dense.hpp b/abdpymc_amd/csrc/abd_dense.hpp
--- a/abdpymc_amd/csrc/abd_dense.hpp
+++ b/abdpymc_amd/csrc/abd_dense.hpp
@@ -3,6 +3,7 @@
 #include <cstddef>
 
 #include "abd_device.hpp"
+#include "abd_planes.hpp"
 #include "abd_terms.hpp"
 
 typedef uint32_t abd_u32x4 __attribute__((ext_vector_type(4)));
@@ -99,6 +100,7 @@
 #define ABD_EXP2_C2 0x1.ebfbe033445b4p-23
 __device__ __forceinline__ void one_plus_exp2_pair(double t_n, double t_s, const double* tab , double c2v, double& A,
                                                    double& B) {
+#pragma clang fp contract(off)
   const double kf_n = __builtin_rint(t_n), kf_s = __builtin_rint(t_s);
   const double f_n = t_n - kf_n, f_s = t_s - kf_s;
   int k_n, k_s;
@@ -122,6 +124,7 @@
 template <bool GRAD>
 __device__ __forceinline__ void obs_pair_scaled(double t_n, double yn, double d_n, double t_s, double ys, double d_s,
                                                 const double* tab, double c2v, double (&acc)[16], double& h_n, double& h_s) {
+#pragma clang fp contract(off)
   double A, B;
   one_plus_exp2_pair(t_n, t_s, tab, c2v, A, B);
   const double r = rcp_newton(A * B);
@@ -131,8 +134,8 @@
   acc[A_S_Q2] = fma(q_s, q_s, acc[A_S_Q2]);
   if (GRAD) {
     const double u_n = q_n * s_n, u_s = q_s * s_s;
-    acc[A_N_QS] += u_n;
-    acc[A_S_QS] += u_s;
+    acc[A_N_QS] = fma(s_n, q_n, acc[A_N_QS]);
+    acc[A_S_QS] = fma(s_s, q_s, acc[A_S_QS]);
     h_n = fma(-u_n, s_n, u_n);
     h_s = fma(-u_s, s_s, u_s);
     acc[A_N_H] += h_n;
@@ -184,7 +187,7 @@
   int wj;
 };
 
-template <typename R, bool XC, typename ARGS>
+template <typename R, bool XC, bool WORDS, typename ARGS>
 __device__ __forceinline__ void piece_issue_loads(const ARGS& a, const RowDesc<XC>& rs_n, const RowDesc<XC>& rs_s,
                                                   const uint32_t* ibase, const uint32_t* vbase, const int8_t* waner, int lane, int j,
                                                   int g0, int g1, PieceLoads<R, XC>& pl) {
@@ -203,13 +206,15 @@
     pl.on = row_load<R, XC>(rs_n, lane, ro, N);
     pl.os = row_load<R, XC>(rs_s, lane, ro, N);
   }
-  const uint32_t j2 = 2u * (uint32_t)j;
-  pl.seg_i = word32(ibase, j2, q, N);
-  pl.seg_v = word32(vbase, j2, q, N);
-  pl.nxt_i = pl.nxt_v = 0;
-  if (q < q_end) {
-    pl.nxt_i = word32(ibase, j2, q + 1, N);
-    pl.nxt_v = word32(vbase, j2, q + 1, N);
+  pl.seg_i = pl.seg_v = pl.nxt_i = pl.nxt_v = 0;
+  if constexpr (WORDS) {
+    const uint32_t j2 = 2u * (uint32_t)j;
+    pl.seg_i = word32(ibase, j2, q, N);
+    pl.seg_v = word32(vbase, j2, q, N);
+    if (q < q_end) {
+      pl.nxt_i = word32(ibase, j2, q + 1, N);
+      pl.nxt_v = word32(vbase, j2, q + 1, N);
+    }
   }
   pl.wj = waner[j];
 }
@@ -294,6 +299,7 @@
                                            uint32_t j2, PieceLoads<R, XC>& pl, int lane, int g0, int g1, bool wj, double tn, double dn, double ts,
                                            double ds, uint32_t cfn_hi, uint32_t cfs_hi, const double* tab_e2, double c2v,
                                            double (&acc)[16]) {
+#pragma clang fp contract(off)
   const int N = a.N;
   const double rho_n = k.rho_n, ct_n = k.ct_n, cp_n = k.cp_n, ci_n = k.ci_n, mc_n = k.mc_n;
   const double c_s = k.c_s, cp_s = k.cp_s, ci_s = k.ci_s, mc_s = k.mc_s, d_n = k.d_n, d_s = k.d_s;
@@ -362,6 +368,96 @@
     if (g < g1 && (g & 31) == 0) next_word();
   }
   if (g < g1) step(g, en, es);
+  acc[A_S_HD] += wj ? hd_s : 0.0;
+}
+
+
+typedef uint64_t abd_u64x2 __attribute__((ext_vector_type(2)));
+typedef uint64_t abd_u64x4 __attribute__((ext_vector_type(4)));
+static_assert(sizeof(abd_u64x2) == sizeof(PlaneGap) && sizeof(abd_u64x4) == sizeof(PlanePair), "plane layout (abd_types.hpp)");
+typedef const abd_u64x2 __attribute__((address_space(4)))* plane_gap_ptr;
+typedef const abd_u64x4 __attribute__((address_space(4)))* plane_pair_ptr;
+__device__ __forceinline__ plane_gap_ptr plane_row(const uint64_t* planes, int lg, int G) {
+  return (plane_gap_ptr)(uintptr_t)(planes + abd_plane_index(lg, 0, G, 0));
+}
+__device__ __forceinline__ uint32_t mask_select(uint64_t mask, uint32_t on, uint32_t off) {
+  return __builtin_amdgcn_inverse_ballot_w64(mask) ? on : off;
+}
+
+template <typename R, bool GRAD, bool XC, typename ARGS>
+__device__ __forceinline__ void dense_walk_planes(const ARGS& a, const DenseChain& k, const RowDesc<XC>& rs_n,
+                                                  const RowDesc<XC>& rs_s, const double* dict_n, const double* dict_s,
+                                                  plane_gap_ptr prow, PieceLoads<R, XC>& pl, int lane, int g0, int g1, bool wj, double tn,
+                                                  double dn, double ts, double ds, uint32_t cfn_hi, uint32_t cfs_hi, ExposureSeen seen,
+                                                  const double* tab_e2, double c2v, double (&acc)[16]) {
+#pragma clang fp contract(off)
+  const int N = a.N;
+  const double rho_n = k.rho_n, ct_n = k.ct_n, mc_n = k.mc_n;
+  const double c_s = k.c_s, mc_s = k.mc_s, d_n = k.d_n, d_s = k.d_s;
+  const double rho_j = wj ? k.rho_s : 1.0;
+  double hd_s = 0.0;
+  const uint32_t z_ei = zero_vgpr(), z_ev = zero_vgpr(), z_cn = zero_vgpr(), z_cs = zero_vgpr();
+  const double b1_n = fma(1.0, k.cp_n, k.ci_n), b1_s = fma(1.0, k.cp_s, k.ci_s);
+  double base_n = cfn_hi ? b1_n : fma(0.0, k.cp_n, k.ci_n), base_s = cfs_hi ? b1_s : fma(0.0, k.cp_s, k.ci_s);
+  const int last = g1 - 1 - g0;
+  auto ldrow = [&](const RowDesc<XC>& rs, int g) { return row_load<R, XC>(rs, lane, min(g - g0, last), N); };
+
+  auto step = [&](uint64_t m_i, uint64_t m_v, const RowData<R, XC>& on, const RowData<R, XC>& os) {
+    const ExposureSeen nw = abd_exposure_new(seen, m_i, m_v);
+    if ((nw.n | nw.s) != 0) {
+      cfn_hi = mask_select(nw.n, 0x3FF00000u, cfn_hi);
+      cfs_hi = mask_select(nw.s, 0x3FF00000u, cfs_hi);
+      base_n = __hiloint2double((int)mask_select(nw.n, (uint32_t)__double2hiint(b1_n), (uint32_t)__double2hiint(base_n)),
+                                (int)mask_select(nw.n, (uint32_t)__double2loint(b1_n), (uint32_t)__double2loint(base_n)));
+      base_s = __hiloint2double((int)mask_select(nw.s, (uint32_t)__double2hiint(b1_s), (uint32_t)__double2hiint(base_s)),
+                                (int)mask_select(nw.s, (uint32_t)__double2loint(b1_s), (uint32_t)__double2loint(base_s)));
+      abd_exposure_mark(seen, m_i, m_v);
+    }
+    const double e_i = hi_to_double(mask_select(m_i, 0x3FF00000u, 0u), z_ei), e_v = hi_to_double(mask_select(m_v, 0x3FF00000u, 0u), z_ev);
+    dn = fma_s(rho_n, dn, tn);
+    tn = fma_s(rho_n, tn, e_i);
+    ds = fma_v(rho_j, ds, ts);
+    ts = fma_v(rho_j, ts, e_i + e_v);
+    const double cf_n = hi_to_double(cfn_hi, z_cn), cf_s = hi_to_double(cfs_hi, z_cs);
+    const double t_n = fma(mc_n, row_x<R, XC>(on, dict_n), fma(ct_n, tn, base_n));
+    const double t_s = fma(mc_s, row_x<R, XC>(os, dict_s), fma(c_s, ts, base_s));
+    double h_n = 0.0, h_s = 0.0;
+    obs_pair_scaled<GRAD>(t_n, row_y<R, XC>(on), d_n, t_s, row_y<R, XC>(os), d_s, tab_e2, c2v, acc, h_n, h_s);
+    if (GRAD) {
+      acc[A_N_HC] = fma(h_n, cf_n, acc[A_N_HC]);
+      acc[A_N_HU] = fma(h_n, tn, acc[A_N_HU]);
+      acc[A_N_HD] = fma(h_n, dn, acc[A_N_HD]);
+      acc[A_S_HC] = fma(h_s, cf_s, acc[A_S_HC]);
+      hd_s = fma(h_s, ds, hd_s);
+      asm volatile("" : "+v"(cfn_hi), "+v"(cfs_hi), "+v"(base_n), "+v"(base_s), "+v"(acc[A_N_HC]), "+v"(acc[A_S_HC]));
+    } else {
+      asm volatile("" : "+v"(base_n), "+v"(base_s), "+v"(acc[A_N_Q2]), "+v"(acc[A_S_Q2]));
+    }
+  };
+
+  RowData<R, XC> en = pl.en, es = pl.es, on = pl.on, os = pl.os;
+  int g = g0;
+  abd_u64x4 cur = *(plane_pair_ptr)(prow + ((g0 + 1) & ~1));
+  if (g & 1) {
+    const abd_u64x2 m = prow[g];
+    step(m.x, m.y, on, os);
+    on = ldrow(rs_n, g + 2);
+    os = ldrow(rs_s, g + 2);
+    ++g;
+  }
+  while (g + 1 < g1) {
+    const abd_u64x4 nxt = *(plane_pair_ptr)(prow + g + 2);
+    __builtin_amdgcn_sched_barrier(0);
+    step(cur.x, cur.y, en, es);
+    en = ldrow(rs_n, g + 2);
+    es = ldrow(rs_s, g + 2);
+    step(cur.z, cur.w, on, os);
+    on = ldrow(rs_n, g + 3);
+    os = ldrow(rs_s, g + 3);
+    cur = nxt;
+    g += 2;
+  }
+  if (g < g1) step(cur.x, cur.y, en, es);
   acc[A_S_HD] += wj ? hd_s : 0.0;
 }
 
@@ -554,7 +650,7 @@
   return true;
 }
 
-template <typename R, int CB, bool GRAD, bool XC, typename ARGS>
+template <typename R, int CB, bool GRAD, bool XC, bool PL, typename ARGS>
 __device__ __forceinline__ void dense_body(const ARGS& a) {
   constexpr bool TRAINK = is_train_args<ARGS>::value;
   static_assert(CB * ABD_NOUT <= 64, "the own-sum hand-off needs every partial row of the workgroup stored by wave 0");
@@ -591,6 +687,7 @@
     p.rw = nullptr;
     p.waner = tc.waner;
     p.iw = tc.iw;
+    p.pl = tc.pl;
     p.cnt = tc.cnt;
     p.perm_n = p.temp_n = p.rho_n = p.init_n = p.perm_s = p.rho_s = p.init_s = p.b_n = p.d_n = p.b_s = p.d_s = 0.0;
     if (chain_on) {
@@ -657,7 +754,7 @@
   uint32_t wi[ABD_SW], wv[ABD_SW];
   const bool first_inside = rows_left > 0 && j < N && g0 > 0;
   RowDesc<XC> rs_n = row_desc<R, XC>(a, 0, lg, g0), rs_s = row_desc<R, XC>(a, 1, lg, g0);
-  if (rows_left > 0 && j < N) piece_issue_loads<R, XC>(a, rs_n, rs_s, ibase, vbase, p.waner, lane, j, g0, g1, pl);
+  if (rows_left > 0 && j < N) piece_issue_loads<R, XC, !PL>(a, rs_n, rs_s, ibase, vbase, p.waner, lane, j, g0, g1, pl);
   if (first_inside) state_issue_loads(ibase, vbase, 2u * (uint32_t)j, N, g0, wi, wv);
   long long n1 = 0, m1 = 0;
   if (blk == 0 && sub == 0 && chain_on) {
@@ -704,14 +801,24 @@
   ABD_STAMP(5);
   if (first_inside)
     dense_start_state(wi, wv, ibase, vbase, 2u * (uint32_t)j, N, g0, tab_n, tab_s, pl.wj != 0, tn, dn, ts, ds, cfn_hi, cfs_hi);
+  ExposureSeen seen = {0, 0};
+  if constexpr (PL) {
+    seen.n = __builtin_amdgcn_ballot_w64(cfn_hi != 0);
+    seen.s = __builtin_amdgcn_ballot_w64(cfs_hi != 0);
+  }
   if (NSUB == 1) __syncthreads();
   ABD_STAMP(6);
 
   while (rows_left > 0) {
     rows_left -= g1 - g0;
-    if (j < N)
-      dense_walk<R, GRAD, XC>(a, kc, rs_n, rs_s, dict_n, dict_s, ibase, vbase, 2u * (uint32_t)j, pl, lane, g0, g1, pl.wj != 0, tn, dn, ts, ds, cfn_hi, cfs_hi, tab_e2, c2v,
-                          acc);
+    if (j < N) {
+      if constexpr (PL)
+        dense_walk_planes<R, GRAD, XC>(a, kc, rs_n, rs_s, dict_n, dict_s, plane_row(p.pl, lg, G), pl, lane, g0, g1, pl.wj != 0, tn, dn, ts, ds, cfn_hi,
+                                       cfs_hi, seen, tab_e2, c2v, acc);
+      else
+        dense_walk<R, GRAD, XC>(a, kc, rs_n, rs_s, dict_n, dict_s, ibase, vbase, 2u * (uint32_t)j, pl, lane, g0, g1, pl.wj != 0, tn, dn, ts, ds, cfn_hi, cfs_hi,
+                                tab_e2, c2v, acc);
+    }
     if (rows_left <= 0) break;
     ++lg;
     g0 = 0;
@@ -719,9 +826,10 @@
     j = lg * 64 + lane;
     tn = dn = ts = ds = 0.0;
     cfn_hi = cfs_hi = 0;
+    seen.n = seen.s = 0;
     rs_n = row_desc<R, XC>(a, 0, lg, g0);
     rs_s = row_desc<R, XC>(a, 1, lg, g0);
-    if (j < N) piece_issue_loads<R, XC>(a, rs_n, rs_s, ibase, vbase, p.waner, lane, j, g0, g1, pl);
+    if (j < N) piece_issue_loads<R, XC, !PL>(a, rs_n, rs_s, ibase, vbase, p.waner, lane, j, g0, g1, pl);
   }
 
   ABD_STAMP(7);
@@ -812,15 +920,20 @@
   }
 }
 
-template <typename R, int CB, bool GRAD, bool XC>
+template <typename R, int CB, bool GRAD, bool XC, bool TRAIN>
+struct dense_plane_form {
+  static constexpr bool value = !TRAIN;
+};
+
+template <typename R, int CB, bool GRAD, bool XC, bool PL>
 #ifndef ABD_DENSE_MINW
 #define ABD_DENSE_MINW 4
 #endif
 __global__ __launch_bounds__(ABD_BLOCK, ABD_DENSE_MINW) void abd_dense_kernel(const EvalArgs a) {
-  dense_body<R, CB, GRAD, XC, EvalArgs>(a);
-}
-
-template <typename R, int CB, bool XC>
+  dense_body<R, CB, GRAD, XC, PL, EvalArgs>(a);
+}
+
+template <typename R, int CB, bool XC, bool PL>
 __global__ __launch_bounds__(ABD_BLOCK, ABD_DENSE_MINW) void abd_train_kernel(const DenseTrainArgs a) {
-  dense_body<R, CB, true, XC, DenseTrainArgs>(a);
-}
+  dense_body<R, CB, true, XC, PL, DenseTrainArgs>(a);
+}
diff --git a/abdpymc_amd/csrc/abd_eval.hip b/abdpymc_amd/csrc/abd_eval.hip
--- a/abdpymc_amd/csrc/abd_eval.hip
+++ b/abdpymc_amd/csrc/abd_eval.hip
@@ -19,13 +19,19 @@
 
 enum class Family { Dense, Lanes, Sparse };
 using EvalKernel = void (*)(const EvalArgs);
+template <typename R, int CB, bool GRAD, bool XC>
+EvalKernel dense_kernel(bool planes) {
+  if constexpr (dense_plane_form<R, CB, GRAD, XC, false>::value)
+    if (planes) return abd_dense_kernel<R, CB, GRAD, XC, true>;
+  return abd_dense_kernel<R, CB, GRAD, XC, false>;
+}
 template <typename R, bool GRAD>
-EvalKernel eval_kernel(Family f, int cpw, bool xc, bool wide) {
+EvalKernel eval_kernel(Family f, int cpw, bool xc, bool wide, bool planes) {
   switch (f) {
     case Family::Dense:
-      if (cpw == 4) return xc ? abd_dense_kernel<R, 4, GRAD, true> : abd_dense_kernel<R, 4, GRAD, false>;
-      if (cpw == 2) return xc ? abd_dense_kernel<R, 2, GRAD, true> : abd_dense_kernel<R, 2, GRAD, false>;
-      return xc ? abd_dense_kernel<R, 1, GRAD, true> : abd_dense_kernel<R, 1, GRAD, false>;
+      if (cpw == 4) return xc ? dense_kernel<R, 4, GRAD, true>(planes) : dense_kernel<R, 4, GRAD, false>(planes);
+      if (cpw == 2) return xc ? dense_kernel<R, 2, GRAD, true>(planes) : dense_kernel<R, 2, GRAD, false>(planes);
+      return xc ? dense_kernel<R, 1, GRAD, true>(planes) : dense_kernel<R, 1, GRAD, false>(planes);
     case Family::Sparse:
       if (cpw == 2) return wide ? abd_sparse_kernel<R, 2, GRAD, ABD_MAXT_MAX> : abd_sparse_kernel<R, 2, GRAD, ABD_MAXT>;
       return wide ? abd_sparse_kernel<R, 1, GRAD, ABD_MAXT_MAX> : abd_sparse_kernel<R, 1, GRAD, ABD_MAXT>;
@@ -217,8 +223,9 @@
   }
   if (c->timing == 2 && stream_ordered) c->win_launches += steps;
   const bool f32 = c->storage == ABD_STORE_F32, xc = p.family == Family::Dense && dense_xc(c, p.cpw), wide = c->nt > ABD_MAXT;
-  const EvalKernel k = f32 ? (grad ? eval_kernel<float, true>(p.family, p.cpw, xc, wide) : eval_kernel<float, false>(p.family, p.cpw, xc, wide))
-                           : (grad ? eval_kernel<double, true>(p.family, p.cpw, xc, wide) : eval_kernel<double, false>(p.family, p.cpw, xc, wide));
+  const bool pf = c->dense_planes;
+  const EvalKernel k = f32 ? (grad ? eval_kernel<float, true>(p.family, p.cpw, xc, wide, pf) : eval_kernel<float, false>(p.family, p.cpw, xc, wide, pf))
+                           : (grad ? eval_kernel<double, true>(p.family, p.cpw, xc, wide, pf) : eval_kernel<double, false>(p.family, p.cpw, xc, wide, pf));
   const hipError_t le = profiled_launch(false, [&] { return launch_kernel(k, p.grid, dim3(ABD_BLOCK), p.lds, pp.st, a); });
   if (e1) HIP_TRY(hipEventRecord(e1, pp.st));
   HIP_TRY(le);
@@ -344,11 +351,17 @@
 }
 
 using TrainKernel = void (*)(const DenseTrainArgs);
+template <typename R, int CB, bool XC>
+TrainKernel train_kernel_form(bool planes) {
+  if constexpr (dense_plane_form<R, CB, true, XC, true>::value)
+    if (planes) return abd_train_kernel<R, CB, XC, true>;
+  return abd_train_kernel<R, CB, XC, false>;
+}
 template <typename R>
-TrainKernel train_kernel(int cb, bool xc) {
-  if (cb == 4) return xc ? abd_train_kernel<R, 4, true> : abd_train_kernel<R, 4, false>;
-  if (cb == 2) return xc ? abd_train_kernel<R, 2, true> : abd_train_kernel<R, 2, false>;
-  return xc ? abd_train_kernel<R, 1, true> : abd_train_kernel<R, 1, false>;
+TrainKernel train_kernel(int cb, bool xc, bool planes) {
+  if (cb == 4) return xc ? train_kernel_form<R, 4, true>(planes) : train_kernel_form<R, 4, false>(planes);
+  if (cb == 2) return xc ? train_kernel_form<R, 2, true>(planes) : train_kernel_form<R, 2, false>(planes);
+  return xc ? train_kernel_form<R, 1, true>(planes) : train_kernel_form<R, 1, false>(planes);
 }
 
 int enqueue_dense_train(abd_ctx* c, int pi, int cb, int blocks, DenseTrainArgs* a) {
@@ -358,7 +371,7 @@
   for (int k = 0; k < cb; ++k) {
     TrainChainArgs& tc = a->tc[k];
     if (tc.action != ABD_TR_SKIP || tc.fwd_slot >= 0) {
-      if (!tc.st || !tc.ring || !tc.iw || !tc.cnt || !tc.waner || (tc.action == ABD_TR_BEGIN && !tc.begin))
+      if (!tc.st || !tc.ring || !tc.iw || !tc.pl || !tc.cnt || !tc.waner || (tc.action == ABD_TR_BEGIN && !tc.begin))
         return fail(ABD_ERR_STATE, "internal: train launch with a NULL pointer for chain %d of the unit", k);
       if ((tc.action == ABD_TR_STEP && (tc.use_slot | 1) != 1) || tc.fwd_slot > 1)
         return fail(ABD_ERR_STATE, "internal: train launch with slot %d / %d for chain %d of the unit", tc.use_slot, tc.fwd_slot, k);
@@ -405,7 +418,7 @@
   range_split(c, blocks, ABD_WAVES_PER_BLOCK / cb, *a, false);
   const size_t lds = abd_dense_lds(c->G, cb, xc, true);
   dim3 grid(blocks + a->service, 1);
-  const TrainKernel k = c->storage == ABD_STORE_F32 ? train_kernel<float>(cb, xc) : train_kernel<double>(cb, xc);
+  const TrainKernel k = c->storage == ABD_STORE_F32 ? train_kernel<float>(cb, xc, c->dense_planes) : train_kernel<double>(cb, xc, c->dense_planes);
   const hipError_t le = profiled_launch(false, [&] { return launch_kernel(k, grid, dim3(ABD_BLOCK), lds, c->pipe[pi].st, *a); });
   HIP_TRY(le);
   return ABD_OK;
diff --git a/abdpymc_amd/csrc/abd_gibbs.hip b/abdpymc_amd/csrc/abd_gibbs.hip
--- a/abdpymc_amd/csrc/abd_gibbs.hip
+++ b/abdpymc_amd/csrc/abd_gibbs.hip
@@ -59,7 +59,7 @@
   const bool stats = stats_dev != nullptr;
   const GibbsKernel k = c->storage == ABD_STORE_F32 ? gibbs_kernel<float>(c, stats) : gibbs_kernel<double>(c, stats);
   HIP_TRY(launch_kernel(k, grid, block, lds, st, ga));
-  return ABD_OK;
+  return enqueue_planes(c, m, chains, st);
 }
 
 }
diff --git a/abdpymc_amd/csrc/abd_host.hpp b/abdpymc_amd/csrc/abd_host.hpp
--- a/abdpymc_amd/csrc/abd_host.hpp
+++ b/abdpymc_amd/csrc/abd_host.hpp
@@ -119,6 +119,7 @@
   DevBuf<int8_t> waner;
   DevBuf<uint64_t> iw;
   DevBuf<long long> cnt;
+  DevBuf<uint64_t> pl;
   bool set = false;
 };
 
@@ -187,6 +188,7 @@
   int next_pipe = 0;
   double seq = 0.0;
   bool dense_own_sum = true;
+  bool dense_planes = true;
   DevBuf<unsigned int> d_fin_count;
   DevBuf<unsigned int> d_train_count;
   uint32_t ind_offset = 0;
@@ -230,6 +232,7 @@
 ChainPar chain_par(const abd_ctx* c, int chain, const Transformed& tr);
 ChainPar chain_par(const abd_ctx* c, int chain, const double* t);
 void base_args(const abd_ctx* c, EvalArgs& a);
+int enqueue_planes(abd_ctx* c, int m, const int32_t* chains, hipStream_t st, int lg0 = 0, int n_lg = -1);
 #ifdef ABD_STAMPS
 unsigned long long* stamps_buffer();
 #endif
diff --git a/abdpymc_amd/csrc/abd_planes.hpp b/abdpymc_amd/csrc/abd_planes.hpp
--- /dev/null
+++ b/abdpymc_amd/csrc/abd_planes.hpp
@@ -0,0 +1,42 @@
+#pragma once
+
+#include "abd_types.hpp"
+
+__host__ __device__ inline int abd_plane_gaps(int G) { return ((G + 1) & ~1) + 2; }
+__host__ __device__ inline size_t abd_plane_words(int n_lg, int G) { return (size_t)n_lg * (size_t)abd_plane_gaps(G) * 2; }
+__host__ __device__ inline size_t abd_plane_index(int lg, int g, int G, int which) {
+  return ((size_t)lg * (size_t)abd_plane_gaps(G) + (size_t)g) * 2 + (size_t)which;
+}
+
+inline void abd_plane_transpose_ref(const uint64_t* words, int N, int G, int which, uint64_t* planes) {
+  const int n_lg = (N + 63) / 64;
+  for (int lg = 0; lg < n_lg; ++lg)
+    for (int g = 0; g < G; ++g) {
+      uint64_t m = 0;
+      for (int l = 0; l < 64; ++l) {
+        const int j = lg * 64 + l;
+        if (j < N) m |= ((words[(size_t)(g >> 6) * N + j] >> (g & 63)) & 1ull) << l;
+      }
+      planes[abd_plane_index(lg, g, G, which)] = m;
+    }
+}
+
+struct ExposureSeen {
+  uint64_t n, s;
+};
+__host__ __device__ inline ExposureSeen abd_exposure_start(uint64_t infected_before, uint64_t vaccinated_before) {
+  ExposureSeen s;
+  s.n = infected_before;
+  s.s = infected_before | vaccinated_before;
+  return s;
+}
+__host__ __device__ inline ExposureSeen abd_exposure_new(const ExposureSeen& seen, uint64_t m_i, uint64_t m_v) {
+  ExposureSeen nw;
+  nw.n = m_i & ~seen.n;
+  nw.s = (m_i | m_v) & ~seen.s;
+  return nw;
+}
+__host__ __device__ inline void abd_exposure_mark(ExposureSeen& seen, uint64_t m_i, uint64_t m_v) {
+  seen.n |= m_i;
+  seen.s |= m_i | m_v;
+}
diff --git a/abdpymc_amd/csrc/abd_sampler.hip b/abdpymc_amd/csrc/abd_sampler.hip
--- a/abdpymc_amd/csrc/abd_sampler.hip
+++ b/abdpymc_amd/csrc/abd_sampler.hip
@@ -855,6 +855,7 @@
           tc.ring = d.ring.dev();
           tc.begin = d.begin.dev();
           tc.iw = slot.iw;
+          tc.pl = slot.pl;
           tc.cnt = slot.cnt;
           tc.waner = slot.waner;
           tc.action = ABD_TR_SKIP;
diff --git a/abdpymc_amd/csrc/abd_small.hpp b/abdpymc_amd/csrc/abd_small.hpp
--- a/abdpymc_amd/csrc/abd_small.hpp
+++ b/abdpymc_amd/csrc/abd_small.hpp
@@ -1,6 +1,7 @@
 #pragma once
 
 #include "abd_device.hpp"
+#include "abd_planes.hpp"
 
 __global__ void abd_spin_kernel(unsigned long long* out, unsigned long long ticks) {
   const unsigned long long t0 = __builtin_amdgcn_s_memrealtime();
@@ -97,6 +98,24 @@
   }
 }
 
+struct PlaneArgs {
+  const uint64_t* src[ABD_MAX_BATCH_K];
+  uint64_t* dst[ABD_MAX_BATCH_K];
+  int32_t N, G, which, lg0;
+};
+__global__ __launch_bounds__(64) void abd_planes_kernel(const PlaneArgs a) {
+  const int lane = threadIdx.x, lg = a.lg0 + (int)blockIdx.x, t = blockIdx.y, k = blockIdx.z;
+  const int j = lg * 64 + lane;
+  const uint64_t w = j < a.N ? a.src[k][(int64_t)t * a.N + j] : 0ull;
+  uint64_t mine = 0;
+  for (int b = 0; b < 64; ++b) {
+    const uint64_t m = __builtin_amdgcn_ballot_w64(((w >> b) & 1ull) != 0);
+    if (lane == b) mine = m;
+  }
+  const int g = t * 64 + lane;
+  if (g < a.G) a.dst[k][abd_plane_index(lg, g, a.G, a.which)] = mine;
+}
+
 template <int MT>
 __global__ __launch_bounds__(ABD_BLOCK) void abd_deterministics_kernel(const EvalArgs a, int8_t* __restrict__ out_i,
                                                                        double* __restrict__ out_mun,
diff --git a/abdpymc_amd/csrc/abd_terms.hpp b/abdpymc_amd/csrc/abd_terms.hpp
--- a/abdpymc_amd/csrc/abd_terms.hpp
+++ b/abdpymc_amd/csrc/abd_terms.hpp
@@ -152,7 +152,7 @@
   p.b_s = tr[14];
   p.d_s = tr[15];
 }
-static_assert(sizeof(ChainPar) == 11 * sizeof(double) + 4 * sizeof(void*), "ChainPar changed: review chain_par_from_tr (11 constants) and chain_par (4 pointers)");
+static_assert(sizeof(ChainPar) == 11 * sizeof(double) + 5 * sizeof(void*), "ChainPar changed: review chain_par_from_tr (11 constants) and chain_par (5 pointers)");
 
 
 ABD_HD void transform_lane(int k, double t, double& tr, double& l0, double& l1) {
diff --git a/abdpymc_amd/csrc/abd_types.hpp b/abdpymc_amd/csrc/abd_types.hpp
--- a/abdpymc_amd/csrc/abd_types.hpp
+++ b/abdpymc_amd/csrc/abd_types.hpp
@@ -43,6 +43,14 @@
   const int8_t* waner;
   const uint64_t* iw;
   const long long* cnt;
+  const uint64_t* pl;
+};
+
+struct alignas(16) PlaneGap {
+  uint64_t i, v;
+};
+struct alignas(32) PlanePair {
+  PlaneGap a, b;
 };
 
 #define ABD_NT 17
@@ -112,6 +120,7 @@
   const uint64_t* iw;
   const long long* cnt;
   const int8_t* waner;
+  const uint64_t* pl;
   int32_t action;
   int32_t use_slot;
   int32_t own;
@@ -194,6 +203,7 @@
   ChainPar ch[ABD_MAX_BATCH_K];
   TrainArgs train;
 };
+static_assert(sizeof(EvalArgs) <= 4096 && sizeof(DenseTrainArgs) <= 4096, "kernel arguments exceed the 4 KiB argument segment");
 
 __host__ __device__ inline uint32_t abd_div_magic(uint32_t G) { return G > 1 ? (uint32_t)((((uint64_t)1 << 32) + G - 1) / G) : 0u; }
 __host__ __device__ inline uint32_t abd_div_by_magic(uint32_t row, uint32_t magic) { return (uint32_t)(((uint64_t)row * magic) >> 32); }
```

New measurement: 258,400 evals/s (median of 6 runs). 2.6% higher.
